# MoonInTheRiver/NeuralSVB

Measured on NVIDIA B200. Metric: audio-seconds/sec generated (HiFi-GAN-NSF generator forward), higher is better.
Workload: dtype 3xbf16 split operands (16-bit mantissa), fp32 accumulate, fp32 storage

## Files before the change

include/svb_vocoder.h:

```cpp
#ifndef SVB_VOCODER_H_
#define SVB_VOCODER_H_

#include <stdint.h>

#ifdef __cplusplus
extern "C" {
#endif

#define SVB_ABI_VERSION 1

typedef enum svb_status {
    SVB_OK = 0,
    SVB_ERR_INVALID = -1,
    SVB_ERR_CUDA = -2,
    SVB_ERR_STATE = -3,
    SVB_ERR_MISSING = -4,
    SVB_ERR_NOMEM = -5
} svb_status;

typedef enum svb_precision {
    SVB_PREC_FP32 = 0,
    SVB_PREC_TF32 = 1,
    SVB_PREC_TF32X3 = 2,
    SVB_PREC_BF16X3 = 3
} svb_precision;

#define SVB_MAX_UPS 8
#define SVB_MAX_RBK 4
#define SVB_MAX_DIL 4

typedef struct svb_gen_config {
    int32_t n_mel;
    int32_t upsample_initial_channel;
    int32_t n_ups;
    int32_t upsample_rates[SVB_MAX_UPS];
    int32_t upsample_kernel_sizes[SVB_MAX_UPS];
    int32_t resblock;
    int32_t n_resblock_kernels;
    int32_t resblock_kernel_sizes[SVB_MAX_RBK];
    int32_t n_dilations;
    int32_t resblock_dilation_sizes[SVB_MAX_RBK][SVB_MAX_DIL];
    int32_t use_pitch_embed;
    int32_t audio_sample_rate;
    int32_t precision;
} svb_gen_config;

typedef struct svb_gen svb_gen_t;

const char *svb_last_error(void);
int svb_abi_version(void);


int svb_gen_create(const svb_gen_config *cfg, int device, svb_gen_t **out);
void svb_gen_destroy(svb_gen_t *g);

int svb_gen_set_weight(svb_gen_t *g, const char *name, const float *data, const int64_t *shape, int32_t ndim);
int svb_fold_weight_norm_host(const float *v_host, const float *g_host, int64_t d0, int64_t inner,
                              float *w_host, int device);
int svb_gen_finalize(svb_gen_t *g);
int svb_gen_set_precision(svb_gen_t *g, int32_t precision);

int svb_gen_forward(svb_gen_t *g, const float *mel_dev, const float *f0_dev, const float *rand_ini_dev,
                    const float *noise_dev, uint64_t seed, int32_t B, int32_t T, float *wav_dev, void *stream);

int svb_gen_spec2wav_host(svb_gen_t *g, const float *mel_host, const float *f0_host, uint64_t seed,
                          int32_t B, int32_t T, float *wav_host, void *stream);

int svb_gen_spec2wav_host_i16(svb_gen_t *g, const float *mel_host, const float *f0_host, uint64_t seed, int32_t B,
                              int32_t T, int32_t norm, int16_t *wav_host, void *stream);
int svb_wav_to_int16(const float *wav_dev, int32_t B, int64_t n, int32_t norm, int16_t *out_dev, void *stream);

int svb_gen_forward_ragged(svb_gen_t *g, const float *mel_dev, const float *f0_dev, const int32_t *lengths_host,
                           const float *rand_ini_dev, const float *noise_dev, uint64_t seed, int32_t B, int32_t T_max,
                           float *wav_dev, void *stream);
int svb_gen_spec2wav_ragged_host(svb_gen_t *g, const float *mel_host, const float *f0_host, const int32_t *lengths_host,
                                 int32_t B, uint64_t seed, float *wav_host, void *stream);
int svb_gen_spec2wav_ragged_host_i16(svb_gen_t *g, const float *mel_host, const float *f0_host, const int32_t *lengths_host,
                                     int32_t B, uint64_t seed, int32_t norm, int16_t *wav_host, void *stream);

int svb_gen_get_tap(svb_gen_t *g, const char *name, float *out_dev, int64_t capacity_floats,
                    int64_t *shape3, void *stream);
int64_t svb_gen_hop(const svb_gen_t *g);
int64_t svb_gen_last_launches(const svb_gen_t *g);
double svb_gen_last_flops(const svb_gen_t *g);
int svb_gen_enable_timing(svb_gen_t *g, int32_t on);
float svb_gen_last_ms(svb_gen_t *g);
int32_t svb_gen_profile_count(svb_gen_t *g);
int svb_gen_profile_get(svb_gen_t *g, int32_t i, char *name, int32_t name_cap, float *ms, double *bytes, double *flops);

int svb_conv_nct_backward(const float *x_dev, const float *w_dev, const float *y_dev, const float *dy_dev, int32_t B,
                          int32_t Cin, int32_t Cout, int32_t Tin, int32_t W, int32_t K, int32_t stride, int32_t dil,
                          int32_t pad, int32_t groups, float out_slope, float *dz_scratch_dev, float *dx_dev,
                          float *dw_dev, float *db_dev, void *stream);
int svb_cond_net_forward(const float *mel_dev, const float *w_dev, const float *bias_dev, int32_t B, int32_t C, int32_t T,
                         int32_t K, int32_t stride, int32_t pad, float *y_dev, void *stream);
int svb_cond_net_backward(const float *mel_dev, const float *dy_dev, int32_t B, int32_t C, int32_t T, int32_t K, int32_t stride,
                          int32_t pad, float *dw_dev, float *db_dev, void *stream);
int svb_avgpool1d_4_2_1_backward(const float *dy_dev, float *dx_dev, int64_t rows, int32_t Tin, void *stream);
int svb_pad_reflect_right_backward(const float *dy_dev, float *dx_dev, int64_t rows, int32_t T, int32_t Tpad, void *stream);
int svb_loss_grad(const float *a_dev, const float *b_dev, int32_t kind, float scale, float *da_dev, int64_t n,
                  int32_t accumulate, void *stream);
int svb_loss_grad_dev(const float *a_dev, const float *b_dev, int32_t kind, float scale, const float *scale_dev,
                      float *da_dev, int64_t n, int32_t accumulate, void *stream);

typedef struct svb_tc_layer svb_tc_layer_t;
int svb_tc_layer_create(int32_t Cin, int32_t Cout, int32_t K, int32_t stride, int32_t pad, int32_t precision, int device,
                        svb_tc_layer_t **out);
int svb_tc_layer_create_grouped(int32_t Cin, int32_t Cout, int32_t K, int32_t stride, int32_t pad, int32_t groups,
                                int32_t precision, int device, svb_tc_layer_t **out);
void svb_tc_layer_destroy(svb_tc_layer_t *layer);
int svb_tc_layer_set_weight_dev(svb_tc_layer_t *layer, const float *w_dev, const float *bias_dev, void *stream);
int64_t svb_tc_layer_out_len(const svb_tc_layer_t *layer, int64_t T);
int svb_tc_layer_forward(svb_tc_layer_t *layer, const float *x_dev, int32_t B, int32_t T, int32_t W, float out_slope,
                         float *y_dev, void *stream);
int svb_tc_layer_backward(svb_tc_layer_t *layer, const float *x_dev, const float *y_dev, const float *dy_dev, int32_t B,
                          int32_t T, int32_t W, float out_slope, float *dx_dev, float *dw_dev, float *db_dev, void *stream);

int svb_gen_set_training(svb_gen_t *g, int32_t on);
int svb_gen_update_weights(svb_gen_t *g);
int svb_gen_set_weight_dev(svb_gen_t *g, const char *name, const float *src_dev, int64_t n, void *stream);
int svb_gen_update_weights_dev(svb_gen_t *g, void *stream);
int svb_fold_weight_norm_dev(const float *v_dev, const float *g_dev, int64_t d0, int64_t inner, float *w_dev, void *stream);
int svb_gen_zero_grad(svb_gen_t *g, void *stream);
int svb_gen_backward(svb_gen_t *g, const float *dwav_dev, void *stream);
int64_t svb_gen_grad_numel(svb_gen_t *g, const char *name);
int svb_gen_get_grad(svb_gen_t *g, const char *name, float *dst_dev, int64_t n, void *stream);
int64_t svb_gen_bwd_launches(const svb_gen_t *g);
int svb_weight_norm_backward(const float *v_dev, const float *g_dev, const float *dw_dev, int64_t rows, int64_t cols,
                             float *dv_dev, float *dg_dev, void *stream);

int svb_conv1d_run(const float *x_nct_dev, const float *w_host, const float *bias_host, const float *res_nct_dev,
                   int32_t B, int32_t Cin, int32_t Cout, int32_t T, int32_t K, int32_t dil,
                   int32_t transposed_stride, float in_slope, float out_scale, int32_t precision, int32_t iters,
                   float *y_nct_dev, float *avg_ms, void *stream);


int svb_conv_nct_forward(const float *x_dev, const float *w_dev, const float *bias_dev, float *y_dev, int32_t B,
                         int32_t Cin, int32_t Cout, int32_t Tin, int32_t W, int32_t K, int32_t stride, int32_t dil,
                         int32_t pad, int32_t groups, float out_slope, void *stream);
int svb_avgpool1d_4_2_1(const float *x_dev, float *y_dev, int64_t rows, int32_t Tin, void *stream);
int svb_pad_reflect_right(const float *x_dev, float *y_dev, int64_t rows, int32_t T, int32_t Tpad, void *stream);
int svb_pair_stats(const float *a_dev, const float *b_dev, int64_t n, int32_t want_log, double *out6_dev, void *stream);
int svb_spectral_sigma_host(const float *w_host, const float *u_host, const float *v_host, int64_t rows, int64_t inner,
                            int device, float *sigma);


typedef enum svb_pad_mode {
    SVB_PAD_CENTER_ZERO = 0,
    SVB_PAD_CENTER_REFLECT = 1,
    SVB_PAD_HALF_REFLECT = 2
} svb_pad_mode;

typedef enum svb_spec_out {
    SVB_OUT_LOG10_MEL = 0,
    SVB_OUT_LN_MEL = 1,
    SVB_OUT_MAG = 2,
    SVB_OUT_MAG_RAW = 3,
    SVB_OUT_MEL_MAG = 4
} svb_spec_out;

typedef struct svb_stft_config {
    int32_t n_fft;
    int32_t hop;
    int32_t win;
    int32_t pad_mode;
    int32_t out_kind;
    int32_t clamp_input;
    int32_t n_mels;
    int32_t frames_major;
    float eps;
} svb_stft_config;

int64_t svb_stft_num_frames(const svb_stft_config *cfg, int64_t n);

int svb_stft_forward(const svb_stft_config *cfg, const float *wav_dev, int32_t B, int64_t n,
                     const float *mel_basis_dev, float *out_dev, void *stream);
int svb_stft_backward(const svb_stft_config *cfg, const float *wav_dev, int32_t B, int64_t n, const float *mel_basis_dev,
                      const float *dout_dev, float *dwav_dev, void *stream);

int svb_denoise(const svb_stft_config *cfg, const float *wav_dev, int32_t B, int64_t n, float v, float *out_dev, void *stream);

int64_t svb_wav2spec_host(const svb_stft_config *cfg, const float *wav_host, int64_t n,
                          const float *mel_basis_host, float *mel_host, float *wav_out_host, int device,
                          void *stream);

int64_t svb_wav2spec_batch_host(const svb_stft_config *cfg, const float *wav_concat_host, const int64_t *lengths,
                                int32_t n_clips, const float *mel_basis_host, float *mel_concat_host, int64_t *frames_out,
                                int device, void *stream);

typedef struct svb_wn svb_wn_t;
int svb_wn_create(int32_t hidden_channels, int32_t kernel_size, int32_t dilation_rate, int32_t n_layers, int32_t gin_channels,
                  int32_t precision, int32_t device, svb_wn_t **out);
void svb_wn_destroy(svb_wn_t *w);
int svb_wn_set_weight(svb_wn_t *w, const char *name, const float *data_host, const int64_t *shape, int32_t ndim);
int svb_wn_finalize(svb_wn_t *w);
int svb_wn_forward(svb_wn_t *w, const float *x_dev, const float *mask_dev, const float *g_dev, int32_t B, int32_t T, float *out_dev,
                   void *stream);
int svb_fvae_decoder_create(int32_t latent_channels, int32_t hidden_channels, int32_t out_channels, int32_t kernel_size, int32_t n_layers,
                            int32_t gin_channels, int32_t stride, int32_t precision, int32_t device, svb_wn_t **out);
int svb_fvae_decoder_forward(svb_wn_t *w, const float *z_dev, const float *mask_dev, const float *g_dev, int32_t B, int32_t T,
                             float *out_dev, void *stream);

int svb_layer_norm_nct(const float *x_dev, const float *gamma_dev, const float *beta_dev, int32_t B, int32_t C, int32_t T, float eps,
                       float *y_dev, void *stream);
int svb_relpos_attention_nct(const float *q_dev, const float *k_dev, const float *v_dev, const float *p_dev, const float *bias_u_dev,
                             const float *bias_v_dev, const float *mask_dev, int32_t B, int32_t C, int32_t T, int32_t n_head,
                             float *out_dev, void *stream);

int64_t svb_tc_schedule_probe(int32_t n_layers, const int32_t *KS, const int32_t *has_res, const int32_t *accumulate, int32_t Cin, int32_t B,
                              int32_t Tq, int32_t MT, int32_t col_blocks, int32_t chain_ordered, int32_t grid, int32_t *items_out,
                              int64_t items_capacity, int32_t *off_out, double *balance_out);
int64_t svb_tc_schedule_probe_ragged(int32_t n_layers, const int32_t *KS, const int32_t *has_res, const int32_t *accumulate,
                                     int32_t Cin, int32_t B, const int32_t *rows_per_clip, int32_t MT, int32_t col_blocks,
                                     int32_t chain_ordered, int32_t grid, int32_t *items_out, int64_t items_capacity,
                                     int32_t *off_out, double *balance_out);

#ifdef __cplusplus
}
#endif
#endif
```

neuralsvb_b200/_native.py:

```python
import ctypes
import os
import shutil
import subprocess
import threading

_HERE = os.path.dirname(os.path.abspath(__file__))
_ROOT = os.path.dirname(_HERE)
CSRC = os.path.join(_HERE, 'csrc')
LIB_PATH = os.path.join(_HERE, 'libsvb_vocoder.so')
HEADER = os.path.join(_ROOT, 'include', 'svb_vocoder.h')
SOURCES = ['wn.cu', 'conformer.cu', 'api.cu', 'conv_ffma.cu', 'conv_tc.cu', 'nsf_source.cu', 'frontend.cu', 'generator.cu', 'layer_api.cu', 'disc_ops.cu',
           'train_ops.cu', 'generator_bwd.cu', 'disc_bwd.cu', 'tc_layer.cu', 'wgrad_tc.cu']
NVCC_FLAGS = ['-gencode', 'arch=compute_100a,code=sm_100a', '-lineinfo', '-O3', '-std=c++17',
              '-Xcompiler', '-fPIC', '-shared']

SVB_MAX_UPS, SVB_MAX_RBK, SVB_MAX_DIL = 8, 4, 4
PREC = {'fp32': 0, 'tf32': 1, 'tf32x3': 2, 'bf16x3': 3}
PAD_CENTER_ZERO, PAD_CENTER_REFLECT, PAD_HALF_REFLECT = 0, 1, 2
OUT_LOG10_MEL, OUT_LN_MEL, OUT_MAG, OUT_MAG_RAW, OUT_MEL_MAG = 0, 1, 2, 3, 4


class GenConfig(ctypes.Structure):
    _fields_ = [
        ('n_mel', ctypes.c_int32),
        ('upsample_initial_channel', ctypes.c_int32),
        ('n_ups', ctypes.c_int32),
        ('upsample_rates', ctypes.c_int32 * SVB_MAX_UPS),
        ('upsample_kernel_sizes', ctypes.c_int32 * SVB_MAX_UPS),
        ('resblock', ctypes.c_int32),
        ('n_resblock_kernels', ctypes.c_int32),
        ('resblock_kernel_sizes', ctypes.c_int32 * SVB_MAX_RBK),
        ('n_dilations', ctypes.c_int32),
        ('resblock_dilation_sizes', (ctypes.c_int32 * SVB_MAX_DIL) * SVB_MAX_RBK),
        ('use_pitch_embed', ctypes.c_int32),
        ('audio_sample_rate', ctypes.c_int32),
        ('precision', ctypes.c_int32),
    ]


class StftConfig(ctypes.Structure):
    _fields_ = [
        ('n_fft', ctypes.c_int32), ('hop', ctypes.c_int32), ('win', ctypes.c_int32),
        ('pad_mode', ctypes.c_int32), ('out_kind', ctypes.c_int32), ('clamp_input', ctypes.c_int32),
        ('n_mels', ctypes.c_int32), ('frames_major', ctypes.c_int32), ('eps', ctypes.c_float),
    ]


def sources():
    return [os.path.join(CSRC, s) for s in SOURCES if os.path.exists(os.path.join(CSRC, s))]


def _stale():
    if not os.path.exists(LIB_PATH):
        return True
    t = os.path.getmtime(LIB_PATH)
    deps = sources() + [HEADER] + [os.path.join(CSRC, f) for f in os.listdir(CSRC) if f.endswith('.cuh')]
    return any(os.path.getmtime(d) > t for d in deps)


def build(force=False, verbose=False):
    if not force and not _stale():
        return LIB_PATH
    nvcc = shutil.which('nvcc') or '/usr/local/cuda/bin/nvcc'
    if not os.path.exists(nvcc):
        raise RuntimeError('nvcc not found: cannot build libsvb_vocoder.so')
    cmd = [nvcc] + NVCC_FLAGS + sources() + ['-o', LIB_PATH + '.tmp']
    if verbose:
        print(' '.join(cmd))
    r = subprocess.run(cmd, capture_output=True, text=True)
    if r.returncode != 0:
        raise RuntimeError('nvcc failed:\n' + r.stdout + r.stderr)
    os.replace(LIB_PATH + '.tmp', LIB_PATH)
    return LIB_PATH


_lib = None
_lock = threading.Lock()

_P = ctypes.c_void_p
_I32, _I64, _U64 = ctypes.c_int32, ctypes.c_int64, ctypes.c_uint64

_PROTOS = {
    'svb_last_error': (ctypes.c_char_p, []),
    'svb_abi_version': (ctypes.c_int, []),
    'svb_gen_create': (ctypes.c_int, [ctypes.POINTER(GenConfig), ctypes.c_int, ctypes.POINTER(_P)]),
    'svb_gen_destroy': (None, [_P]),
    'svb_gen_set_weight': (ctypes.c_int, [_P, ctypes.c_char_p, _P, ctypes.POINTER(_I64), _I32]),
    'svb_fold_weight_norm_host': (ctypes.c_int, [_P, _P, _I64, _I64, _P, ctypes.c_int]),
    'svb_gen_finalize': (ctypes.c_int, [_P]),
    'svb_gen_set_precision': (ctypes.c_int, [_P, _I32]),
    'svb_gen_forward': (ctypes.c_int, [_P, _P, _P, _P, _P, _U64, _I32, _I32, _P, _P]),
    'svb_gen_spec2wav_host': (ctypes.c_int, [_P, _P, _P, _U64, _I32, _I32, _P, _P]),
    'svb_gen_get_tap': (ctypes.c_int, [_P, ctypes.c_char_p, _P, _I64, ctypes.POINTER(_I64), _P]),
    'svb_gen_hop': (_I64, [_P]),
    'svb_gen_last_launches': (_I64, [_P]),
    'svb_gen_last_flops': (ctypes.c_double, [_P]),
    'svb_gen_enable_timing': (ctypes.c_int, [_P, _I32]),
    'svb_gen_last_ms': (ctypes.c_float, [_P]),
    'svb_conv_nct_backward': (ctypes.c_int, [_P, _P, _P, _P, _I32, _I32, _I32, _I32, _I32, _I32, _I32, _I32, _I32, _I32,
                                             ctypes.c_float, _P, _P, _P, _P, _P]),
    'svb_avgpool1d_4_2_1_backward': (ctypes.c_int, [_P, _P, _I64, _I32, _P]),
    'svb_cond_net_forward': (ctypes.c_int, [_P, _P, _P, _I32, _I32, _I32, _I32, _I32, _I32, _P, _P]),
    'svb_cond_net_backward': (ctypes.c_int, [_P, _P, _I32, _I32, _I32, _I32, _I32, _I32, _P, _P, _P]),
    'svb_pad_reflect_right_backward': (ctypes.c_int, [_P, _P, _I64, _I32, _I32, _P]),
    'svb_loss_grad': (ctypes.c_int, [_P, _P, _I32, ctypes.c_float, _P, _I64, _I32, _P]),
    'svb_loss_grad_dev': (ctypes.c_int, [_P, _P, _I32, ctypes.c_float, _P, _P, _I64, _I32, _P]),
    'svb_tc_layer_create': (ctypes.c_int, [_I32, _I32, _I32, _I32, _I32, _I32, ctypes.c_int, ctypes.POINTER(_P)]),
    'svb_tc_layer_create_grouped': (ctypes.c_int, [_I32, _I32, _I32, _I32, _I32, _I32, _I32, ctypes.c_int, ctypes.POINTER(_P)]),
    'svb_tc_layer_destroy': (None, [_P]),
    'svb_tc_layer_set_weight_dev': (ctypes.c_int, [_P, _P, _P, _P]),
    'svb_tc_layer_out_len': (_I64, [_P, _I64]),
    'svb_tc_layer_forward': (ctypes.c_int, [_P, _P, _I32, _I32, _I32, ctypes.c_float, _P, _P]),
    'svb_tc_layer_backward': (ctypes.c_int, [_P, _P, _P, _P, _I32, _I32, _I32, ctypes.c_float, _P, _P, _P, _P]),
    'svb_gen_set_training': (ctypes.c_int, [_P, _I32]),
    'svb_gen_update_weights': (ctypes.c_int, [_P]),
    'svb_gen_zero_grad': (ctypes.c_int, [_P, _P]),
    'svb_gen_set_weight_dev': (ctypes.c_int, [_P, ctypes.c_char_p, _P, _I64, _P]),
    'svb_gen_update_weights_dev': (ctypes.c_int, [_P, _P]),
    'svb_fold_weight_norm_dev': (ctypes.c_int, [_P, _P, _I64, _I64, _P, _P]),
    'svb_gen_backward': (ctypes.c_int, [_P, _P, _P]),
    'svb_gen_grad_numel': (_I64, [_P, ctypes.c_char_p]),
    'svb_gen_get_grad': (ctypes.c_int, [_P, ctypes.c_char_p, _P, _I64, _P]),
    'svb_gen_bwd_launches': (_I64, [_P]),
    'svb_weight_norm_backward': (ctypes.c_int, [_P, _P, _P, _I64, _I64, _P, _P, _P]),
    'svb_gen_profile_count': (_I32, [_P]),
    'svb_gen_profile_get': (ctypes.c_int, [_P, _I32, ctypes.c_char_p, _I32, ctypes.POINTER(ctypes.c_float),
                                            ctypes.POINTER(ctypes.c_double), ctypes.POINTER(ctypes.c_double)]),
    'svb_conv1d_run': (ctypes.c_int, [_P, _P, _P, _P, _I32, _I32, _I32, _I32, _I32, _I32, _I32, ctypes.c_float,
                                      ctypes.c_float, _I32, _I32, _P, ctypes.POINTER(ctypes.c_float), _P]),
    'svb_conv_nct_forward': (ctypes.c_int, [_P, _P, _P, _P, _I32, _I32, _I32, _I32, _I32, _I32, _I32, _I32, _I32, _I32,
                                            ctypes.c_float, _P]),
    'svb_avgpool1d_4_2_1': (ctypes.c_int, [_P, _P, _I64, _I32, _P]),
    'svb_pad_reflect_right': (ctypes.c_int, [_P, _P, _I64, _I32, _I32, _P]),
    'svb_pair_stats': (ctypes.c_int, [_P, _P, _I64, _I32, _P, _P]),
    'svb_spectral_sigma_host': (ctypes.c_int, [_P, _P, _P, _I64, _I64, ctypes.c_int, ctypes.POINTER(ctypes.c_float)]),
    'svb_stft_num_frames': (_I64, [ctypes.POINTER(StftConfig), _I64]),
    'svb_stft_forward': (ctypes.c_int, [ctypes.POINTER(StftConfig), _P, _I32, _I64, _P, _P, _P]),
    'svb_stft_backward': (ctypes.c_int, [ctypes.POINTER(StftConfig), _P, _I32, _I64, _P, _P, _P, _P]),
    'svb_denoise': (ctypes.c_int, [ctypes.POINTER(StftConfig), _P, _I32, _I64, ctypes.c_float, _P, _P]),
    'svb_wav2spec_host': (_I64, [ctypes.POINTER(StftConfig), _P, _I64, _P, _P, _P, ctypes.c_int, _P]),
    'svb_wav2spec_batch_host': (_I64, [ctypes.POINTER(StftConfig), _P, _P, _I32, _P, _P, _P, ctypes.c_int, _P]),
    'svb_gen_spec2wav_host_i16': (ctypes.c_int, [_P, _P, _P, _U64, _I32, _I32, _I32, _P, _P]),
    'svb_wav_to_int16': (ctypes.c_int, [_P, _I32, _I64, _I32, _P, _P]),
    'svb_wn_create': (ctypes.c_int, [_I32, _I32, _I32, _I32, _I32, _I32, _I32, ctypes.POINTER(_P)]),
    'svb_wn_destroy': (None, [_P]),
    'svb_wn_set_weight': (ctypes.c_int, [_P, ctypes.c_char_p, _P, ctypes.POINTER(_I64), _I32]),
    'svb_wn_finalize': (ctypes.c_int, [_P]),
    'svb_wn_forward': (ctypes.c_int, [_P, _P, _P, _P, _I32, _I32, _P, _P]),
    'svb_fvae_decoder_create': (ctypes.c_int, [_I32, _I32, _I32, _I32, _I32, _I32, _I32, _I32, _I32, ctypes.POINTER(_P)]),
    'svb_fvae_decoder_forward': (ctypes.c_int, [_P, _P, _P, _P, _I32, _I32, _P, _P]),
    'svb_tc_schedule_probe': (_I64, [_I32, _P, _P, _P, _I32, _I32, _I32, _I32, _I32, _I32, _I32, _P, _I64, _P, ctypes.POINTER(ctypes.c_double)]),
    'svb_tc_schedule_probe_ragged': (_I64, [_I32, _P, _P, _P, _I32, _I32, _P, _I32, _I32, _I32, _I32, _P, _I64, _P,
                                            ctypes.POINTER(ctypes.c_double)]),
    'svb_gen_forward_ragged': (ctypes.c_int, [_P, _P, _P, _P, _P, _P, _U64, _I32, _I32, _P, _P]),
    'svb_gen_spec2wav_ragged_host': (ctypes.c_int, [_P, _P, _P, _P, _I32, _U64, _P, _P]),
    'svb_gen_spec2wav_ragged_host_i16': (ctypes.c_int, [_P, _P, _P, _P, _I32, _U64, _I32, _P, _P]),
    'svb_layer_norm_nct': (ctypes.c_int, [_P, _P, _P, _I32, _I32, _I32, ctypes.c_float, _P, _P]),
    'svb_relpos_attention_nct': (ctypes.c_int, [_P, _P, _P, _P, _P, _P, _P, _I32, _I32, _I32, _I32, _P, _P]),
}


def declared_symbols():
    import re
    txt = open(HEADER).read()
    txt = re.sub(r'/\*.*?\*/', '', txt, flags=re.S)
    return sorted(set(re.findall(r'\b(svb_[a-z0-9_]+)\s*\(', txt)))


def lib():
    global _lib
    if _lib is not None:
        return _lib
    with _lock:
        if _lib is None:
            if not os.path.exists(LIB_PATH):
                raise RuntimeError(
                    f'{LIB_PATH} is missing: run `python -c "import __graft_entry__ as g; g.build()"` '
                    '(nvcc, sm_100a). neuralsvb_b200 has no CPU or PyTorch fallback.')
            l = ctypes.CDLL(LIB_PATH)
            for name, (res, args) in _PROTOS.items():
                if hasattr(l, name):
                    fn = getattr(l, name)
                    fn.restype, fn.argtypes = res, args
            _lib = l
    return _lib


def check(status, what=''):
    if status is not None and status < 0:
        msg = lib().svb_last_error().decode('utf-8', 'replace')
        raise RuntimeError(f'libsvb_vocoder {what} failed ({status}): {msg}')
    return status


def ptr(t):
    if t is None:
        return None
    assert t.is_contiguous(), 'native calls need contiguous tensors'
    return ctypes.c_void_p(t.data_ptr())


def current_stream_ptr(device=None):
    import torch
    return ctypes.c_void_p(torch.cuda.current_stream(device).cuda_stream)
```

neuralsvb_b200/csrc/conv_tc.cu:

```cuda
#include <algorithm>
#include <cmath>
#include <cstring>
#include <cstdlib>
#include <vector>

#include <cuda_bf16.h>

#include "conv_tc.cuh"
#include "tc_ptx.cuh"

namespace svb {

constexpr int kTcM = 128;
constexpr int kTcCK = 32;
constexpr int kMaxItems = 120;
constexpr int kItemBytes = 2048;


struct TcLayer {
    const float *in;
    const float *res;
    float *out;
    const float *bias;
    const unsigned char *w;
    int KS, dil;
    float out_scale;
    int accumulate;
    int bias_off;
    uint32_t w_res_off;
};

struct TcArgs {
    ConvArgs a;
    TcLayer L[kTcMaxLayers];
    int n_layers;
    const int4 *work;
    const int *work_off;
    int n_tile, n_chunks, MT, nW, nA, tmem_cols;
    int n_sets;
    int col_blocks, groups_per_b, total_groups;
    int w_resident;
    int blk_chunk_step;
    uint32_t w_res_bytes;
    int pdl;
    int collect;
    long long *stats;
    int dbg;
    uint32_t op_bytes;
    uint32_t wtile_bytes;
    uint32_t off_op, off_w, off_stage, off_bias;
};

constexpr int kMaxW = 8;
constexpr int kMaxDevices = 64;
constexpr int kTcThreadsP = 576;
constexpr int kWarpProducer = 16, kWarpMma = 17, kWarpTransform0 = 8;
constexpr int kStageBytes = 8 * 4096;
constexpr int kBiasBytes = 4096;

template <bool ST>
__device__ __forceinline__ void mbar_wait_t(uint64_t *bar, uint32_t parity, long long &acc) {
    if (ST) {
        const long long t = clock64();
        mbar_wait(bar, parity);
        acc += clock64() - t;
    } else {
        mbar_wait(bar, parity);
    }
}
template <bool ST>
__device__ __forceinline__ void mbar_wait_warp(uint64_t *bar, uint32_t parity, long long &acc) {
    mbar_wait_t<ST>(bar, parity, acc);
    __syncwarp();
}
constexpr int kTcStatSlots = 16;

struct TcItem {
    int layer, nblk, mt, b, t0, rows;
};
__device__ __forceinline__ TcItem item_decode(const int4 v) {
    TcItem it;
    it.layer = v.x & 0xff, it.nblk = (v.x >> 8) & 0xffff, it.mt = v.x >> 24, it.b = v.y, it.t0 = v.z, it.rows = v.w;
    return it;
}

template <int MODE, bool ST = false, bool RG = false>
__global__ void __launch_bounds__(kTcThreadsP, 1) conv1d_c4_tc_kernel(const __grid_constant__ TcArgs p) {
    extern __shared__ __align__(1024) unsigned char smem[];
    constexpr bool BF = MODE == SVB_PREC_BF16X3;
    constexpr bool X3 = MODE == SVB_PREC_TF32X3;
    const ConvArgs &a = p.a;
    uint64_t *bars = reinterpret_cast<uint64_t *>(smem);
    uint64_t *raw_full = bars, *a_ready = bars + 4, *a_empty = bars + 8;
    uint64_t *w_full = bars + 12, *w_empty = bars + 12 + kMaxW;
    uint64_t *acc_full = bars + 12 + 2 * kMaxW, *acc_empty = acc_full + 2;
    uint32_t *tmem_ptr = reinterpret_cast<uint32_t *>(acc_empty + 2);
    int *n_items_s = reinterpret_cast<int *>(tmem_ptr + 1);
    TcLayer *Ls = reinterpret_cast<TcLayer *>(smem + 512);
    const int4 *items = reinterpret_cast<const int4 *>(smem + 1024);
    unsigned char *op0 = smem + p.off_op;
    unsigned char *wring = smem + p.off_w;

    const int warp = threadIdx.x >> 5, lane = threadIdx.x & 31;
    const int acc_cols = p.MT * p.n_tile;
    long long st_w0 = 0, st_w1 = 0, st_w2 = 0;
    const long long st_t0 = ST ? clock64() : 0;
    unsigned long long st_g0 = 0;
    if (ST) asm volatile("mov.u64 %0, %%globaltimer;" : "=l"(st_g0));

    if (threadIdx.x == 0) {
        for (int i = 0; i < 4; ++i) mbar_init(raw_full + i, 1), mbar_init(a_ready + i, 8), mbar_init(a_empty + i, 1);
        for (int i = 0; i < 2; ++i) mbar_init(acc_full + i, 1), mbar_init(acc_empty + i, 8);
        for (int i = 0; i < kMaxW; ++i) mbar_init(w_full + i, 1), mbar_init(w_empty + i, 1);
        fence_barrier_init();
    }
    if (warp == kWarpMma) tmem_alloc(tmem_ptr, p.tmem_cols);
    {
        float *sb = reinterpret_cast<float *>(smem + p.off_bias);
        for (int l = 0; l < p.n_layers; ++l)
            for (int i = threadIdx.x; i < a.Cout; i += kTcThreadsP) sb[p.L[l].bias_off + i] = __ldg(p.L[l].bias + i);
        if (threadIdx.x < p.n_layers) Ls[threadIdx.x] = p.L[threadIdx.x];
        int4 *it_w = reinterpret_cast<int4 *>(smem + 1024);
        if (p.work) {
            const int i0 = __ldg(p.work_off + blockIdx.x), n = __ldg(p.work_off + blockIdx.x + 1) - i0;
            for (int i = threadIdx.x; i < n; i += kTcThreadsP) it_w[i] = __ldg(p.work + i0 + i);
            if (threadIdx.x == 0) *n_items_s = n;
        } else if (RG) {
            if (threadIdx.x == 0) {
                int n = 0;
                for (int g = blockIdx.x; g < p.total_groups; g += gridDim.x) {
                    const int tg = g % p.groups_per_b, r = g / p.groups_per_b, b = r % a.B;
                    const int rows = a.rows[b] * a.rows_mul, tiles = (rows + kTcM - 1) / kTcM;
                    if (tg * p.MT >= tiles) continue;
                    it_w[n++] = make_int4(((r / a.B) << 8) | (min(p.MT, tiles - tg * p.MT) << 24), b, tg * (kTcM * p.MT), rows);
                }
                *n_items_s = n;
            }
        } else {
            const int n = ((int)blockIdx.x < p.total_groups) ? (p.total_groups - 1 - (int)blockIdx.x) / (int)gridDim.x + 1 : 0;
            for (int i = threadIdx.x; i < n; i += kTcThreadsP) {
                const int g = blockIdx.x + i * gridDim.x;
                const int tg = g % p.groups_per_b, r = g / p.groups_per_b;
                it_w[i] = make_int4(((r / a.B) << 8) | (p.MT << 24), r % a.B, tg * (kTcM * p.MT), a.Tq);
            }
            if (threadIdx.x == 0) *n_items_s = n;
        }
    }
    tc_fence_before();
    __syncthreads();
    tc_fence_after();
    const uint32_t tmem_base = *tmem_ptr;
    const int n_items = *n_items_s;
    if (p.pdl) {
        asm volatile("griddepcontrol.wait;" ::: "memory");
        asm volatile("griddepcontrol.launch_dependents;" ::: "memory");
    }

    if (warp == kWarpProducer) {
        if (lane == 0) {
            const int gin = c4t_groups(a.Cin);
            const size_t group_stride = (size_t)a.in_Tp * 32;
            int sA = 0, phA = 1, sW = 0, phW = 1;
            if (p.w_resident && n_items > 0) {
                mbar_expect_tx(w_full, p.w_res_bytes);
                for (int l = 0; l < p.n_layers; ++l)
                    bulk_g2s(wring + Ls[l].w_res_off, Ls[l].w, (uint32_t)Ls[l].KS * p.wtile_bytes, w_full);
            }
            for (int n = 0; n < n_items; ++n) {
                const TcItem it = item_decode(items[n]);
                const TcLayer &L = Ls[it.layer];
                const int halo = (L.KS - 1) / 2 * L.dil;
                const uint32_t raw_bytes = (uint32_t)(it.mt * kTcM + 2 * halo) * 128;
                const float *in_c = L.in + (((size_t)it.b * gin + (size_t)it.nblk * p.blk_chunk_step) * a.in_Tp + (kPad + it.t0 - halo)) * 32;
                const unsigned char *w_k = L.w + (size_t)it.nblk * p.n_chunks * L.KS * p.wtile_bytes;
                for (int c = 0; c < p.n_chunks; ++c) {
                    mbar_wait_t<ST>(a_empty + sA, phA, st_w0);
                    mbar_expect_tx(raw_full + sA, raw_bytes);
                    bulk_g2s(op0 + sA * p.op_bytes, in_c, raw_bytes, raw_full + sA);
                    in_c += group_stride;
                    if (++sA == p.nA) sA = 0, phA ^= 1;
                    if (!p.w_resident) {
                        for (int k = 0; k < L.KS; ++k) {
                            mbar_wait_t<ST>(w_empty + sW, phW, st_w1);
                            mbar_expect_tx(w_full + sW, p.wtile_bytes);
                            bulk_g2s(wring + sW * p.wtile_bytes, w_k, p.wtile_bytes, w_full + sW);
                            w_k += p.wtile_bytes;
                            if (++sW == p.nW) sW = 0, phW ^= 1;
                        }
                    }
                }
            }
            if (ST) {
                long long *o = p.stats + (size_t)blockIdx.x * kTcStatSlots;
                o[0] = st_w0, o[1] = st_w1, o[2] = clock64() - st_t0;
            }
        }
    } else if (warp == kWarpMma) {
        const uint32_t elected = elect_one_sync();
        const uint32_t idesc = umma_idesc(BF ? 1 : 2, kTcM, p.n_tile);
        const uint32_t hi_word = desc_hi_sw128(0);
        const uint32_t a_lo_plane = (X3 ? p.op_bytes / 2 : 64u) >> 4;
        const uint32_t b_lo_plane = (X3 ? p.wtile_bytes / 2 : 64u) >> 4;
        const uint32_t op_base = desc_lo(smem_u32(op0)), w_base = desc_lo(smem_u32(wring));
        const uint32_t op_step = p.op_bytes >> 4, wtile_step = p.wtile_bytes >> 4;
        const bool mma_on = ST ? !(p.dbg & 1) : true, hh_only = ST ? (p.dbg & 2) != 0 : false, collect = ST ? p.collect != 0 : true;
        int sA = 0, phA = 0, sW = 0, phW = 0, as = 0, phE = 1;
        if (p.w_resident && n_items > 0) {
            mbar_wait_warp<ST>(w_full, 0, st_w2);
            tc_fence_after();
        }
        const int n_items_u = __reduce_max_sync(0xffffffffu, n_items);
        for (int n = 0; n < n_items_u; ++n) {
            const int ix = __reduce_max_sync(0xffffffffu, items[n].x);
            const int layer = ix & 0xff, mt = ix >> 24;
            const int KS = p.L[layer].KS;
            const uint32_t tap_step = (uint32_t)p.L[layer].dil * (128 >> 4);
            const uint32_t w_res_off = p.L[layer].w_res_off >> 4;
            mbar_wait_warp<ST>(acc_empty + as, phE, st_w0);
            tc_fence_after();
            const uint32_t d_set = tmem_base + (uint32_t)(as * acc_cols);
            uint32_t fresh = 1;
            for (int c = 0; c < p.n_chunks; ++c) {
                mbar_wait_warp<ST>(a_ready + sA, phA, st_w1);
                tc_fence_after();
                uint32_t a_tap = op_base + sA * op_step;
                uint32_t b_tap = w_base + w_res_off;
                for (int k = 0; k < KS; ++k) {
                    if (!p.w_resident) {
                        mbar_wait_warp<ST>(w_full + sW, phW, st_w2);
                        tc_fence_after();
                        b_tap = w_base + sW * wtile_step;
                    }
                    if (mma_on) {
                        uint32_t d = d_set, a_row = a_tap;
#pragma unroll 1
                        for (int m = 0; m < mt; ++m) {
                            const uint32_t acc = fresh ^ 1u;
                            if (BF) {
                                if (hh_only) {
                                    umma<true>(d, a_row, hi_word, b_tap, hi_word, idesc, acc, elected);
                                    umma<true>(d, a_row + 2, hi_word, b_tap + 2, hi_word, idesc, 1u, elected);
                                } else if (collect) {
                                    umma<true>(d, a_row + a_lo_plane, hi_word, b_tap, hi_word, idesc, acc, elected);
                                    umma<true, 1>(d, a_row, hi_word, b_tap + b_lo_plane, hi_word, idesc, 1u, elected);
                                    umma<true, 2>(d, a_row, hi_word, b_tap, hi_word, idesc, 1u, elected);
                                    umma<true>(d, a_row + a_lo_plane + 2, hi_word, b_tap + 2, hi_word, idesc, 1u, elected);
                                    umma<true, 1>(d, a_row + 2, hi_word, b_tap + b_lo_plane + 2, hi_word, idesc, 1u, elected);
                                    umma<true, 2>(d, a_row + 2, hi_word, b_tap + 2, hi_word, idesc, 1u, elected);
                                } else {
                                    umma<true>(d, a_row + a_lo_plane, hi_word, b_tap, hi_word, idesc, acc, elected);
                                    umma<true>(d, a_row, hi_word, b_tap + b_lo_plane, hi_word, idesc, 1u, elected);
                                    umma<true>(d, a_row, hi_word, b_tap, hi_word, idesc, 1u, elected);
                                    umma<true>(d, a_row + a_lo_plane + 2, hi_word, b_tap + 2, hi_word, idesc, 1u, elected);
                                    umma<true>(d, a_row + 2, hi_word, b_tap + b_lo_plane + 2, hi_word, idesc, 1u, elected);
                                    umma<true>(d, a_row + 2, hi_word, b_tap + 2, hi_word, idesc, 1u, elected);
                                }
                            } else {
#pragma unroll
                                for (uint32_t kb = 0; kb < 8; kb += 2) {
                                    const uint32_t acc_k = kb == 0 ? acc : 1u;
                                    if (X3) {
                                        umma<false>(d, a_row + a_lo_plane + kb, hi_word, b_tap + kb, hi_word, idesc, acc_k, elected);
                                        umma<false, 1>(d, a_row + kb, hi_word, b_tap + b_lo_plane + kb, hi_word, idesc, 1u, elected);
                                        umma<false, 2>(d, a_row + kb, hi_word, b_tap + kb, hi_word, idesc, 1u, elected);
                                    } else {
                                        umma<false>(d, a_row + kb, hi_word, b_tap + kb, hi_word, idesc, acc_k, elected);
                                    }
                                }
                            }
                            d += (uint32_t)p.n_tile, a_row += (kTcM * 128) >> 4;
                        }
                    }
                    fresh = 0;
                    a_tap += tap_step, b_tap += wtile_step;
                    if (!p.w_resident) {
                        umma_commit(w_empty + sW, elected);
                        if (++sW == p.nW) sW = 0, phW ^= 1;
                    }
                }
                umma_commit(a_empty + sA, elected);
                if (++sA == p.nA) sA = 0, phA ^= 1;
            }
            umma_commit(acc_full + as, elected);
            if (++as == p.n_sets) as = 0, phE ^= 1;
        }
        if (ST && elected) {
            long long *o = p.stats + (size_t)blockIdx.x * kTcStatSlots;
            o[3] = st_w0, o[4] = st_w1, o[5] = st_w2, o[6] = clock64() - st_t0;
        }
    } else if (warp >= kWarpTransform0) {
        const int tid = threadIdx.x - kWarpTransform0 * 32;
        const int cl = tid & 7;
        const bool odd = cl & 1;
        const float slope = a.in_slope;
        int sA = 0, phA = 0;
        for (int n = 0; n < n_items; ++n) {
            const TcItem it = item_decode(items[n]);
            const int R = it.mt * kTcM + (Ls[it.layer].KS - 1) / 2 * Ls[it.layer].dil * 2;
            for (int c = 0; c < p.n_chunks; ++c) {
                mbar_wait_t<ST>(raw_full + sA, phA, st_w0);
                uint4 *op = reinterpret_cast<uint4 *>(op0 + sA * p.op_bytes);
                for (int r0 = 0; r0 < ((p.dbg & 4) ? 0 : R); r0 += 64) {
                    int rr[2];
                    bool ok[2];
                    float4 v[2];
#pragma unroll
                    for (int u = 0; u < 2; ++u) {
                        rr[u] = r0 + 32 * u + (tid >> 3);
                        ok[u] = rr[u] < R;
                        v[u] = make_float4(0.f, 0.f, 0.f, 0.f);
                        if (ok[u]) v[u] = *reinterpret_cast<const float4 *>(op + (size_t)rr[u] * 8 + cl);
                    }
#pragma unroll
                    for (int u = 0; u < 2; ++u) {
                        float4 &x = v[u];
                        x.x = fmaxf(x.x, x.x * slope), x.y = fmaxf(x.y, x.y * slope);
                        x.z = fmaxf(x.z, x.z * slope), x.w = fmaxf(x.w, x.w * slope);
                    }
                    if (BF) {
                        uint32_t h0[2], h1[2], l0[2], l1[2], g0[2], g1[2];
#pragma unroll
                        for (int u = 0; u < 2; ++u) {
                            const __nv_bfloat162 hA = __floats2bfloat162_rn(v[u].x, v[u].y), hB = __floats2bfloat162_rn(v[u].z, v[u].w);
                            h0[u] = *reinterpret_cast<const uint32_t *>(&hA), h1[u] = *reinterpret_cast<const uint32_t *>(&hB);
                            const __nv_bfloat162 lA = __floats2bfloat162_rn(v[u].x - __uint_as_float(h0[u] << 16),
                                                                           v[u].y - __uint_as_float(h0[u] & 0xffff0000u));
                            const __nv_bfloat162 lB = __floats2bfloat162_rn(v[u].z - __uint_as_float(h1[u] << 16),
                                                                           v[u].w - __uint_as_float(h1[u] & 0xffff0000u));
                            l0[u] = *reinterpret_cast<const uint32_t *>(&lA), l1[u] = *reinterpret_cast<const uint32_t *>(&lB);
                        }
#pragma unroll
                        for (int u = 0; u < 2; ++u) {
                            g0[u] = __shfl_xor_sync(0xffffffffu, odd ? h0[u] : l0[u], 1);
                            g1[u] = __shfl_xor_sync(0xffffffffu, odd ? h1[u] : l1[u], 1);
                        }
#pragma unroll
                        for (int u = 0; u < 2; ++u) {
                            if (!ok[u]) continue;
                            uint4 *row = op + (size_t)rr[u] * 8;
                            const int sw = rr[u] & 7;
                            if (!odd) row[(cl >> 1) ^ sw] = make_uint4(h0[u], h1[u], g0[u], g1[u]);
                            else row[(4 + (cl >> 1)) ^ sw] = make_uint4(g0[u], g1[u], l0[u], l1[u]);
                        }
                    } else {
                        __syncwarp();
#pragma unroll
                        for (int u = 0; u < 2; ++u) {
                            if (!ok[u]) continue;
                            uint4 *row = op + (size_t)rr[u] * 8;
                            const int sw = rr[u] & 7;
                            const float4 h = make_float4(to_tf32(v[u].x), to_tf32(v[u].y), to_tf32(v[u].z), to_tf32(v[u].w));
                            row[cl ^ sw] = make_uint4(__float_as_uint(h.x), __float_as_uint(h.y), __float_as_uint(h.z), __float_as_uint(h.w));
                            if (X3)
                                (row + p.op_bytes / 32)[cl ^ sw] =
                                    make_uint4(__float_as_uint(to_tf32(v[u].x - h.x)), __float_as_uint(to_tf32(v[u].y - h.y)),
                                               __float_as_uint(to_tf32(v[u].z - h.z)), __float_as_uint(to_tf32(v[u].w - h.w)));
                        }
                    }
                }
                fence_proxy_async();
                __syncwarp();
                if (lane == 0) mbar_arrive(a_ready + sA);
                if (++sA == p.nA) sA = 0, phA ^= 1;
            }
        }
        if (ST && tid == 0) {
            long long *o = p.stats + (size_t)blockIdx.x * kTcStatSlots;
            o[7] = st_w0, o[8] = clock64() - st_t0;
        }
    } else {
        const int ew = warp;
        const int lane_base = 32 * (warp & 3);
        const int half = ew >> 2;
        const int gout = c4t_groups(a.Cout);
        float4 *tile = reinterpret_cast<float4 *>(smem + p.off_stage + ew * 4096);
        const int jb = p.n_tile / 32;
        const int wr = lane >> 3, wc = lane & 7;
        const bool no_mem = p.dbg & 8;
        const size_t rstep = (size_t)(a.ups_u > 0 ? a.ups_u : 1) * 8;
        float4 rres[8];
        auto block_base = [&](const TcItem &it, int blk, int &co0, int &q_base) -> size_t {
            const int m = blk / jb, j = blk - m * jb;
            q_base = it.t0 + m * kTcM + lane_base;
            const int cop0 = it.nblk * p.n_tile + j * 32;
            int phi = 0;
            co0 = cop0;
            if (a.ups_u > 0) { phi = cop0 / a.Cout; co0 = cop0 - phi * a.Cout; }
            return (((size_t)it.b * gout + (co0 >> 5)) * a.out_Tp + kPad +
                    (a.ups_u > 0 ? (size_t)q_base * a.ups_u + phi : (size_t)q_base)) * 8;
        };
        auto fetch_res = [&](int n, int blk) {
            if (no_mem || n >= n_items) return;
            const TcItem it = item_decode(items[n]);
            const float4 *res4 = reinterpret_cast<const float4 *>(Ls[it.layer].res);
            if (!res4 || blk >= it.mt * jb) return;
            int co0, q_base;
            const size_t base = block_base(it, blk, co0, q_base);
#pragma unroll
            for (int i = 0; i < 8; ++i) {
                const int rr = 4 * i + wr;
                rres[i] = (q_base + rr < (RG ? it.rows : a.Tq)) ? __ldg(res4 + base + (size_t)rr * rstep + wc) : make_float4(0.f, 0.f, 0.f, 0.f);
            }
        };
        fetch_res(0, half);
        int as = 0, phF = 0;
        for (int n = 0; n < n_items; ++n) {
            const TcItem it = item_decode(items[n]);
            const TcLayer &L = Ls[it.layer];
            const bool has_res = L.res != nullptr;
            float4 *out4 = reinterpret_cast<float4 *>(L.out);
            const float out_scale = L.out_scale;
            const int accumulate = L.accumulate;
            const unsigned char *bias_s = smem + p.off_bias + (size_t)L.bias_off * 4;
            const int nblocks = it.mt * jb;
            mbar_wait_t<ST>(acc_full + as, phF, st_w0);
            tc_fence_after();
            for (int blk = half; blk < nblocks; blk += 2) {
                const int m = blk / jb, j = blk - m * jb;
                int co0, q_base;
                const size_t base = block_base(it, blk, co0, q_base);
                if (has_res) {
#pragma unroll
                    for (int i = 0; i < 8; ++i) tile[(4 * i + wr) * 8 + (wc ^ ((4 * i + wr) & 7))] = rres[i];
                    __syncwarp();
                }
                if (blk + 2 < nblocks) fetch_res(n, blk + 2);
                else fetch_res(n + 1, half);
#pragma unroll
                for (int hq = 0; hq < 2; ++hq) {
                    float v[16];
                    tmem_ld16(tmem_base + ((uint32_t)lane_base << 16) + (uint32_t)(as * acc_cols + m * p.n_tile + j * 32 + hq * 16), v);
#pragma unroll
                    for (int g4 = 0; g4 < 4; ++g4) {
                        const int gq = hq * 4 + g4;
                        const float4 bv = *reinterpret_cast<const float4 *>(bias_s + (size_t)(co0 + 4 * gq) * 4);
                        float4 o = make_float4(v[4 * g4] + bv.x, v[4 * g4 + 1] + bv.y, v[4 * g4 + 2] + bv.z, v[4 * g4 + 3] + bv.w);
                        float4 *slot = tile + lane * 8 + (gq ^ (lane & 7));
                        if (has_res) {
                            const float4 rv = *slot;
                            o.x += rv.x, o.y += rv.y, o.z += rv.z, o.w += rv.w;
                        }
                        o.x *= out_scale, o.y *= out_scale, o.z *= out_scale, o.w *= out_scale;
                        *slot = o;
                    }
                }
                __syncwarp();
                if (!no_mem) {
#pragma unroll
                    for (int i = 0; i < 8; ++i) {
                        const int rr = 4 * i + wr;
                        if (q_base + rr >= (RG ? it.rows : a.Tq)) continue;
                        float4 o = tile[rr * 8 + (wc ^ (rr & 7))];
                        float4 *dst = out4 + base + (size_t)rr * rstep + wc;
                        if (accumulate) {
                            const float4 old = *dst;
                            o.x += old.x, o.y += old.y, o.z += old.z, o.w += old.w;
                        }
                        *dst = o;
                    }
                }
                __syncwarp();
            }
            if (half >= nblocks) fetch_res(n + 1, half);
            tc_fence_before();
            __syncwarp();
            if (lane == 0) mbar_arrive(acc_empty + as);
            if (++as == p.n_sets) as = 0, phF ^= 1;
        }
        if (ST && threadIdx.x == 0) {
            long long *o = p.stats + (size_t)blockIdx.x * kTcStatSlots;
            o[9] = st_w0, o[10] = clock64() - st_t0;
        }
    }
    tc_fence_before();
    __syncthreads();
    if (ST && threadIdx.x == 0) {
        unsigned long long g1;
        asm volatile("mov.u64 %0, %%globaltimer;" : "=l"(g1));
        p.stats[(size_t)blockIdx.x * kTcStatSlots + 11] = clock64() - st_t0;
        p.stats[(size_t)blockIdx.x * kTcStatSlots + 12] = (long long)st_g0;
        p.stats[(size_t)blockIdx.x * kTcStatSlots + 13] = (long long)g1;
    }
    if (warp == kWarpMma) {
        tc_fence_after();
        tmem_dealloc(tmem_base, p.tmem_cols);
    }
}

static float host_tf32(float x) {
    uint32_t u;
    std::memcpy(&u, &x, 4);
    if ((u & 0x7F800000u) == 0x7F800000u) return x;
    u += 0x1000u;
    u &= 0xFFFFE000u;
    float r;
    std::memcpy(&r, &u, 4);
    return r;
}
static uint16_t host_bf16(float x) {
    uint32_t u;
    std::memcpy(&u, &x, 4);
    if ((u & 0x7F800000u) == 0x7F800000u) return (uint16_t)(u >> 16);
    u += 0x7FFFu + ((u >> 16) & 1u);
    return (uint16_t)(u >> 16);
}
static float bf16_to_float(uint16_t h) {
    const uint32_t u = (uint32_t)h << 16;
    float r;
    std::memcpy(&r, &u, 4);
    return r;
}

static int pick_n_tile(int CoutP) {
    if (CoutP % 32 != 0) return 0;
    if (CoutP <= 128) return CoutP;
    for (int n = 128; n >= 32; n -= 32)
        if (CoutP % n == 0) return n;
    return 0;
}

int tc_pack_weights(const float *packed, int KS, int Cin, int CoutP, TcWeights *out, std::vector<void *> *allocs, int force_n_tile) {
    out->KS = KS, out->Cin = Cin, out->CoutP = CoutP, out->ok = false;
    const int n_tile = force_n_tile > 0 ? force_n_tile : pick_n_tile(CoutP);
    if (force_n_tile > 0 && (CoutP % force_n_tile != 0 || force_n_tile % 32 != 0 || force_n_tile > 128)) return SVB_OK;
    if (n_tile == 0 || n_tile % 8 != 0 || Cin % 4 != 0) return SVB_OK;
    out->n_tile = n_tile;
    const int n_chunks = (Cin + kTcCK - 1) / kTcCK, n_blk = CoutP / n_tile;
    const size_t tile_b = (size_t)n_tile * 128;
    const size_t n_tiles = (size_t)n_blk * n_chunks * KS;
    std::vector<unsigned char> tf(n_tiles * tile_b), tf3(n_tiles * tile_b * 2), bf(n_tiles * tile_b);
    for (int nb = 0; nb < n_blk; ++nb)
        for (int c = 0; c < n_chunks; ++c)
            for (int k = 0; k < KS; ++k) {
                const size_t t = ((size_t)nb * n_chunks + c) * KS + k;
                float *t1 = reinterpret_cast<float *>(tf.data() + t * tile_b);
                float *t3h = reinterpret_cast<float *>(tf3.data() + t * tile_b * 2);
                float *t3l = reinterpret_cast<float *>(tf3.data() + t * tile_b * 2 + tile_b);
                uint16_t *tb = reinterpret_cast<uint16_t *>(bf.data() + t * tile_b);
                for (int n = 0; n < n_tile; ++n)
                    for (int ci = 0; ci < kTcCK; ++ci) {
                        const int cin_i = c * kTcCK + ci;
                        const float w = cin_i < Cin ? packed[((size_t)k * Cin + cin_i) * CoutP + nb * n_tile + n] : 0.f;
                        const float h = host_tf32(w);
                        const int c16 = ci >> 2;
                        const size_t i4 = (size_t)n * 32 + ((c16 ^ (n & 7)) << 2) + (ci & 3);
                        t1[i4] = h, t3h[i4] = h, t3l[i4] = host_tf32(w - h);
                        const uint16_t bh = host_bf16(w), bl = host_bf16(w - bf16_to_float(bh));
                        const int ch = ci >> 3, cl = 4 + (ci >> 3);
                        tb[(size_t)n * 64 + ((ch ^ (n & 7)) << 3) + (ci & 7)] = bh;
                        tb[(size_t)n * 64 + ((cl ^ (n & 7)) << 3) + (ci & 7)] = bl;
                    }
            }
    auto up = [&](const void *src, size_t bytes, void **dst) -> int {
        SVB_CUDA(cudaMalloc(dst, bytes));
        allocs->push_back(*dst);
        SVB_CUDA(cudaMemcpy(*dst, src, bytes, cudaMemcpyHostToDevice));
        return SVB_OK;
    };
    SVB_TRY(up(tf.data(), tf.size(), &out->blob[SVB_PREC_TF32]));
    SVB_TRY(up(tf3.data(), tf3.size(), &out->blob[SVB_PREC_TF32X3]));
    SVB_TRY(up(bf.data(), bf.size(), &out->blob[SVB_PREC_BF16X3]));
    out->ok = true;
    return SVB_OK;
}

__global__ void tc_repack_kernel(const float *__restrict__ packed, int KS, int Cin, int CoutP, int n_tile, int n_chunks,
                                 long long total, unsigned char *__restrict__ tf, unsigned char *__restrict__ tf3,
                                 unsigned char *__restrict__ bf) {
    const long long i = (long long)blockIdx.x * blockDim.x + threadIdx.x;
    if (i >= total) return;
    const int ci = (int)(i % kTcCK);
    const int n = (int)((i / kTcCK) % n_tile);
    const long long t = i / ((long long)kTcCK * n_tile);
    const int k = (int)(t % KS);
    const int c = (int)((t / KS) % n_chunks);
    const int nb = (int)(t / ((long long)KS * n_chunks));
    const int cin_i = c * kTcCK + ci;
    const float w = cin_i < Cin ? packed[((size_t)k * Cin + cin_i) * CoutP + nb * n_tile + n] : 0.f;
    auto tf32 = [](float x) {
        uint32_t u = __float_as_uint(x);
        if ((u & 0x7F800000u) == 0x7F800000u) return x;
        u += 0x1000u;
        u &= 0xFFFFE000u;
        return __uint_as_float(u);
    };
    const size_t tile_b = (size_t)n_tile * 128;
    const float h = tf32(w);
    const size_t i4 = (size_t)n * 32 + (((ci >> 2) ^ (n & 7)) << 2) + (ci & 3);
    reinterpret_cast<float *>(tf + t * tile_b)[i4] = h;
    reinterpret_cast<float *>(tf3 + t * tile_b * 2)[i4] = h;
    reinterpret_cast<float *>(tf3 + t * tile_b * 2 + tile_b)[i4] = tf32(w - h);
    const __nv_bfloat16 bh = __float2bfloat16_rn(w);
    const __nv_bfloat16 bl = __float2bfloat16_rn(w - __bfloat162float(bh));
    uint16_t *tb = reinterpret_cast<uint16_t *>(bf + t * tile_b);
    const int ch = ci >> 3, cl = 4 + (ci >> 3);
    tb[(size_t)n * 64 + ((ch ^ (n & 7)) << 3) + (ci & 7)] = __bfloat16_as_ushort(bh);
    tb[(size_t)n * 64 + ((cl ^ (n & 7)) << 3) + (ci & 7)] = __bfloat16_as_ushort(bl);
}

int tc_repack_weights_dev(const float *packed_dev, const TcWeights &w, cudaStream_t st) {
    if (!w.ok) return SVB_OK;
    const int n_chunks = (w.Cin + kTcCK - 1) / kTcCK, n_blk = w.CoutP / w.n_tile;
    const long long total = (long long)n_blk * n_chunks * w.KS * w.n_tile * kTcCK;
    tc_repack_kernel<<<(unsigned)((total + 255) / 256), 256, 0, st>>>(
        packed_dev, w.KS, w.Cin, w.CoutP, w.n_tile, n_chunks, total, reinterpret_cast<unsigned char *>(w.blob[SVB_PREC_TF32]),
        reinterpret_cast<unsigned char *>(w.blob[SVB_PREC_TF32X3]), reinterpret_cast<unsigned char *>(w.blob[SVB_PREC_BF16X3]));
    SVB_CUDA(cudaGetLastError());
    return SVB_OK;
}

bool tc_supported(const TcWeights &w, const ConvArgs &a) {
    if (a.cin_blk > 0 && (a.cin_blk % 32 != 0 || a.ups_u != 0 || (a.CoutP / w.n_tile) * a.cin_blk != a.Cin || w.Cin != a.cin_blk)) return false;
    return w.ok && a.Cin % 4 == 0 && a.bias != nullptr && (a.KS - 1) / 2 * a.dil <= kPad &&
           (a.ups_u == 0 || a.Cout % 32 == 0) && a.Cout <= 3072;
}

template <int MODE, bool ST, bool RG = false>
static int launch_mode(const TcArgs &p, int grid, size_t smem, cudaStream_t st) {
    auto kern = conv1d_c4_tc_kernel<MODE, ST, RG>;
    static size_t configured[kMaxDevices] = {};
    static bool carve[kMaxDevices] = {};
    int dev = 0;
    SVB_CUDA(cudaGetDevice(&dev));
    dev = dev < kMaxDevices ? dev : kMaxDevices - 1;
    if (smem > configured[dev] || dev == kMaxDevices - 1) {
        SVB_CUDA(cudaFuncSetAttribute(kern, cudaFuncAttributeMaxDynamicSharedMemorySize, (int)smem));
        configured[dev] = smem;
    }
    if (!carve[dev]) {
        SVB_CUDA(cudaFuncSetAttribute(kern, cudaFuncAttributePreferredSharedMemoryCarveout, cudaSharedmemCarveoutMaxShared));
        carve[dev] = true;
    }
    cudaLaunchConfig_t cfg = {};
    cfg.gridDim = dim3(grid), cfg.blockDim = dim3(kTcThreadsP), cfg.dynamicSmemBytes = smem, cfg.stream = st;
    cudaLaunchAttribute attr[1];
    attr[0].id = cudaLaunchAttributeProgrammaticStreamSerialization;
    attr[0].val.programmaticStreamSerializationAllowed = p.pdl ? 1 : 0;
    cfg.attrs = attr, cfg.numAttrs = 1;
    SVB_CUDA(cudaLaunchKernelEx(&cfg, kern, p));
    return SVB_OK;
}

static int sm_count() {
    static int n[kMaxDevices] = {};
    int dev = 0;
    cudaGetDevice(&dev);
    const int slot = dev < kMaxDevices ? dev : kMaxDevices - 1;
    if (n[slot] == 0 || slot == kMaxDevices - 1) {
        cudaDeviceGetAttribute(&n[slot], cudaDevAttrMultiProcessorCount, dev);
        if (n[slot] <= 0) n[slot] = 148;
    }
    return n[slot];
}

static int tc_plan(int n, const TcWeights *const *w, const ConvArgs *a, int precision, TcArgs &p, size_t &smem) {
    SVB_CHECK(n >= 1 && n <= kTcMaxLayers, SVB_ERR_INVALID, "tc conv: %d layers in one launch", n);
    const ConvArgs &a0 = a[0];
    for (int l = 1; l < n; ++l)
        SVB_CHECK(a[l].B == a0.B && a[l].Cin == a0.Cin && a[l].Cout == a0.Cout && a[l].CoutP == a0.CoutP && a[l].Tq == a0.Tq &&
                      a[l].in_Tp == a0.in_Tp && a[l].out_Tp == a0.out_Tp && a[l].ups_u == a0.ups_u && a[l].in_slope == a0.in_slope &&
                      a[l].cin_blk == a0.cin_blk && w[l]->n_tile == w[0]->n_tile,
                  SVB_ERR_INVALID, "tc conv: layers of one launch must share the shape class");
    p.a = a0, p.n_layers = n;
    p.work = nullptr, p.work_off = nullptr;
    const int cin_eff = a0.cin_blk > 0 ? a0.cin_blk : a0.Cin;
    p.n_tile = w[0]->n_tile, p.n_chunks = (cin_eff + kTcCK - 1) / kTcCK;
    p.blk_chunk_step = a0.cin_blk > 0 ? p.n_chunks : 0;
    int halo = 0, ks_sum = 0;
    for (int l = 0; l < n; ++l) halo = std::max(halo, (a[l].KS - 1) / 2 * a[l].dil), ks_sum += a[l].KS;
    const int tiles = (a0.Tq + kTcM - 1) / kTcM;
    p.col_blocks = a0.CoutP / p.n_tile;
    const int planes = precision == SVB_PREC_TF32X3 ? 2 : 1;
    p.wtile_bytes = (uint32_t)p.n_tile * 128 * planes;
    p.dbg = 0;
    if (const char *e = getenv("SVB_TC_DBG")) p.dbg = atoi(e);
    p.collect = 1;
    if (const char *e = getenv("SVB_TC_COLLECT")) p.collect = atoi(e) != 0;
    p.pdl = 1;
    if (const char *e = getenv("SVB_TC_PDL")) p.pdl = atoi(e) != 0;
    int force_mt = 0;
    if (const char *e = getenv("SVB_TC_MT")) force_mt = atoi(e);
    smem = 0;
    const size_t bias_bytes = (size_t)n * a0.Cout <= 1024 ? kBiasBytes : 3 * kBiasBytes;
    SVB_CHECK((size_t)n * a0.Cout * 4 <= bias_bytes, SVB_ERR_INVALID, "tc conv: %d layers x %d biases exceed the shared-memory bias area", n, a0.Cout);
    const size_t budget = 226 * 1024 - kStageBytes - bias_bytes;
    int force_sets = 0;
    if (const char *e = getenv("SVB_TC_SETS")) force_sets = atoi(e);
    bool planned = false;
    for (int MT : {4, 2, 1}) {
        if (force_mt && MT != force_mt && MT != 1) continue;
        int sets = 2 * MT * p.n_tile <= 512 ? 2 : 1;
        if (force_sets) sets = force_sets;
        if (sets * MT * p.n_tile > 512) continue;
        if (!force_mt) {
            if (MT == 4) continue;
            if (MT == 2 && tiles < 2) continue;
        }
        p.n_sets = sets;
        if ((tiles + MT - 1) / MT * MT * kTcM > round_up(a0.Tq, kTileT) && MT != 1) continue;
        p.MT = MT;
        const int R = MT * kTcM + 2 * halo;
        p.op_bytes = (uint32_t)round_up(R, 8) * 128 * planes;
        p.nA = 3;
        if (const char *e = getenv("SVB_TC_NA")) p.nA = std::max(2, std::min(4, atoi(e)));
        p.off_op = 1024 + kItemBytes;
        const size_t res_bytes = (size_t)ks_sum * p.wtile_bytes;
        const bool can_res = p.n_chunks == 1 && p.col_blocks == 1;
        p.w_resident = 0;
        for (int nA : {p.nA, 2}) {
            if (can_res && p.off_op + (size_t)nA * p.op_bytes + res_bytes <= budget) {
                p.nA = nA, p.w_resident = 1;
                break;
            }
        }
        p.off_w = p.off_op + (uint32_t)p.nA * p.op_bytes;
        if (!p.w_resident && p.off_w + 2 * (size_t)p.wtile_bytes > budget) {
            p.nA = 2;
            p.off_w = p.off_op + (uint32_t)p.nA * p.op_bytes;
        }
        if (!p.w_resident && p.off_w + 2 * (size_t)p.wtile_bytes > budget && MT != 1) continue;
        SVB_CHECK(p.w_resident || p.off_w + (size_t)p.wtile_bytes <= budget, SVB_ERR_INVALID,
                  "tc conv: tile does not fit shared memory (N %d)", p.n_tile);
        const size_t avail = budget - p.off_w;
        size_t w_area;
        if (p.w_resident) {
            p.nW = 1, p.w_res_bytes = (uint32_t)res_bytes, w_area = res_bytes;
        } else {
            p.nW = std::max(1, std::min((int)(avail / p.wtile_bytes), kMaxW));
            p.w_res_bytes = 0, w_area = (size_t)p.nW * p.wtile_bytes;
        }
        p.off_stage = p.off_w + (uint32_t)round_up((int)w_area, 1024);
        p.off_bias = p.off_stage + kStageBytes;
        smem = (size_t)p.off_bias + bias_bytes;
        planned = true;
        break;
    }
    SVB_CHECK(planned && smem <= 227 * 1024, SVB_ERR_INVALID, "tc conv: no tiling fits (N %d, %d layers)", p.n_tile, n);
    uint32_t res_off = 0;
    for (int l = 0; l < n; ++l) {
        TcLayer &L = p.L[l];
        L.in = a[l].in, L.res = a[l].res, L.out = a[l].out, L.bias = a[l].bias;
        L.w = reinterpret_cast<const unsigned char *>(w[l]->blob[precision]);
        L.KS = a[l].KS, L.dil = a[l].dil, L.out_scale = a[l].out_scale, L.accumulate = a[l].accumulate;
        L.bias_off = l * a0.Cout, L.w_res_off = res_off;
        res_off += (uint32_t)a[l].KS * p.wtile_bytes;
    }
    for (int l = n; l < kTcMaxLayers; ++l) p.L[l] = p.L[0];
    if (getenv("SVB_TC_VERBOSE"))
        fprintf(stderr, "[tc] %d layer(s) Cin %d CoutP %d KS %d.. halo %d Tq %d | n_tile %d MT %d sets %d nA %d nW %d resident %d smem %zu\n", n,
                a0.Cin, a0.CoutP, a0.KS, halo, a0.Tq, p.n_tile, p.MT, p.n_sets, p.nA, p.nW, p.w_resident, smem);
    int cols = 32;
    while (cols < p.n_sets * p.MT * p.n_tile) cols <<= 1;
    p.tmem_cols = cols;
    p.groups_per_b = (tiles + p.MT - 1) / p.MT;
    p.total_groups = p.groups_per_b * a0.B * p.col_blocks;
    p.stats = nullptr;
    return SVB_OK;
}

static int tc_dispatch(TcArgs &p, int precision, int grid, size_t smem, cudaStream_t st) {
    const ConvArgs &a = p.a;
    const bool want_stats = getenv("SVB_TC_STATS") != nullptr;
    if (a.rows) {
        switch (precision) {
            case SVB_PREC_TF32: return launch_mode<SVB_PREC_TF32, false, true>(p, grid, smem, st);
            case SVB_PREC_TF32X3: return launch_mode<SVB_PREC_TF32X3, false, true>(p, grid, smem, st);
            default: return launch_mode<SVB_PREC_BF16X3, false, true>(p, grid, smem, st);
        }
    }
    if ((want_stats || p.dbg != 0 || !p.collect) && precision == SVB_PREC_BF16X3) {
        const size_t n = (size_t)grid * kTcStatSlots;
        SVB_CUDA(cudaMalloc((void **)&p.stats, n * sizeof(long long)));
        SVB_CUDA(cudaMemsetAsync(p.stats, 0, n * sizeof(long long), st));
        SVB_TRY((launch_mode<SVB_PREC_BF16X3, true>(p, grid, smem, st)));
        SVB_CUDA(cudaStreamSynchronize(st));
        std::vector<long long> h(n);
        SVB_CUDA(cudaMemcpy(h.data(), p.stats, n * sizeof(long long), cudaMemcpyDeviceToHost));
        SVB_CUDA(cudaFree(p.stats));
        double mean[kTcStatSlots] = {};
        long long mx[kTcStatSlots] = {};
        for (int c = 0; c < grid; ++c)
            for (int i = 0; i < kTcStatSlots; ++i) mean[i] += (double)h[(size_t)c * kTcStatSlots + i] / grid, mx[i] = std::max(mx[i], h[(size_t)c * kTcStatSlots + i]);
        long long g_first = h[12], g_last = h[13];
        for (int c = 0; c < grid; ++c) g_first = std::min(g_first, h[(size_t)c * kTcStatSlots + 12]), g_last = std::max(g_last, h[(size_t)c * kTcStatSlots + 13]);
        if (want_stats) fprintf(stderr, "[tc-stats] grid span %.1f us (globaltimer, first CTA start -> last CTA end) = %.2f GHz over the mean CTA\n",
                                (g_last - g_first) / 1e3, mean[11] / std::max(1.0, (double)(g_last - g_first)));
        if (want_stats) fprintf(stderr,
                "[tc-stats] %dx C%d>%d k%d d%d Tq %d grid %d groups %d MT %d | kcycles mean (max): total %.0f (%.0f) | producer: a_empty %.0f w_empty %.0f of %.0f | "
                "mma: acc_empty %.0f a_ready %.0f w_full %.0f of %.0f | transform: raw_full %.0f of %.0f | epilogue: acc_full %.0f of %.0f\n",
                p.n_layers, a.Cin, a.CoutP, a.KS, a.dil, a.Tq, grid, p.total_groups, p.MT, mean[11] / 1e3, mx[11] / 1e3, mean[0] / 1e3, mean[1] / 1e3, mean[2] / 1e3,
                mean[3] / 1e3, mean[4] / 1e3, mean[5] / 1e3, mean[6] / 1e3, mean[7] / 1e3, mean[8] / 1e3, mean[9] / 1e3, mean[10] / 1e3);
        return SVB_OK;
    }
    switch (precision) {
        case SVB_PREC_TF32: return launch_mode<SVB_PREC_TF32, false>(p, grid, smem, st);
        case SVB_PREC_TF32X3: return launch_mode<SVB_PREC_TF32X3, false>(p, grid, smem, st);
        default: return launch_mode<SVB_PREC_BF16X3, false>(p, grid, smem, st);
    }
}

int launch_conv_tc(const TcWeights &w, const ConvArgs &a, int precision, cudaStream_t st, int max_ctas) {
    SVB_CHECK(precision >= SVB_PREC_TF32 && precision <= SVB_PREC_BF16X3, SVB_ERR_INVALID, "tc conv: bad precision %d",
              precision);
    TcArgs p;
    size_t smem = 0;
    const TcWeights *wp = &w;
    SVB_TRY(tc_plan(1, &wp, &a, precision, p, smem));
    const int grid = std::min(p.total_groups, max_ctas > 0 ? std::min(max_ctas, sm_count()) : sm_count());
    if ((p.total_groups + grid - 1) / grid > kMaxItems) {
        const int per_b = p.groups_per_b * p.col_blocks;
        const int nb = std::max(1, kMaxItems * grid / per_b);
        SVB_CHECK(per_b <= kMaxItems * grid, SVB_ERR_INVALID, "tc conv: one clip alone has %d work items", per_b);
        for (int b0 = 0; b0 < a.B; b0 += nb) {
            ConvArgs s = a;
            s.B = std::min(nb, a.B - b0);
            s.in = a.in + (size_t)b0 * c4t_groups(a.Cin) * a.in_Tp * 32;
            s.out = a.out + (size_t)b0 * c4t_groups(a.Cout) * a.out_Tp * 32;
            if (a.res) s.res = a.res + (size_t)b0 * c4t_groups(a.Cout) * a.out_Tp * 32;
            if (a.rows) s.rows = a.rows + b0;
            SVB_TRY(launch_conv_tc(w, s, precision, st, max_ctas));
        }
        return SVB_OK;
    }
    return tc_dispatch(p, precision, grid, smem, st);
}

bool tc_merge_fits(int n, int B, int Tq, int Cout, int n_tile, const int *rows) {
    long long groups = 0;
    for (int b = 0; b < B; ++b) {
        const int tiles = ((rows ? rows[b] : Tq) + kTcM - 1) / kTcM;
        groups += (tiles + 1) / 2;
    }
    groups *= std::max(1, Cout / std::max(1, n_tile));
    return groups * n <= (long long)(kMaxItems * 8 / 10) * sm_count();
}

void tc_worklist_free(TcWorkList *wl) {
    if (wl->items) cudaFree(wl->items);
    if (wl->off) cudaFree(wl->off);
    *wl = TcWorkList();
}

int tc_schedule(int n, const int *KS, const int *has_res, const int *accum, int Cin, int B, int Tq, int MT, int col_blocks, bool chain_ordered,
                int grid, std::vector<int4> *items_out, std::vector<int> *off_out, double *balance_out, const int *rows) {
    const double beta = 160.0 / std::max(32, Cin);
    struct Unit {
        double cost;
        int nblk, b, t0, mt, layer;
    };
    auto unit_cost = [&](int layer, int mt) {
        if (layer >= 0) return mt * (KS[layer] + beta + (has_res[layer] ? 1.0 : 0.0));
        double c = 0;
        for (int l = 0; l < n; ++l) c += mt * (KS[l] + beta + (has_res[l] ? 1.0 : 0.0) + (accum[l] ? 1.0 : 0.0));
        return c;
    };
    std::vector<Unit> units;
    for (int nblk = 0; nblk < col_blocks; ++nblk)
        for (int b = 0; b < B; ++b) {
            const int tiles = ((rows ? rows[b] : Tq) + kTcM - 1) / kTcM;
            for (int t = 0; t < tiles; t += MT) {
                const int mt = std::min(MT, tiles - t);
                if (chain_ordered) {
                    units.push_back({unit_cost(-1, mt), nblk, b, t * kTcM, mt, -1});
                } else {
                    for (int l = 0; l < n; ++l) units.push_back({unit_cost(l, mt), nblk, b, t * kTcM, mt, l});
                }
            }
        }
    std::vector<double> load;
    std::vector<std::vector<int>> mine;
    double balance = 0;
    for (int round = 0; round < 4; ++round) {
        std::stable_sort(units.begin(), units.end(), [](const Unit &x, const Unit &y) { return x.cost > y.cost; });
        load.assign(grid, 0.0);
        mine.assign(grid, std::vector<int>());
        for (size_t u = 0; u < units.size(); ++u) {
            int best = 0;
            for (int c = 1; c < grid; ++c)
                if (load[c] < load[best]) best = c;
            load[best] += units[u].cost;
            mine[best].push_back((int)u);
        }
        double mx = 0, sum = 0;
        for (double v : load) mx = std::max(mx, v), sum += v;
        balance = sum / grid / mx;
        if (balance >= 0.95 || !getenv("SVB_TC_SPLIT")) break;
        int split = 0;
        for (size_t u = units.size(); u-- > 0 && split < grid;) {
            if (units[u].mt != 2) continue;
            Unit h0 = units[u], h1 = units[u];
            h0.mt = h1.mt = 1, h1.t0 += kTcM;
            h0.cost = h1.cost = unit_cost(h0.layer, 1);
            units[u] = h0;
            units.push_back(h1);
            ++split;
        }
        if (!split) break;
    }
    std::vector<int4> &items = *items_out;
    std::vector<int> &off = *off_out;
    items.clear();
    off.assign(grid + 1, 0);
    for (int c = 0; c < grid; ++c) {
        std::sort(mine[c].begin(), mine[c].end(), [&](int x, int y) {
            const Unit &X = units[x], &Y = units[y];
            if (X.layer != Y.layer) return X.layer < Y.layer;
            if (X.nblk != Y.nblk) return X.nblk < Y.nblk;
            if (X.b != Y.b) return X.b < Y.b;
            return X.t0 < Y.t0;
        });
        const char *il = getenv("SVB_TC_INTERLEAVE");
        if (!chain_ordered && n > 1 && !(il && atoi(il) == 0)) {
            std::vector<std::vector<int>> by(n);
            for (int u : mine[c]) by[units[u].layer].push_back(u);
            std::vector<int> order;
            std::vector<size_t> pos(n, 0);
            const size_t total = mine[c].size();
            while (order.size() < total) {
                int best = -1;
                double lag = -1e30;
                for (int l = 0; l < n; ++l) {
                    if (pos[l] >= by[l].size()) continue;
                    const double want = (double)(order.size() + 1) * by[l].size() / total - (double)pos[l];
                    if (want > lag) lag = want, best = l;
                }
                order.push_back(by[best][pos[best]++]);
            }
            mine[c] = order;
        }
        for (int u : mine[c]) {
            const Unit &U = units[u];
            for (int l = (U.layer < 0 ? 0 : U.layer); l < (U.layer < 0 ? n : U.layer + 1); ++l)
                items.push_back(make_int4(l | (U.nblk << 8) | (U.mt << 24), U.b, U.t0, rows ? rows[U.b] : Tq));
        }
        off[c + 1] = (int)items.size();
        SVB_CHECK(off[c + 1] - off[c] <= kMaxItems, SVB_ERR_INVALID, "tc conv: %d work items on one CTA (limit %d)", off[c + 1] - off[c], kMaxItems);
    }
    *balance_out = balance;
    return SVB_OK;
}

int tc_worklist_build(int n, const TcWeights *const *w, const ConvArgs *a, int precision, bool chain_ordered, TcWorkList *out,
                      const int *rows, cudaStream_t st) {
    TcArgs p;
    size_t smem = 0;
    SVB_TRY(tc_plan(n, w, a, precision, p, smem));
    const int grid = sm_count();
    int KS[kTcMaxLayers], has_res[kTcMaxLayers], accum[kTcMaxLayers];
    for (int l = 0; l < n; ++l) KS[l] = a[l].KS, has_res[l] = a[l].res != nullptr, accum[l] = a[l].accumulate;
    std::vector<int4> items;
    std::vector<int> off;
    double balance = 0;
    SVB_TRY(tc_schedule(n, KS, has_res, accum, a[0].Cin, a[0].B, a[0].Tq, p.MT, p.col_blocks, chain_ordered, grid, &items, &off, &balance,
                        rows));
    if (items.size() > out->cap_items || off.size() > out->cap_off) {
        if (out->items) SVB_CUDA(cudaFree(out->items));
        if (out->off) SVB_CUDA(cudaFree(out->off));
        out->items = nullptr, out->off = nullptr;
        out->cap_items = std::max<size_t>(items.size(), 1) * 5 / 4, out->cap_off = off.size();
        SVB_CUDA(cudaMalloc((void **)&out->items, out->cap_items * sizeof(int4)));
        SVB_CUDA(cudaMalloc((void **)&out->off, out->cap_off * sizeof(int)));
    }
    SVB_CUDA(cudaMemcpyAsync(out->items, items.data(), items.size() * sizeof(int4), cudaMemcpyHostToDevice, st));
    SVB_CUDA(cudaMemcpyAsync(out->off, off.data(), off.size() * sizeof(int), cudaMemcpyHostToDevice, st));
    out->grid = grid, out->n_items = (int)items.size(), out->MT = p.MT, out->n_layers = n, out->chain_ordered = chain_ordered;
    out->valid = true;
    if (getenv("SVB_TC_VERBOSE"))
        fprintf(stderr, "[tc] work list: %d layers, %zu items over %d CTAs, balance %.3f (mean / max load)\n", n, items.size(), grid, balance);
    return SVB_OK;
}

int launch_conv_tc_multi(int n, const TcWeights *const *w, const ConvArgs *a, int precision, cudaStream_t st, const TcWorkList &wl) {
    SVB_CHECK(precision >= SVB_PREC_TF32 && precision <= SVB_PREC_BF16X3, SVB_ERR_INVALID, "tc conv: bad precision %d", precision);
    TcArgs p;
    size_t smem = 0;
    SVB_TRY(tc_plan(n, w, a, precision, p, smem));
    SVB_CHECK(wl.valid && wl.n_layers == n && wl.MT == p.MT && wl.grid == sm_count(), SVB_ERR_STATE,
              "tc conv: work list was built for another plan (layers %d / %d, MT %d / %d)", wl.n_layers, n, wl.MT, p.MT);
    p.work = wl.items, p.work_off = wl.off;
    return tc_dispatch(p, precision, wl.grid, smem, st);
}

}

extern "C" int64_t svb_tc_schedule_probe(int32_t n_layers, const int32_t *KS, const int32_t *has_res, const int32_t *accumulate, int32_t Cin,
                                         int32_t B, int32_t Tq, int32_t MT, int32_t col_blocks, int32_t chain_ordered, int32_t grid,
                                         int32_t *items_out, int64_t items_capacity, int32_t *off_out, double *balance_out) {
    SVB_CHECK(n_layers >= 1 && n_layers <= svb::kTcMaxLayers && KS && has_res && accumulate && B > 0 && Tq > 0 && (MT == 1 || MT == 2) &&
                  col_blocks >= 1 && grid >= 1 && items_out && off_out && balance_out,
              SVB_ERR_INVALID, "tc_schedule_probe: bad argument");
    std::vector<int4> items;
    std::vector<int> off;
    int ks[svb::kTcMaxLayers], hr[svb::kTcMaxLayers], ac[svb::kTcMaxLayers];
    for (int l = 0; l < n_layers; ++l) ks[l] = KS[l], hr[l] = has_res[l], ac[l] = accumulate[l];
    SVB_TRY(svb::tc_schedule(n_layers, ks, hr, ac, Cin, B, Tq, MT, col_blocks, chain_ordered != 0, grid, &items, &off, balance_out, nullptr));
    SVB_CHECK((int64_t)items.size() <= items_capacity, SVB_ERR_INVALID, "tc_schedule_probe: %zu items, capacity %lld", items.size(),
              (long long)items_capacity);
    for (size_t i = 0; i < items.size(); ++i) {
        int32_t *o = items_out + 5 * i;
        o[0] = items[i].x & 0xff, o[1] = (items[i].x >> 8) & 0xffff, o[2] = items[i].y, o[3] = items[i].z, o[4] = items[i].x >> 24;
    }
    for (int c = 0; c <= grid; ++c) off_out[c] = off[c];
    return (int64_t)items.size();
}

extern "C" int64_t svb_tc_schedule_probe_ragged(int32_t n_layers, const int32_t *KS, const int32_t *has_res, const int32_t *accumulate,
                                                int32_t Cin, int32_t B, const int32_t *rows_per_clip, int32_t MT, int32_t col_blocks,
                                                int32_t chain_ordered, int32_t grid, int32_t *items_out, int64_t items_capacity,
                                                int32_t *off_out, double *balance_out) {
    SVB_CHECK(n_layers >= 1 && n_layers <= svb::kTcMaxLayers && KS && has_res && accumulate && B > 0 && rows_per_clip && (MT == 1 || MT == 2) &&
                  col_blocks >= 1 && grid >= 1 && items_out && off_out && balance_out,
              SVB_ERR_INVALID, "tc_schedule_probe_ragged: bad argument");
    int Tq = 0;
    for (int b = 0; b < B; ++b) {
        SVB_CHECK(rows_per_clip[b] >= 1, SVB_ERR_INVALID, "tc_schedule_probe_ragged: clip %d has %d rows", b, rows_per_clip[b]);
        Tq = std::max(Tq, (int)rows_per_clip[b]);
    }
    std::vector<int4> items;
    std::vector<int> off;
    int ks[svb::kTcMaxLayers], hr[svb::kTcMaxLayers], ac[svb::kTcMaxLayers];
    for (int l = 0; l < n_layers; ++l) ks[l] = KS[l], hr[l] = has_res[l], ac[l] = accumulate[l];
    const std::vector<int> rows(rows_per_clip, rows_per_clip + B);
    SVB_TRY(svb::tc_schedule(n_layers, ks, hr, ac, Cin, B, Tq, MT, col_blocks, chain_ordered != 0, grid, &items, &off, balance_out, rows.data()));
    SVB_CHECK((int64_t)items.size() <= items_capacity, SVB_ERR_INVALID, "tc_schedule_probe_ragged: %zu items, capacity %lld", items.size(),
              (long long)items_capacity);
    for (size_t i = 0; i < items.size(); ++i) {
        int32_t *o = items_out + 5 * i;
        o[0] = items[i].x & 0xff, o[1] = (items[i].x >> 8) & 0xffff, o[2] = items[i].y, o[3] = items[i].z, o[4] = items[i].x >> 24;
    }
    for (int c = 0; c <= grid; ++c) off_out[c] = off[c];
    return (int64_t)items.size();
}
```

neuralsvb_b200/csrc/conv_tc.cuh:

```cuda
#pragma once
#include <vector>

#include "conv_ffma.cuh"

namespace svb {

struct TcWeights {
    void *blob[4] = {nullptr, nullptr, nullptr, nullptr};
    int KS = 0, Cin = 0, CoutP = 0;
    int n_tile = 0;
    bool ok = false;
};

int tc_pack_weights(const float *packed_ffma, int KS, int Cin, int CoutP, TcWeights *out, std::vector<void *> *allocs,
                    int force_n_tile = 0);
int tc_repack_weights_dev(const float *packed_ffma_dev, const TcWeights &w, cudaStream_t st);
bool tc_supported(const TcWeights &w, const ConvArgs &a);

constexpr int kTcMaxLayers = 3;
struct TcWorkList {
    int4 *items = nullptr;
    int *off = nullptr;
    int grid = 0, n_items = 0, MT = 0, n_layers = 0;
    bool chain_ordered = false;
    bool valid = false;
    size_t cap_items = 0, cap_off = 0;
};
int tc_worklist_build(int n, const TcWeights *const *w, const ConvArgs *a, int precision, bool chain_ordered, TcWorkList *out,
                      const int *rows = nullptr, cudaStream_t st = 0);
void tc_worklist_free(TcWorkList *wl);
bool tc_merge_fits(int n, int B, int Tq, int Cout, int n_tile, const int *rows = nullptr);
int launch_conv_tc_multi(int n, const TcWeights *const *w, const ConvArgs *a, int precision, cudaStream_t st, const TcWorkList &wl);
int launch_conv_tc(const TcWeights &w, const ConvArgs &a, int precision, cudaStream_t st, int max_ctas = 0);

}
```

neuralsvb_b200/csrc/generator.cu:

```cuda
#include <algorithm>
#include <cstring>
#include <map>
#include <string>
#include <vector>

#include "generator.cuh"

using namespace svb;

int svb::gen_upload(svb_gen *g, const std::vector<float> &h, float **out) {
    float *d = nullptr;
    SVB_CUDA(cudaMalloc((void **)&d, std::max<size_t>(h.size(), 4) * sizeof(float)));
    SVB_CUDA(cudaMemcpy(d, h.data(), h.size() * sizeof(float), cudaMemcpyHostToDevice));
    g->dev_allocs.push_back(d);
    *out = d;
    return SVB_OK;
}

int svb::gen_get_w(svb_gen *g, const std::string &name, std::vector<int64_t> want, const HostTensor **out) {
    auto it = g->host_w.find(name);
    SVB_CHECK(it != g->host_w.end(), SVB_ERR_MISSING, "weight '%s' was never set", name.c_str());
    if (!want.empty()) {
        bool ok = it->second.shape.size() == want.size();
        for (size_t i = 0; ok && i < want.size(); ++i) ok = it->second.shape[i] == want[i];
        if (!ok) {
            std::string s;
            for (auto v : it->second.shape) s += std::to_string(v) + ",";
            std::string w;
            for (auto v : want) w += std::to_string(v) + ",";
            set_error("weight '%s' has shape [%s] but the config needs [%s]", name.c_str(), s.c_str(), w.c_str());
            return SVB_ERR_INVALID;
        }
    }
    *out = &it->second;
    return SVB_OK;
}

namespace {

int pack_conv(svb_gen *g, const std::string &prefix, int Cin, int Cout, int K, int dil, ConvLayer *L) {
    const HostTensor *w, *b;
    SVB_TRY(gen_get_w(g, prefix + ".weight", {Cout, Cin, K}, &w));
    SVB_TRY(gen_get_w(g, prefix + ".bias", {Cout}, &b));
    const std::vector<float> p = pack_conv_weights(w->data.data(), Cout, Cin, K);
    L->Cin = Cin, L->Cout = Cout, L->CoutP = Cout, L->KS = K, L->dil = dil, L->ups_u = 0;
    L->macs_per_row = (double)Cin * Cout * K;
    SVB_TRY(gen_upload(g, p, &L->w));
    SVB_TRY(gen_upload(g, b->data, &L->b));
    SVB_TRY(tc_pack_weights(p.data(), K, Cin, Cout, &L->tc, &g->dev_allocs));
    return SVB_OK;
}

int pack_convT(svb_gen *g, const std::string &prefix, int Cin, int Cout, int K, int u, int pad, ConvLayer *L) {
    const HostTensor *w, *b;
    SVB_TRY(gen_get_w(g, prefix + ".weight", {Cin, Cout, K}, &w));
    SVB_TRY(gen_get_w(g, prefix + ".bias", {Cout}, &b));
    int KS = 0;
    const std::vector<float> p = pack_convT_weights(w->data.data(), Cin, Cout, K, u, pad, &KS);
    SVB_CHECK(KS <= 11, SVB_ERR_INVALID, "upsampler %s: kernel %d / stride %d needs %d taps", prefix.c_str(), K, u, KS);
    L->Cin = Cin, L->Cout = Cout, L->CoutP = u * Cout, L->KS = KS, L->dil = 1, L->ups_u = u;
    L->macs_per_row = (double)Cin * Cout * K;
    SVB_TRY(gen_upload(g, p, &L->w));
    SVB_TRY(gen_upload(g, b->data, &L->b));
    SVB_TRY(tc_pack_weights(p.data(), KS, Cin, u * Cout, &L->tc, &g->dev_allocs));
    return SVB_OK;
}

struct Plan {
    size_t total = 0;
    size_t take(size_t bytes) {
        const size_t off = total;
        total += (bytes + 255) / 256 * 256;
        return off;
    }
};

Buffers plan_workspace(const svb_gen *g, int B, int T, size_t *total) {
    Plan p;
    Buffers b;
    b.mel = p.take(c4t_floats(B, g->cfg.n_mel, T) * 4);
    b.pre = p.take(c4t_floats(B, g->cfg.upsample_initial_channel, T) * 4);
    b.har = p.take((size_t)B * T * g->hop * 4);
    b.nsf = p.take(nsf_workspace_bytes(B, T, g->hop));
    int Ti = T;
    for (auto &s : g->stages) {
        Ti *= s.u;
        const size_t n = c4t_floats(B, s.C, Ti) * 4;
        b.X.push_back(p.take(n)), b.S.push_back(p.take(n));
        b.A.emplace_back(), b.R.emplace_back();
        for (int j = 0; j < g->cfg.n_resblock_kernels; ++j) {
            std::vector<size_t> a(g->cfg.n_dilations), r(g->cfg.n_dilations);
            for (int m = 0; m < g->cfg.n_dilations; ++m) {
                a[m] = (m == 0 || g->training) ? p.take(n) : a[0];
                r[m] = (m == 0 || g->training) ? p.take(n) : r[0];
            }
            b.A.back().push_back(a), b.R.back().push_back(r);
        }
    }
    if (g->training) {
        b.sines = p.take((size_t)B * T * g->hop * 9 * 4);
        b.wav = p.take((size_t)B * T * g->hop * 4);
    }
    *total = p.total;
    return b;
}

cudaEvent_t prof_event(svb_gen *g) {
    if (g->ev_used == g->ev_pool.size()) {
        cudaEvent_t e;
        cudaEventCreate(&e);
        g->ev_pool.push_back(e);
    }
    return g->ev_pool[g->ev_used++];
}
struct ProfScope {
    svb_gen *g;
    cudaStream_t st;
    cudaEvent_t e1 = nullptr;
    ProfScope(svb_gen *g_, cudaStream_t st_, const char *name, double bytes, double flops) : g(g_), st(st_) {
        if (!g->profile) return;
        cudaEvent_t e0 = prof_event(g);
        e1 = prof_event(g);
        cudaEventRecord(e0, st);
        g->recs.push_back({name, e0, e1, bytes, flops});
    }
    ~ProfScope() {
        if (e1) cudaEventRecord(e1, st);
    }
};

double valid_rows_total(const svb_gen *g, int Tq) { return g->cur_frames * (double)(Tq / g->cur_T); }
std::vector<int> clip_rows(const svb_gen *g, int Tq) {
    std::vector<int> r(g->cur_len);
    for (int &v : r) v *= Tq / g->cur_T;
    return r;
}

int run_conv(svb_gen *g, const ConvLayer &L, const float *in, int in_Tp, float *out, int out_Tp, const float *res,
             int B, int Tq, float in_slope, float scale, int accumulate, cudaStream_t st, int max_ctas = 0) {
    const double rows = valid_rows_total(g, Tq);
    g->last_launches += 1;
    g->last_flops += 2.0 * L.macs_per_row * rows;
    const bool tc = g->cfg.precision != SVB_PREC_FP32 && L.tc.ok;
    const double rows_out = rows * (L.ups_u > 0 ? L.ups_u : 1);
    const double bytes = 4.0 * (rows * L.Cin + rows_out * L.Cout * (1 + (res ? 1 : 0) + (accumulate ? 1 : 0)));
    ProfScope ps(g, st, tc ? (L.ups_u ? "conv1d_c4_tc (upsampler)" : "conv1d_c4_tc (resblock)") : "conv1d_c4_ffma", bytes,
                 2.0 * L.macs_per_row * rows);
    ConvArgs a;
    a.in = in, a.w = L.w, a.bias = L.b, a.res = res, a.out = out;
    a.B = B, a.Cin = L.Cin, a.in_Tp = in_Tp, a.Cout = L.Cout, a.out_Tp = out_Tp, a.CoutP = L.CoutP, a.Tq = Tq;
    a.KS = L.KS, a.dil = L.dil, a.ups_u = L.ups_u, a.in_slope = in_slope, a.out_scale = scale, a.accumulate = accumulate;
    a.rows = g->cur_len_dev, a.rows_mul = Tq / g->cur_T;
    if (g->cfg.precision != SVB_PREC_FP32 && tc_supported(L.tc, a)) return launch_conv_tc(L.tc, a, g->cfg.precision, st, max_ctas);
    return launch_conv_ffma(a, st);
}

int run_conv_multi(svb_gen *g, int stage, int nk, const ConvLayer *const *Ls, const float *const *in, float *const *out,
                   const float *const *res, const float *scale, const int *accumulate, bool chain_ordered, int B, int Tq, int Tp,
                   float in_slope, cudaStream_t st) {
    ConvArgs a[kTcMaxLayers];
    const TcWeights *w[kTcMaxLayers];
    double bytes = 0, flops = 0;
    const double rows = valid_rows_total(g, Tq);
    for (int j = 0; j < nk; ++j) {
        const ConvLayer &L = *Ls[j];
        a[j].in = in[j], a[j].w = L.w, a[j].bias = L.b, a[j].res = res[j], a[j].out = out[j];
        a[j].B = B, a[j].Cin = L.Cin, a[j].in_Tp = Tp, a[j].Cout = L.Cout, a[j].out_Tp = Tp, a[j].CoutP = L.CoutP, a[j].Tq = Tq;
        a[j].KS = L.KS, a[j].dil = L.dil, a[j].ups_u = 0, a[j].in_slope = in_slope, a[j].out_scale = scale[j], a[j].accumulate = accumulate[j];
        a[j].rows = g->cur_len_dev, a[j].rows_mul = Tq / g->cur_T;
        w[j] = &L.tc;
        bytes += 4.0 * (rows * L.Cin + rows * L.Cout * (1 + (res[j] ? 1 : 0) + (accumulate[j] ? 1 : 0)));
        flops += 2.0 * L.macs_per_row * rows;
    }
    g->last_launches += 1;
    g->last_flops += flops;
    ProfScope ps(g, st, "conv1d_c4_tc (resblock)", bytes, flops);
    for (int attempt = 0; attempt < 2; ++attempt) {
        const int key = stage * 4 + (chain_ordered ? 2 : 0) + attempt;
        TcWorkList &wl = g->worklists[key];
        if (!wl.valid) {
            const std::vector<int> rh = clip_rows(g, Tq);
            SVB_TRY(tc_worklist_build(nk, w, a, g->cfg.precision, chain_ordered, &wl, rh.empty() ? nullptr : rh.data(), st));
        }
        const int rc = launch_conv_tc_multi(nk, w, a, g->cfg.precision, st, wl);
        if (rc != SVB_ERR_STATE) return rc;
    }
    set_error("merged launch: no cached work list matches the plan of stage %d", stage);
    return SVB_ERR_STATE;
}

int forward_impl(svb_gen *g, const float *mel, bool mel_frame_major, const float *f0, const float *rand_ini,
                 const float *noise, uint64_t seed, int B, int T, float *wav, cudaStream_t st, const int32_t *lens = nullptr,
                 bool packed = false) {
    SVB_CHECK(g && g->finalized, SVB_ERR_STATE, "generator: forward before finalize");
    SVB_CHECK(!g->dirty, SVB_ERR_STATE, "generator: weights were set after finalize; call svb_gen_update_weights first");
    SVB_CHECK(mel && wav && B > 0 && T > 0, SVB_ERR_INVALID, "generator: null buffer or empty batch (B %d T %d)", B, T);
    SVB_CHECK(!f0 || g->cfg.use_pitch_embed, SVB_ERR_INVALID, "generator: f0 given but use_pitch_embed is off");
    SVB_CHECK((rand_ini == nullptr) == (noise == nullptr), SVB_ERR_INVALID,
              "generator: rand_ini and noise must be given together");
    SVB_CHECK(!lens || !g->training, SVB_ERR_INVALID,
              "generator: a ragged batch is inference only (training takes clips of equal length)");
    SVB_CHECK(!packed || (lens && mel_frame_major && !noise), SVB_ERR_INVALID, "generator: bad packed-layout call");
    SVB_CUDA(cudaSetDevice(g->device));
    size_t need = 0;
    Buffers bf = plan_workspace(g, B, T, &need);
    if (need > g->ws_cap) {
        if (g->ws) SVB_CUDA(cudaFree(g->ws));
        g->ws = nullptr, g->ws_cap = 0;
        SVB_CUDA(cudaMalloc((void **)&g->ws, need));
        g->ws_cap = need, g->ws_B = 0;
    }
    std::vector<int> len;
    if (lens) len.assign(lens, lens + B);
    if (g->ws_B != B || g->ws_T != T || len != g->wl_len) {
        for (auto &kv : g->worklists) kv.second.valid = false;
        g->wl_len = len;
    }
    if (g->ws_B != B || g->ws_T != T || g->ws_training != g->training) {
        SVB_CUDA(cudaMemsetAsync(g->ws, 0, need, st));
        g->ws_B = B, g->ws_T = T, g->ws_training = g->training;
        g->hw.assign(B, 0);
    }
    g->cur_len = len, g->cur_len_dev = nullptr, g->cur_T = T, g->cur_frames = (double)B * T;
    Ragged rg;
    int stale_rows = 0;
    if (lens) {
        std::vector<int> tab(3 * (size_t)B + 1);
        double frames = 0;
        for (int b = 0; b < B; ++b) {
            tab[b] = len[b], tab[B + b] = g->hw[b], tab[2 * B + b] = (int)frames;
            stale_rows = std::max(stale_rows, g->hw[b] - len[b]);
            frames += len[b];
        }
        tab[3 * B] = (int)frames;
        if (tab.size() > g->rg_cap) {
            if (g->rg_dev) SVB_CUDA(cudaFree(g->rg_dev));
            g->rg_dev = nullptr, g->rg_cap = 0;
            SVB_CUDA(cudaMalloc((void **)&g->rg_dev, tab.size() * sizeof(int)));
            g->rg_cap = tab.size();
        }
        SVB_CUDA(cudaMemcpyAsync(g->rg_dev, tab.data(), tab.size() * sizeof(int), cudaMemcpyHostToDevice, st));
        g->cur_len_dev = g->rg_dev, g->cur_frames = frames;
        rg.len = g->rg_dev, rg.off = packed ? g->rg_dev + 2 * B : nullptr;
    }
    for (int b = 0; b < B; ++b) g->hw[b] = lens ? len[b] : T;
    g->bf = bf, g->last_T = T, g->last_nsf = f0 != nullptr;
    g->last_launches = 0, g->last_flops = 0, g->last_B = B;
    g->taps.clear();
    g->recs.clear(), g->ev_used = 0;
    if (g->timing) SVB_CUDA(cudaEventRecord(g->ev0, st));

    auto F = [&](size_t off) { return reinterpret_cast<float *>(g->ws + off); };
    const int n_mel = g->cfg.n_mel, C0 = g->cfg.upsample_initial_channel;
    const int Tp0 = c4t_rows(T);
    const double frames = g->cur_frames;
    if (stale_rows > 0) {
        std::vector<ZeroSeg> segs;
        segs.push_back({F(bf.pre), c4t_groups(C0), Tp0, 1});
        int mul = 1, max_rows = stale_rows;
        for (size_t i = 0; i < g->stages.size(); ++i) {
            const Stage &s = g->stages[i];
            mul *= s.u;
            const int Tip = c4t_rows(T * mul), gr = c4t_groups(s.C);
            std::vector<size_t> offs = {bf.X[i], bf.S[i]};
            for (auto &v : bf.A[i]) offs.insert(offs.end(), v.begin(), v.end());
            for (auto &v : bf.R[i]) offs.insert(offs.end(), v.begin(), v.end());
            std::sort(offs.begin(), offs.end());
            offs.erase(std::unique(offs.begin(), offs.end()), offs.end());
            for (size_t o : offs) segs.push_back({F(o), gr, Tip, mul});
            max_rows = std::max(max_rows, stale_rows * mul);
        }
        ProfScope ps(g, st, "zero stale rows", 0, 0);
        for (size_t i0 = 0; i0 < segs.size(); i0 += kMaxZeroSegs)
            SVB_TRY(launch_zero_tails(segs.data() + i0, (int)std::min<size_t>(kMaxZeroSegs, segs.size() - i0), B, g->rg_dev,
                                      g->rg_dev + B, max_rows, st));
        g->last_launches += (int64_t)((segs.size() + kMaxZeroSegs - 1) / kMaxZeroSegs);
    }
    {
        ProfScope ps(g, st, "mel layout", 8.0 * n_mel * frames, 0);
        if (mel_frame_major) SVB_TRY(launch_btc_to_c4t(mel, F(bf.mel), B, n_mel, T, Tp0, st, rg));
        else SVB_TRY(launch_nct_to_c4t(mel, F(bf.mel), B, n_mel, T, Tp0, st, rg));
    }
    g->last_launches += 1;

    const int Tw = T * g->hop;
    float *har = nullptr;
    bool har_on_side = false;
    if (f0) {
        har = F(bf.har);
        har_on_side = !g->profile;
        cudaStream_t ns = har_on_side ? g->side[0] : st;
        if (har_on_side) {
            SVB_CUDA(cudaEventRecord(g->ev_fork, st));
            SVB_CUDA(cudaStreamWaitEvent(ns, g->ev_fork, 0));
        }
        int l = 0;
        {
            const double samples = frames * g->hop;
            ProfScope ps(g, ns, "nsf source (4 kernels)", 4.0 * (frames + samples * (noise ? 10 : 1)), 60.0 * samples * 9);
            SVB_TRY(launch_nsf_source(f0, rand_ini, noise, seed, B, T, g->hop, (float)g->cfg.audio_sample_rate, g->lin_w,
                                      g->lin_b_dev, g->ws + bf.nsf, har, g->training ? F(bf.sines) : nullptr, ns, &l, rg.len, rg.off));
        }
        if (har_on_side) SVB_CUDA(cudaEventRecord(g->ev_chain[0], ns));
        g->last_launches += l;
        g->taps["har_source"] = Tap{har, 1, Tw, 0, true};
    }

    SVB_TRY(run_conv(g, g->conv_pre, F(bf.mel), Tp0, F(bf.pre), Tp0, nullptr, B, T, 1.f, 1.f, 0, st));
    g->taps["conv_pre"] = Tap{F(bf.pre), C0, T, Tp0, false};

    const float *x_in = F(bf.pre);
    int Tin = T, Tin_p = Tp0;
    const int nk = g->cfg.n_resblock_kernels, nd = g->cfg.n_dilations;
    for (size_t i = 0; i < g->stages.size(); ++i) {
        Stage &s = g->stages[i];
        const int Ti = Tin * s.u, Tip = c4t_rows(Ti);
        float *X = F(bf.X[i]), *S = F(bf.S[i]);
        SVB_TRY(run_conv(g, s.up, x_in, Tin_p, X, Tip, nullptr, B, Tin, 0.1f, 1.f, 0, st));
        if (f0) {
            if (har_on_side && i == 0) SVB_CUDA(cudaStreamWaitEvent(st, g->ev_chain[0], 0));
            const double rows = valid_rows_total(g, Ti);
            ProfScope ps(g, st, "noise_conv_add", 4.0 * (2.0 * rows * s.C + frames * g->hop), 2.0 * rows * s.C * s.noise.K);
            SVB_TRY(launch_noise_conv_add(X, B, s.C, Ti, Tip, har, Tw, s.noise.w, s.noise.b, s.noise.K, s.noise.stride,
                                          s.noise.pad, st, rg, Ti / T, g->hop));
            g->last_launches += 1;
            g->last_flops += 2.0 * rows * s.C * s.noise.K;
        }
        g->taps["ups" + std::to_string(i)] = Tap{X, s.C, Ti, Tip, false};
        const bool par = g->chains > 1 && nk > 1 && nk <= 3 && g->cfg.precision != SVB_PREC_FP32 && !g->profile;
        const int sms = 148;
        bool merged = g->merge && !par && nk > 1 && nk <= kTcMaxLayers && g->cfg.precision != SVB_PREC_FP32 &&
                      s.c1[0][0].tc.ok;
        if (merged) {
            const std::vector<int> rh = clip_rows(g, Ti);
            merged = tc_merge_fits(nk, B, Ti, s.C, s.c1[0][0].tc.n_tile, rh.empty() ? nullptr : rh.data());
        }
        for (int j = 0; merged && j < nk; ++j)
            for (int m = 0; m < nd; ++m) {
                ConvArgs probe;
                probe.Cin = s.C, probe.Cout = s.C, probe.CoutP = s.C, probe.KS = s.c1[j][m].KS, probe.dil = s.c1[j][m].dil, probe.ups_u = 0;
                probe.bias = s.c1[j][m].b, probe.cin_blk = 0;
                merged = merged && tc_supported(s.c1[j][m].tc, probe) && s.c1[j][m].tc.n_tile == s.c1[0][0].tc.n_tile;
                if (g->cfg.resblock == 1) merged = merged && s.c2[j][m].tc.ok && s.c2[j][m].tc.n_tile == s.c1[0][0].tc.n_tile;
            }
        if (merged) {
            for (int m = 0; m < nd; ++m) {
                const bool last = m == nd - 1;
                const ConvLayer *L1[kTcMaxLayers], *L2[kTcMaxLayers];
                const float *xin[kTcMaxLayers], *ain[kTcMaxLayers], *none[kTcMaxLayers];
                float *aout[kTcMaxLayers], *dst[kTcMaxLayers];
                float one[kTcMaxLayers], scl[kTcMaxLayers];
                int zero[kTcMaxLayers], acc[kTcMaxLayers];
                for (int j = 0; j < nk; ++j) {
                    L1[j] = &s.c1[j][m], none[j] = nullptr, one[j] = 1.f, zero[j] = 0;
                    scl[j] = last ? 1.f / nk : 1.f, acc[j] = (last && j > 0) ? 1 : 0;
                    if (g->cfg.resblock == 1) {
                        L2[j] = &s.c2[j][m];
                        xin[j] = m == 0 ? X : F(bf.R[i][j][m - 1]);
                        aout[j] = F(bf.A[i][j][m]), ain[j] = aout[j];
                        dst[j] = last ? S : F(bf.R[i][j][m]);
                    } else {
                        xin[j] = m == 0 ? X : (m % 2 ? F(bf.R[i][j][m - 1]) : F(bf.A[i][j][m - 1]));
                        dst[j] = last ? S : (m % 2 ? F(bf.A[i][j][m]) : F(bf.R[i][j][m]));
                    }
                }
                if (g->cfg.resblock == 1) {
                    SVB_TRY(run_conv_multi(g, (int)i, nk, L1, xin, aout, none, one, zero, false, B, Ti, Tip, 0.1f, st));
                    SVB_TRY(run_conv_multi(g, (int)i, nk, L2, ain, dst, xin, scl, acc, last, B, Ti, Tip, 0.1f, st));
                } else {
                    SVB_TRY(run_conv_multi(g, (int)i, nk, L1, xin, dst, xin, scl, acc, last, B, Ti, Tip, 0.1f, st));
                }
            }
        }
        if (par) SVB_CUDA(cudaEventRecord(g->ev_fork, st));
        for (int j = 0; j < nk && !merged; ++j) {
            cudaStream_t cs = par ? g->side[j] : st;
            int cap = 0;
            if (par) {
                double wsum = 0, wj = 0;
                for (int jj = 0; jj < nk; ++jj) {
                    const double wv = g->cfg.resblock_kernel_sizes[jj] + g->chain_bias;
                    wsum += wv;
                    if (jj == j) wj = wv;
                }
                cap = std::max(8, (int)(sms * wj / wsum + 0.5));
                if (g->chains == 2) cap = 0;
            }
            if (par) SVB_CUDA(cudaStreamWaitEvent(cs, g->ev_fork, 0));
            for (int m = 0; m < nd; ++m) {
                float *A = F(bf.A[i][j][m]);
                const float *xin = m == 0 ? X : F(bf.R[i][j][m - 1]);
                const bool last = m == nd - 1;
                float *dst = last ? S : F(bf.R[i][j][m]);
                const float scale = last ? 1.f / nk : 1.f;
                const int accum = (last && j > 0) ? 1 : 0;
                if (g->cfg.resblock == 1) {
                    SVB_TRY(run_conv(g, s.c1[j][m], xin, Tip, A, Tip, nullptr, B, Ti, 0.1f, 1.f, 0, cs, cap));
                    if (par && last && j > 0) SVB_CUDA(cudaStreamWaitEvent(cs, g->ev_chain[j - 1], 0));
                    SVB_TRY(run_conv(g, s.c2[j][m], A, Tip, dst, Tip, xin, B, Ti, 0.1f, scale, accum, cs, cap));
                } else {
                    const float *xin2 = m == 0 ? X : (m % 2 ? F(bf.R[i][j][m - 1]) : F(bf.A[i][j][m - 1]));
                    float *dst2 = last ? S : (m % 2 ? F(bf.A[i][j][m]) : F(bf.R[i][j][m]));
                    if (par && last && j > 0) SVB_CUDA(cudaStreamWaitEvent(cs, g->ev_chain[j - 1], 0));
                    SVB_TRY(run_conv(g, s.c1[j][m], xin2, Tip, dst2, Tip, xin2, B, Ti, 0.1f, scale, accum, cs, cap));
                }
            }
            if (par) SVB_CUDA(cudaEventRecord(g->ev_chain[j], cs));
        }
        if (par) SVB_CUDA(cudaStreamWaitEvent(st, g->ev_chain[nk - 1], 0));
        g->taps["stage" + std::to_string(i)] = Tap{S, s.C, Ti, Tip, false};
        x_in = S, Tin = Ti, Tin_p = Tip;
    }
    {
        const double rows = valid_rows_total(g, Tin);
        ProfScope ps(g, st, "conv_post_tanh", 4.0 * rows * (g->post_C + 1.0), 2.0 * rows * g->post_C * g->post_K);
        SVB_TRY(launch_conv_post_tanh(x_in, B, g->post_C, Tin, Tin_p, g->post_wq, g->post_b_dev, g->post_K, 0.01f, wav, st, rg,
                                      Tin / T));
    }
    g->last_launches += 1;
    g->last_flops += 2.0 * valid_rows_total(g, Tin) * g->post_C * g->post_K;
    if (g->training) SVB_CUDA(cudaMemcpyAsync(F(bf.wav), wav, (size_t)B * Tw * 4, cudaMemcpyDeviceToDevice, st));
    if (g->timing) SVB_CUDA(cudaEventRecord(g->ev1, st));
    return SVB_OK;
}

}

extern "C" int svb_gen_create(const svb_gen_config *cfg, int device, svb_gen_t **out) {
    SVB_CHECK(cfg && out, SVB_ERR_INVALID, "gen_create: null argument");
    SVB_CHECK(cfg->n_ups >= 1 && cfg->n_ups <= SVB_MAX_UPS, SVB_ERR_INVALID, "gen_create: n_ups %d out of range", cfg->n_ups);
    SVB_CHECK(cfg->n_resblock_kernels >= 1 && cfg->n_resblock_kernels <= SVB_MAX_RBK, SVB_ERR_INVALID,
              "gen_create: n_resblock_kernels %d out of range", cfg->n_resblock_kernels);
    SVB_CHECK(cfg->n_dilations >= 1 && cfg->n_dilations <= SVB_MAX_DIL, SVB_ERR_INVALID, "gen_create: n_dilations %d",
              cfg->n_dilations);
    SVB_CHECK(cfg->resblock == 1 || cfg->resblock == 2, SVB_ERR_INVALID, "gen_create: resblock must be 1 or 2");
    SVB_CHECK(cfg->n_mel > 0 && cfg->n_mel % 4 == 0, SVB_ERR_INVALID, "gen_create: n_mel %d must be a multiple of 4",
              cfg->n_mel);
    SVB_CHECK(cfg->precision >= 0 && cfg->precision <= 3, SVB_ERR_INVALID, "gen_create: bad precision %d", cfg->precision);
    const int cfin = cfg->upsample_initial_channel >> cfg->n_ups;
    SVB_CHECK(cfin >= 4 && (cfin << cfg->n_ups) == cfg->upsample_initial_channel && cfin % 4 == 0, SVB_ERR_INVALID,
              "gen_create: upsample_initial_channel %d must stay a multiple of 4 after %d halvings",
              cfg->upsample_initial_channel, cfg->n_ups);
    for (int j = 0; j < cfg->n_resblock_kernels; ++j) {
        const int k = cfg->resblock_kernel_sizes[j];
        SVB_CHECK(k % 2 == 1 && k >= 1 && k <= 11, SVB_ERR_INVALID, "gen_create: resblock kernel %d unsupported", k);
        for (int m = 0; m < cfg->n_dilations; ++m)
            SVB_CHECK((k - 1) / 2 * cfg->resblock_dilation_sizes[j][m] <= kPad && cfg->resblock_dilation_sizes[j][m] >= 1,
                      SVB_ERR_INVALID, "gen_create: kernel %d dilation %d exceeds the %d-row halo", k,
                      cfg->resblock_dilation_sizes[j][m], kPad);
    }
    int count = 0;
    SVB_CUDA(cudaGetDeviceCount(&count));
    SVB_CHECK(device >= 0 && device < count, SVB_ERR_INVALID, "gen_create: device %d of %d", device, count);
    SVB_CUDA(cudaSetDevice(device));
    svb_gen *g = new (std::nothrow) svb_gen();
    SVB_CHECK(g, SVB_ERR_NOMEM, "gen_create: out of host memory");
    g->cfg = *cfg, g->device = device;
    g->hop = 1;
    for (int i = 0; i < cfg->n_ups; ++i) g->hop *= cfg->upsample_rates[i];
    SVB_CUDA(cudaEventCreate(&g->ev0));
    SVB_CUDA(cudaEventCreate(&g->ev1));
    SVB_CUDA(cudaEventCreateWithFlags(&g->ev_fork, cudaEventDisableTiming));
    for (int i = 0; i < 3; ++i) {
        SVB_CUDA(cudaStreamCreateWithFlags(&g->side[i], cudaStreamNonBlocking));
        SVB_CUDA(cudaEventCreateWithFlags(&g->ev_chain[i], cudaEventDisableTiming));
    }
    if (const char *e = getenv("SVB_CHAINS")) g->chains = atoi(e);
    if (const char *e = getenv("SVB_MERGE")) g->merge = atoi(e) != 0;
    if (const char *e = getenv("SVB_CHAIN_BIAS")) g->chain_bias = atof(e);
    *out = g;
    return SVB_OK;
}

extern "C" void svb_gen_destroy(svb_gen_t *g) {
    if (!g) return;
    cudaSetDevice(g->device);
    for (void *p : g->dev_allocs) cudaFree(p);
    for (auto &kv : g->worklists) tc_worklist_free(&kv.second);
    if (g->ws) cudaFree(g->ws);
    if (g->rg_dev) cudaFree(g->rg_dev);
    if (g->bws) cudaFree(g->bws);
    for (void *p : g->job_allocs) cudaFree(p);
    for (auto &kv : g->nat_dev) cudaFree(kv.second.p);
    if (g->grad_flat) cudaFree(g->grad_flat);
    if (g->pin_in) cudaFreeHost(g->pin_in);
    if (g->pin_out) cudaFreeHost(g->pin_out);
    if (g->dev_in) cudaFree(g->dev_in);
    if (g->dev_out) cudaFree(g->dev_out);
    if (g->dev_i16) cudaFree(g->dev_i16);
    for (cudaEvent_t e : g->ev_pool) cudaEventDestroy(e);
    for (int i = 0; i < 3; ++i) {
        if (g->side[i]) cudaStreamDestroy(g->side[i]);
        if (g->ev_chain[i]) cudaEventDestroy(g->ev_chain[i]);
    }
    if (g->ev_fork) cudaEventDestroy(g->ev_fork);
    if (g->ev0) cudaEventDestroy(g->ev0);
    if (g->ev1) cudaEventDestroy(g->ev1);
    delete g;
}

extern "C" int svb_gen_set_weight(svb_gen_t *g, const char *name, const float *data, const int64_t *shape, int32_t ndim) {
    SVB_CHECK(g && name && data && shape && ndim >= 1 && ndim <= 4, SVB_ERR_INVALID, "set_weight: bad argument");
    SVB_CHECK(!g->finalized || g->training, SVB_ERR_STATE, "set_weight('%s') after finalize (only a training handle takes new weights)", name);
    if (g->finalized) g->dirty = true;
    HostTensor t;
    size_t n = 1;
    for (int i = 0; i < ndim; ++i) {
        SVB_CHECK(shape[i] > 0, SVB_ERR_INVALID, "set_weight('%s'): non-positive dim", name);
        t.shape.push_back(shape[i]);
        n *= (size_t)shape[i];
    }
    t.data.assign(data, data + n);
    g->host_w[name] = std::move(t);
    return SVB_OK;
}

int svb::gen_build_layers(svb_gen *g) {
    SVB_CUDA(cudaSetDevice(g->device));
    for (void *p : g->dev_allocs) cudaFree(p);
    g->dev_allocs.clear();
    g->stages.clear();
    g->conv_pre = ConvLayer();
    const svb_gen_config &c = g->cfg;
    const int C0 = c.upsample_initial_channel;
    SVB_TRY(pack_conv(g, "conv_pre", c.n_mel, C0, 7, 1, &g->conv_pre));
    int cin = C0;
    g->stages.resize(c.n_ups);
    for (int i = 0; i < c.n_ups; ++i) {
        Stage &s = g->stages[i];
        const int u = c.upsample_rates[i], k = c.upsample_kernel_sizes[i];
        s.C = cin / 2, s.u = u;
        SVB_CHECK(k >= u && (k - u) % 2 == 0, SVB_ERR_INVALID, "upsampler %d: kernel %d / rate %d unsupported", i, k, u);
        SVB_TRY(pack_convT(g, "ups." + std::to_string(i), cin, s.C, k, u, (k - u) / 2, &s.up));
        if (c.use_pitch_embed) {
            int stride = 1;
            for (int r = i + 1; r < c.n_ups; ++r) stride *= c.upsample_rates[r];
            const bool last = i + 1 == c.n_ups;
            s.noise.C = s.C, s.noise.K = last ? 1 : 2 * stride, s.noise.stride = last ? 1 : stride;
            s.noise.pad = last ? 0 : stride / 2;
            const HostTensor *w, *b;
            SVB_TRY(gen_get_w(g, "noise_convs." + std::to_string(i) + ".weight", {s.C, 1, s.noise.K}, &w));
            SVB_TRY(gen_get_w(g, "noise_convs." + std::to_string(i) + ".bias", {s.C}, &b));
            std::vector<float> wt((size_t)s.noise.K * s.C);
            for (int ch = 0; ch < s.C; ++ch)
                for (int j = 0; j < s.noise.K; ++j) wt[(size_t)j * s.C + ch] = w->data[(size_t)ch * s.noise.K + j];
            SVB_TRY(gen_upload(g, wt, &s.noise.w));
            SVB_TRY(gen_upload(g, b->data, &s.noise.b));
        }
        s.c1.resize(c.n_resblock_kernels), s.c2.resize(c.n_resblock_kernels);
        for (int j = 0; j < c.n_resblock_kernels; ++j) {
            const int n = i * c.n_resblock_kernels + j, rk = c.resblock_kernel_sizes[j];
            s.c1[j].resize(c.n_dilations), s.c2[j].resize(c.n_dilations);
            for (int m = 0; m < c.n_dilations; ++m) {
                const int d = c.resblock_dilation_sizes[j][m];
                const std::string base = "resblocks." + std::to_string(n);
                if (c.resblock == 1) {
                    SVB_TRY(pack_conv(g, base + ".convs1." + std::to_string(m), s.C, s.C, rk, d, &s.c1[j][m]));
                    SVB_TRY(pack_conv(g, base + ".convs2." + std::to_string(m), s.C, s.C, rk, 1, &s.c2[j][m]));
                } else {
                    SVB_TRY(pack_conv(g, base + ".convs." + std::to_string(m), s.C, s.C, rk, d, &s.c1[j][m]));
                }
            }
        }
        cin = s.C;
    }
    {
        const HostTensor *w, *b;
        SVB_TRY(gen_get_w(g, "conv_post.weight", {1, cin, 7}, &w));
        SVB_TRY(gen_get_w(g, "conv_post.bias", {1}, &b));
        std::vector<float> p((size_t)cin * 7);
        for (int cq = 0; cq < cin / 4; ++cq)
            for (int k = 0; k < 7; ++k)
                for (int e = 0; e < 4; ++e) p[((size_t)cq * 7 + k) * 4 + e] = w->data[(size_t)(cq * 4 + e) * 7 + k];
        SVB_TRY(gen_upload(g, p, &g->post_wq));
        SVB_TRY(gen_upload(g, b->data, &g->post_b_dev));
        g->post_K = 7, g->post_C = cin;
    }
    if (c.use_pitch_embed) {
        const HostTensor *w, *b;
        SVB_TRY(gen_get_w(g, "m_source.l_linear.weight", {1, 9}, &w));
        SVB_TRY(gen_get_w(g, "m_source.l_linear.bias", {1}, &b));
        SVB_TRY(gen_upload(g, w->data, &g->lin_w));
        SVB_TRY(gen_upload(g, b->data, &g->lin_b_dev));
    }
    return SVB_OK;
}

extern "C" int svb_gen_finalize(svb_gen_t *g) {
    SVB_CHECK(g, SVB_ERR_INVALID, "finalize: null handle");
    SVB_CHECK(!g->finalized, SVB_ERR_STATE, "finalize called twice");
    SVB_TRY(gen_build_layers(g));
    g->finalized = true;
    return SVB_OK;
}

extern "C" int svb_gen_set_precision(svb_gen_t *g, int32_t precision) {
    SVB_CHECK(g && precision >= 0 && precision <= 3, SVB_ERR_INVALID, "set_precision: bad argument");
    g->cfg.precision = precision;
    return SVB_OK;
}

extern "C" int svb_gen_forward(svb_gen_t *g, const float *mel_dev, const float *f0_dev, const float *rand_ini_dev,
                               const float *noise_dev, uint64_t seed, int32_t B, int32_t T, float *wav_dev, void *stream) {
    return forward_impl(g, mel_dev, false, f0_dev, rand_ini_dev, noise_dev, seed, B, T, wav_dev, as_stream(stream));
}

namespace {
int check_lengths(const char *what, const int32_t *lens, int B, int T_max) {
    SVB_CHECK(lens, SVB_ERR_INVALID, "%s: lengths is NULL", what);
    SVB_CHECK(B > 0, SVB_ERR_INVALID, "%s: empty batch (B %d)", what, B);
    long long frames = 0;
    for (int b = 0; b < B; ++b) {
        SVB_CHECK(lens[b] >= 1 && (T_max <= 0 || lens[b] <= T_max), SVB_ERR_INVALID,
                  "%s: length %d of clip %d is outside [1, T_max %d]", what, lens[b], b, T_max);
        frames += lens[b];
    }
    SVB_CHECK(frames < (1ll << 31) / 4096, SVB_ERR_INVALID, "%s: %lld frames in one batch", what, frames);
    return SVB_OK;
}
}

extern "C" int svb_gen_forward_ragged(svb_gen_t *g, const float *mel_dev, const float *f0_dev, const int32_t *lengths_host,
                                      const float *rand_ini_dev, const float *noise_dev, uint64_t seed, int32_t B, int32_t T_max,
                                      float *wav_dev, void *stream) {
    SVB_CHECK(T_max > 0, SVB_ERR_INVALID, "gen_forward_ragged: T_max %d", T_max);
    SVB_TRY(check_lengths("gen_forward_ragged", lengths_host, B, T_max));
    SVB_CHECK(g, SVB_ERR_INVALID, "gen_forward_ragged: null handle");
    return forward_impl(g, mel_dev, false, f0_dev, rand_ini_dev, noise_dev, seed, B, T_max, wav_dev, as_stream(stream), lengths_host);
}

extern "C" int svb_gen_spec2wav_host(svb_gen_t *g, const float *mel_host, const float *f0_host, uint64_t seed, int32_t B,
                                     int32_t T, float *wav_host, void *stream) {
    SVB_CHECK(g && g->finalized, SVB_ERR_STATE, "spec2wav: generator not finalized");
    SVB_CHECK(mel_host && wav_host && B > 0 && T > 0, SVB_ERR_INVALID, "spec2wav: null buffer or empty input");
    SVB_CUDA(cudaSetDevice(g->device));
    cudaStream_t st = as_stream(stream);
    const size_t n_mel = (size_t)B * T * g->cfg.n_mel, n_f0 = f0_host ? (size_t)B * T : 0;
    const size_t n_in = n_mel + n_f0, n_out = (size_t)B * T * g->hop;
    if (n_in > g->pin_in_cap) {
        if (g->pin_in) cudaFreeHost(g->pin_in);
        if (g->dev_in) cudaFree(g->dev_in);
        g->pin_in = nullptr, g->dev_in = nullptr, g->pin_in_cap = 0;
        SVB_CUDA(cudaMallocHost((void **)&g->pin_in, n_in * 4));
        SVB_CUDA(cudaMalloc((void **)&g->dev_in, n_in * 4));
        g->pin_in_cap = n_in;
    }
    if (n_out > g->pin_out_cap) {
        if (g->pin_out) cudaFreeHost(g->pin_out);
        if (g->dev_out) cudaFree(g->dev_out);
        g->pin_out = nullptr, g->dev_out = nullptr, g->pin_out_cap = 0;
        SVB_CUDA(cudaMallocHost((void **)&g->pin_out, n_out * 4));
        SVB_CUDA(cudaMalloc((void **)&g->dev_out, n_out * 4));
        g->pin_out_cap = n_out;
    }
    memcpy(g->pin_in, mel_host, n_mel * 4);
    if (f0_host) memcpy(g->pin_in + n_mel, f0_host, n_f0 * 4);
    SVB_CUDA(cudaMemcpyAsync(g->dev_in, g->pin_in, n_in * 4, cudaMemcpyHostToDevice, st));
    SVB_TRY(forward_impl(g, g->dev_in, true, f0_host ? g->dev_in + n_mel : nullptr, nullptr, nullptr, seed, B, T,
                         g->dev_out, st));
    SVB_CUDA(cudaMemcpyAsync(g->pin_out, g->dev_out, n_out * 4, cudaMemcpyDeviceToHost, st));
    SVB_CUDA(cudaStreamSynchronize(st));
    memcpy(wav_host, g->pin_out, n_out * 4);
    return SVB_OK;
}

namespace {
__global__ void clip_absmax_kernel(const float *__restrict__ x, long long n, unsigned *__restrict__ mx, const int *__restrict__ off, int hop) {
    const int b = blockIdx.y;
    const size_t base = off ? (size_t)off[b] * hop : (size_t)b * n;
    if (off) n = (long long)(off[b + 1] - off[b]) * hop;
    float m = 0.f;
    for (long long i = (long long)blockIdx.x * blockDim.x + threadIdx.x; i < n; i += (long long)gridDim.x * blockDim.x)
        m = fmaxf(m, fabsf(x[base + i]));
#pragma unroll
    for (int o = 16; o > 0; o >>= 1) m = fmaxf(m, __shfl_xor_sync(0xffffffffu, m, o));
    if ((threadIdx.x & 31) == 0) atomicMax(mx + b, __float_as_uint(m));
}
__global__ void to_int16_kernel(const float *__restrict__ x, long long n, const unsigned *__restrict__ mx, int16_t *__restrict__ y,
                                const int *__restrict__ off, int hop) {
    const int b = blockIdx.y;
    const size_t base = off ? (size_t)off[b] * hop : (size_t)b * n;
    if (off) n = (long long)(off[b + 1] - off[b]) * hop;
    for (long long i = (long long)blockIdx.x * blockDim.x + threadIdx.x; i < n; i += (long long)gridDim.x * blockDim.x) {
        float v = x[base + i];
        if (mx) v = __fdiv_rn(v, __uint_as_float(mx[b]));
        v = __fmul_rn(v, 32767.f);
        y[base + i] = (int16_t)__float2int_rz(v);
    }
}
int wav_to_int16(const float *wav_dev, int B, long long n, int norm, int16_t *out_dev, unsigned *mx_dev, cudaStream_t st,
                 const int *off = nullptr, int hop = 1) {
    const dim3 grid((unsigned)std::min<long long>((n + 255) / 256, 148 * 4), (unsigned)B);
    if (norm) {
        SVB_CUDA(cudaMemsetAsync(mx_dev, 0, (size_t)B * sizeof(unsigned), st));
        clip_absmax_kernel<<<grid, 256, 0, st>>>(wav_dev, n, mx_dev, off, hop);
    }
    to_int16_kernel<<<grid, 256, 0, st>>>(wav_dev, n, norm ? mx_dev : nullptr, out_dev, off, hop);
    SVB_CUDA(cudaGetLastError());
    return SVB_OK;
}
}

extern "C" int svb_wav_to_int16(const float *wav_dev, int32_t B, int64_t n, int32_t norm, int16_t *out_dev, void *stream) {
    SVB_CHECK(wav_dev && out_dev && B > 0 && n > 0, SVB_ERR_INVALID, "wav_to_int16: bad argument");
    cudaStream_t st = as_stream(stream);
    unsigned *mx = nullptr;
    if (norm) SVB_CUDA(cudaMallocAsync((void **)&mx, (size_t)B * sizeof(unsigned), st));
    const int rc = wav_to_int16(wav_dev, B, n, norm, out_dev, mx, st);
    if (mx) cudaFreeAsync(mx, st);
    return rc;
}

extern "C" int svb_gen_spec2wav_host_i16(svb_gen_t *g, const float *mel_host, const float *f0_host, uint64_t seed, int32_t B,
                                         int32_t T, int32_t norm, int16_t *wav_host, void *stream) {
    SVB_CHECK(g && g->finalized, SVB_ERR_STATE, "spec2wav_i16: generator not finalized");
    SVB_CHECK(mel_host && wav_host && B > 0 && T > 0, SVB_ERR_INVALID, "spec2wav_i16: null buffer or empty input");
    SVB_CUDA(cudaSetDevice(g->device));
    cudaStream_t st = as_stream(stream);
    const size_t n_mel = (size_t)B * T * g->cfg.n_mel, n_f0 = f0_host ? (size_t)B * T : 0;
    const size_t n_in = n_mel + n_f0, n_out = (size_t)B * T * g->hop;
    if (n_in > g->pin_in_cap) {
        if (g->pin_in) cudaFreeHost(g->pin_in);
        if (g->dev_in) cudaFree(g->dev_in);
        g->pin_in = nullptr, g->dev_in = nullptr, g->pin_in_cap = 0;
        SVB_CUDA(cudaMallocHost((void **)&g->pin_in, n_in * 4));
        SVB_CUDA(cudaMalloc((void **)&g->dev_in, n_in * 4));
        g->pin_in_cap = n_in;
    }
    if (n_out > g->pin_out_cap) {
        if (g->pin_out) cudaFreeHost(g->pin_out);
        if (g->dev_out) cudaFree(g->dev_out);
        g->pin_out = nullptr, g->dev_out = nullptr, g->pin_out_cap = 0;
        SVB_CUDA(cudaMallocHost((void **)&g->pin_out, n_out * 4));
        SVB_CUDA(cudaMalloc((void **)&g->dev_out, n_out * 4));
        g->pin_out_cap = n_out;
    }
    if (n_out > g->i16_cap) {
        if (g->dev_i16) cudaFree(g->dev_i16);
        g->dev_i16 = nullptr, g->i16_cap = 0;
        SVB_CUDA(cudaMalloc((void **)&g->dev_i16, n_out * 2 + (size_t)4096 * sizeof(unsigned)));
        g->i16_cap = n_out;
    }
    SVB_CHECK(B <= 4096, SVB_ERR_INVALID, "spec2wav_i16: batch %d > 4096", B);
    memcpy(g->pin_in, mel_host, n_mel * 4);
    if (f0_host) memcpy(g->pin_in + n_mel, f0_host, n_f0 * 4);
    SVB_CUDA(cudaMemcpyAsync(g->dev_in, g->pin_in, n_in * 4, cudaMemcpyHostToDevice, st));
    SVB_TRY(forward_impl(g, g->dev_in, true, f0_host ? g->dev_in + n_mel : nullptr, nullptr, nullptr, seed, B, T, g->dev_out, st));
    unsigned *mx;
    mx = reinterpret_cast<unsigned *>(reinterpret_cast<char *>(g->dev_i16) + (g->i16_cap * 2 + 3) / 4 * 4);
    SVB_TRY(wav_to_int16(g->dev_out, B, (long long)T * g->hop, norm, g->dev_i16, mx, st));
    SVB_CUDA(cudaMemcpyAsync(g->pin_out, g->dev_i16, n_out * 2, cudaMemcpyDeviceToHost, st));
    SVB_CUDA(cudaStreamSynchronize(st));
    memcpy(wav_host, g->pin_out, n_out * 2);
    return SVB_OK;
}

namespace {
int spec2wav_ragged(svb_gen_t *g, const char *what, const float *mel_host, const float *f0_host, const int32_t *lens, int B,
                    uint64_t seed, bool i16, int norm, void *wav_host, void *stream) {
    SVB_CHECK(mel_host && wav_host, SVB_ERR_INVALID, "%s: null buffer", what);
    SVB_TRY(check_lengths(what, lens, B, 0));
    SVB_CHECK(g && g->finalized, SVB_ERR_STATE, "%s: generator not finalized", what);
    SVB_CHECK(!i16 || B <= 4096, SVB_ERR_INVALID, "%s: batch %d > 4096", what, B);
    int T_max = 0;
    size_t frames = 0;
    for (int b = 0; b < B; ++b) T_max = std::max(T_max, (int)lens[b]), frames += lens[b];
    SVB_CUDA(cudaSetDevice(g->device));
    cudaStream_t st = as_stream(stream);
    const size_t n_mel = frames * g->cfg.n_mel, n_f0 = f0_host ? frames : 0;
    const size_t n_in = n_mel + n_f0, n_out = frames * g->hop;
    if (n_in > g->pin_in_cap) {
        if (g->pin_in) cudaFreeHost(g->pin_in);
        if (g->dev_in) cudaFree(g->dev_in);
        g->pin_in = nullptr, g->dev_in = nullptr, g->pin_in_cap = 0;
        SVB_CUDA(cudaMallocHost((void **)&g->pin_in, n_in * 4));
        SVB_CUDA(cudaMalloc((void **)&g->dev_in, n_in * 4));
        g->pin_in_cap = n_in;
    }
    if (n_out > g->pin_out_cap) {
        if (g->pin_out) cudaFreeHost(g->pin_out);
        if (g->dev_out) cudaFree(g->dev_out);
        g->pin_out = nullptr, g->dev_out = nullptr, g->pin_out_cap = 0;
        SVB_CUDA(cudaMallocHost((void **)&g->pin_out, n_out * 4));
        SVB_CUDA(cudaMalloc((void **)&g->dev_out, n_out * 4));
        g->pin_out_cap = n_out;
    }
    if (i16 && n_out > g->i16_cap) {
        if (g->dev_i16) cudaFree(g->dev_i16);
        g->dev_i16 = nullptr, g->i16_cap = 0;
        SVB_CUDA(cudaMalloc((void **)&g->dev_i16, n_out * 2 + (size_t)4096 * sizeof(unsigned)));
        g->i16_cap = n_out;
    }
    memcpy(g->pin_in, mel_host, n_mel * 4);
    if (f0_host) memcpy(g->pin_in + n_mel, f0_host, n_f0 * 4);
    SVB_CUDA(cudaMemcpyAsync(g->dev_in, g->pin_in, n_in * 4, cudaMemcpyHostToDevice, st));
    SVB_TRY(forward_impl(g, g->dev_in, true, f0_host ? g->dev_in + n_mel : nullptr, nullptr, nullptr, seed, B, T_max, g->dev_out, st,
                         lens, true));
    if (i16) {
        unsigned *mx = reinterpret_cast<unsigned *>(reinterpret_cast<char *>(g->dev_i16) + (g->i16_cap * 2 + 3) / 4 * 4);
        SVB_TRY(wav_to_int16(g->dev_out, B, (long long)T_max * g->hop, norm, g->dev_i16, mx, st, g->rg_dev + 2 * B, g->hop));
        SVB_CUDA(cudaMemcpyAsync(g->pin_out, g->dev_i16, n_out * 2, cudaMemcpyDeviceToHost, st));
    } else {
        SVB_CUDA(cudaMemcpyAsync(g->pin_out, g->dev_out, n_out * 4, cudaMemcpyDeviceToHost, st));
    }
    SVB_CUDA(cudaStreamSynchronize(st));
    memcpy(wav_host, g->pin_out, n_out * (i16 ? 2 : 4));
    return SVB_OK;
}
}

extern "C" int svb_gen_spec2wav_ragged_host(svb_gen_t *g, const float *mel_host, const float *f0_host, const int32_t *lengths_host,
                                            int32_t B, uint64_t seed, float *wav_host, void *stream) {
    return spec2wav_ragged(g, "spec2wav_ragged", mel_host, f0_host, lengths_host, B, seed, false, 0, wav_host, stream);
}

extern "C" int svb_gen_spec2wav_ragged_host_i16(svb_gen_t *g, const float *mel_host, const float *f0_host, const int32_t *lengths_host,
                                                int32_t B, uint64_t seed, int32_t norm, int16_t *wav_host, void *stream) {
    return spec2wav_ragged(g, "spec2wav_ragged_i16", mel_host, f0_host, lengths_host, B, seed, true, norm, wav_host, stream);
}

extern "C" int svb_gen_get_tap(svb_gen_t *g, const char *name, float *out_dev, int64_t capacity_floats, int64_t *shape3,
                               void *stream) {
    SVB_CHECK(g && name && out_dev && shape3, SVB_ERR_INVALID, "get_tap: null argument");
    auto it = g->taps.find(name);
    SVB_CHECK(it != g->taps.end(), SVB_ERR_INVALID, "get_tap: no activation named '%s' in the last forward", name);
    const Tap &t = it->second;
    const int B = g->last_B;
    shape3[0] = B, shape3[1] = t.C, shape3[2] = t.T;
    SVB_CHECK((int64_t)B * t.C * t.T <= capacity_floats, SVB_ERR_INVALID, "get_tap: buffer too small");
    cudaStream_t st = as_stream(stream);
    if (t.plain) SVB_CUDA(cudaMemcpyAsync(out_dev, t.p, (size_t)B * t.T * 4, cudaMemcpyDeviceToDevice, st));
    else SVB_TRY(launch_c4t_to_nct(t.p, out_dev, B, t.C, t.T, t.Tp, st));
    return SVB_OK;
}

extern "C" int64_t svb_gen_hop(const svb_gen_t *g) { return g ? g->hop : 0; }
extern "C" int64_t svb_gen_last_launches(const svb_gen_t *g) { return g ? g->last_launches : 0; }
extern "C" double svb_gen_last_flops(const svb_gen_t *g) { return g ? g->last_flops : 0.0; }
extern "C" int svb_gen_enable_timing(svb_gen_t *g, int32_t on) {
    SVB_CHECK(g, SVB_ERR_INVALID, "enable_timing: null handle");
    g->timing = on != 0;
    g->profile = on == 2;
    return SVB_OK;
}
extern "C" int32_t svb_gen_profile_count(svb_gen_t *g) { return g ? (int32_t)g->recs.size() : 0; }
extern "C" int svb_gen_profile_get(svb_gen_t *g, int32_t i, char *name, int32_t name_cap, float *ms, double *bytes,
                                   double *flops) {
    SVB_CHECK(g && i >= 0 && i < (int32_t)g->recs.size() && name && ms && bytes && flops && name_cap > 0, SVB_ERR_INVALID,
              "profile_get: bad argument");
    const auto &r = g->recs[i];
    SVB_CUDA(cudaEventSynchronize(r.e1));
    SVB_CUDA(cudaEventElapsedTime(ms, r.e0, r.e1));
    snprintf(name, name_cap, "%s", r.name);
    *bytes = r.bytes, *flops = r.flops;
    return SVB_OK;
}
extern "C" float svb_gen_last_ms(svb_gen_t *g) {
    if (!g || !g->timing) return -1.f;
    float ms = -1.f;
    if (cudaEventSynchronize(g->ev1) != cudaSuccess) return -1.f;
    if (cudaEventElapsedTime(&ms, g->ev0, g->ev1) != cudaSuccess) return -1.f;
    return ms;
}
```

neuralsvb_b200/csrc/generator.cuh:

```cuda
#pragma once
#include <map>
#include <string>
#include <vector>

#include "conv_ffma.cuh"
#include "conv_tc.cuh"
#include "nsf_source.cuh"

namespace svb {

struct HostTensor {
    std::vector<int64_t> shape;
    std::vector<float> data;
};

struct ConvLayer {
    float *w = nullptr;
    float *b = nullptr;
    TcWeights tc;
    int Cin = 0, Cout = 0, CoutP = 0, KS = 1, dil = 1, ups_u = 0;
    double macs_per_row = 0;
};

struct NoiseConv {
    float *w = nullptr, *b = nullptr;
    int C = 0, K = 1, stride = 1, pad = 0;
};

struct Stage {
    int C = 0;
    int u = 1;
    ConvLayer up;
    NoiseConv noise;
    std::vector<std::vector<ConvLayer>> c1, c2;
};

struct Tap {
    const float *p = nullptr;
    int C = 0, T = 0, Tp = 0;
    bool plain = false;
};

struct Buffers {
    size_t mel = 0, pre = 0, har = 0, nsf = 0, sines = 0, wav = 0;
    std::vector<size_t> X, S;
    std::vector<std::vector<std::vector<size_t>>> A, R;
};

struct BwdStage {
    std::vector<std::vector<ConvLayer>> d1, d2;
    float *up_wt = nullptr;
};

struct PackJob {
    std::string src;
    float *dst = nullptr;
    int *idx = nullptr;
    size_t n = 0;
    const TcWeights *tc = nullptr;
};

struct GradBuf {
    float *p = nullptr;
    size_t n = 0;
};
}

struct svb_gen {
    svb_gen_config cfg{};
    int device = 0;
    bool finalized = false;
    std::map<std::string, svb::HostTensor> host_w;
    std::vector<void *> dev_allocs;

    svb::ConvLayer conv_pre;
    std::vector<svb::Stage> stages;
    float *post_wq = nullptr;
    int post_K = 7, post_C = 0;
    float *lin_w = nullptr;
    float *lin_b_dev = nullptr;
    int hop = 1;

    char *ws = nullptr;
    size_t ws_cap = 0;
    int ws_B = 0, ws_T = 0;
    std::map<std::string, svb::Tap> taps;
    int last_B = 0, last_T = 0;
    bool last_nsf = false;
    svb::Buffers bf;

    bool training = false, ws_training = false, dirty = false;
    bool bwd_built = false;
    std::vector<svb::BwdStage> bwd;
    float *zero_bias = nullptr;
    float *post_w_nat = nullptr;
    float *post_b_dev = nullptr;
    float *grad_flat = nullptr;
    size_t grad_floats = 0;
    std::map<std::string, svb::GradBuf> grads;
    char *bws = nullptr;
    size_t bws_cap = 0;
    int bws_B = 0, bws_T = 0;
    int64_t bwd_launches = 0;
    std::map<std::string, svb::GradBuf> nat_dev;
    std::vector<svb::PackJob> jobs;
    std::vector<void *> job_allocs;
    bool dev_dirty = false;

    float *pin_in = nullptr, *pin_out = nullptr, *dev_in = nullptr, *dev_out = nullptr;
    size_t pin_in_cap = 0, pin_out_cap = 0;
    int16_t *dev_i16 = nullptr;
    size_t i16_cap = 0;

    int64_t last_launches = 0;
    double last_flops = 0;
    bool timing = false;
    cudaEvent_t ev0 = nullptr, ev1 = nullptr;

    struct LaunchRec {
        const char *name;
        cudaEvent_t e0, e1;
        double bytes, flops;
    };
    cudaStream_t side[3] = {nullptr, nullptr, nullptr};
    cudaEvent_t ev_fork = nullptr, ev_chain[3] = {nullptr, nullptr, nullptr};
    int chains = 1;
    double chain_bias = 4.0;

    bool merge = true;
    std::map<int, svb::TcWorkList> worklists;
    std::vector<int> wl_len;

    std::vector<int> hw;
    int *rg_dev = nullptr;
    size_t rg_cap = 0;
    std::vector<int> cur_len;
    const int *cur_len_dev = nullptr;
    double cur_frames = 0;
    int cur_T = 1;

    bool profile = false;
    std::vector<LaunchRec> recs;
    std::vector<cudaEvent_t> ev_pool;
    size_t ev_used = 0;
};


namespace svb {
int gen_upload(svb_gen *g, const std::vector<float> &h, float **out);
int gen_get_w(svb_gen *g, const std::string &name, std::vector<int64_t> want, const HostTensor **out);
int gen_build_layers(svb_gen *g);
int gen_build_bwd_layers(svb_gen *g);
}
```

Measured before the change: 5219.

## Fuse resblock conv1/conv2 pairs into a single tcgen05 kernel keeping intermediates in smem

Adds a pair kernel that computes each resblock's dilated conv1 and following conv2 back to back inside one CTA. The conv1 output is staged in shared memory as bf16x3 split operands for conv2, with halo rows recomputed, so the intermediate activation never round-trips through global memory. It comes with its own work-item scheduler, weight residency and a probe API. It is enabled by default for C=32 stages in inference, which are the late high-rate stages. The cost is more kernel complexity and redundant halo compute per tile.

```diff
diff --git a/include/svb_vocoder.h b/include/svb_vocoder.h
--- a/include/svb_vocoder.h
+++ b/include/svb_vocoder.h
@@ -214,6 +214,9 @@
                                      int32_t Cin, int32_t B, const int32_t *rows_per_clip, int32_t MT, int32_t col_blocks,
                                      int32_t chain_ordered, int32_t grid, int32_t *items_out, int64_t items_capacity,
                                      int32_t *off_out, double *balance_out);
+int64_t svb_tc_pair_schedule_probe(int32_t n_chains, const int32_t *KS1, const int32_t *KS2, int32_t C, int32_t B, int32_t Tq,
+                                   const int32_t *rows_per_clip, int32_t chain_ordered, int32_t grid, int32_t *items_out,
+                                   int64_t items_capacity, int32_t *off_out, double *balance_out);
 
 #ifdef __cplusplus
 }
diff --git a/neuralsvb_b200/_native.py b/neuralsvb_b200/_native.py
--- a/neuralsvb_b200/_native.py
+++ b/neuralsvb_b200/_native.py
@@ -152,6 +152,7 @@
     'svb_tc_schedule_probe': (_I64, [_I32, _P, _P, _P, _I32, _I32, _I32, _I32, _I32, _I32, _I32, _P, _I64, _P, ctypes.POINTER(ctypes.c_double)]),
     'svb_tc_schedule_probe_ragged': (_I64, [_I32, _P, _P, _P, _I32, _I32, _P, _I32, _I32, _I32, _I32, _P, _I64, _P,
                                             ctypes.POINTER(ctypes.c_double)]),
+    'svb_tc_pair_schedule_probe': (_I64, [_I32, _P, _P, _I32, _I32, _I32, _P, _I32, _I32, _P, _I64, _P, ctypes.POINTER(ctypes.c_double)]),
     'svb_gen_forward_ragged': (ctypes.c_int, [_P, _P, _P, _P, _P, _P, _U64, _I32, _I32, _P, _P]),
     'svb_gen_spec2wav_ragged_host': (ctypes.c_int, [_P, _P, _P, _P, _I32, _U64, _P, _P]),
     'svb_gen_spec2wav_ragged_host_i16': (ctypes.c_int, [_P, _P, _P, _P, _I32, _U64, _I32, _P, _P]),
diff --git a/neuralsvb_b200/csrc/conv_tc.cu b/neuralsvb_b200/csrc/conv_tc.cu
--- a/neuralsvb_b200/csrc/conv_tc.cu
+++ b/neuralsvb_b200/csrc/conv_tc.cu
@@ -82,6 +82,68 @@
     TcItem it;
     it.layer = v.x & 0xff, it.nblk = (v.x >> 8) & 0xffff, it.mt = v.x >> 24, it.b = v.y, it.t0 = v.z, it.rows = v.w;
     return it;
+}
+
+template <bool BF, bool X3>
+__device__ __forceinline__ void transform_slab(uint4 *op, int R, float slope, int tid, int cl, bool odd, uint32_t op_bytes) {
+    for (int r0 = 0; r0 < R; r0 += 64) {
+        int rr[2];
+        bool ok[2];
+        float4 v[2];
+#pragma unroll
+        for (int u = 0; u < 2; ++u) {
+            rr[u] = r0 + 32 * u + (tid >> 3);
+            ok[u] = rr[u] < R;
+            v[u] = make_float4(0.f, 0.f, 0.f, 0.f);
+            if (ok[u]) v[u] = *reinterpret_cast<const float4 *>(op + (size_t)rr[u] * 8 + cl);
+        }
+#pragma unroll
+        for (int u = 0; u < 2; ++u) {
+            float4 &x = v[u];
+            x.x = fmaxf(x.x, x.x * slope), x.y = fmaxf(x.y, x.y * slope);
+            x.z = fmaxf(x.z, x.z * slope), x.w = fmaxf(x.w, x.w * slope);
+        }
+        if (BF) {
+            uint32_t h0[2], h1[2], l0[2], l1[2], g0[2], g1[2];
+#pragma unroll
+            for (int u = 0; u < 2; ++u) {
+                const __nv_bfloat162 hA = __floats2bfloat162_rn(v[u].x, v[u].y), hB = __floats2bfloat162_rn(v[u].z, v[u].w);
+                h0[u] = *reinterpret_cast<const uint32_t *>(&hA), h1[u] = *reinterpret_cast<const uint32_t *>(&hB);
+                const __nv_bfloat162 lA = __floats2bfloat162_rn(v[u].x - __uint_as_float(h0[u] << 16),
+                                                               v[u].y - __uint_as_float(h0[u] & 0xffff0000u));
+                const __nv_bfloat162 lB = __floats2bfloat162_rn(v[u].z - __uint_as_float(h1[u] << 16),
+                                                               v[u].w - __uint_as_float(h1[u] & 0xffff0000u));
+                l0[u] = *reinterpret_cast<const uint32_t *>(&lA), l1[u] = *reinterpret_cast<const uint32_t *>(&lB);
+            }
+#pragma unroll
+            for (int u = 0; u < 2; ++u) {
+                g0[u] = __shfl_xor_sync(0xffffffffu, odd ? h0[u] : l0[u], 1);
+                g1[u] = __shfl_xor_sync(0xffffffffu, odd ? h1[u] : l1[u], 1);
+            }
+#pragma unroll
+            for (int u = 0; u < 2; ++u) {
+                if (!ok[u]) continue;
+                uint4 *row = op + (size_t)rr[u] * 8;
+                const int sw = rr[u] & 7;
+                if (!odd) row[(cl >> 1) ^ sw] = make_uint4(h0[u], h1[u], g0[u], g1[u]);
+                else row[(4 + (cl >> 1)) ^ sw] = make_uint4(g0[u], g1[u], l0[u], l1[u]);
+            }
+        } else {
+            __syncwarp();
+#pragma unroll
+            for (int u = 0; u < 2; ++u) {
+                if (!ok[u]) continue;
+                uint4 *row = op + (size_t)rr[u] * 8;
+                const int sw = rr[u] & 7;
+                const float4 h = make_float4(to_tf32(v[u].x), to_tf32(v[u].y), to_tf32(v[u].z), to_tf32(v[u].w));
+                row[cl ^ sw] = make_uint4(__float_as_uint(h.x), __float_as_uint(h.y), __float_as_uint(h.z), __float_as_uint(h.w));
+                if (X3)
+                    (row + op_bytes / 32)[cl ^ sw] =
+                        make_uint4(__float_as_uint(to_tf32(v[u].x - h.x)), __float_as_uint(to_tf32(v[u].y - h.y)),
+                                   __float_as_uint(to_tf32(v[u].z - h.z)), __float_as_uint(to_tf32(v[u].w - h.w)));
+            }
+        }
+    }
 }
 
 template <int MODE, bool ST = false, bool RG = false>
@@ -981,6 +1043,610 @@
     return tc_dispatch(p, precision, wl.grid, smem, st);
 }
 
+
+constexpr int kPairSets = 4;
+constexpr int kPairMaxB = 3;
+
+struct PairChain {
+    const float *x;
+    float *out;
+    const float *b1, *b2;
+    const unsigned char *w1, *w2;
+    int KS1, dil1, KS2;
+    float out_scale;
+    int accumulate;
+    int bias1_off, bias2_off;
+};
+
+struct PairArgs {
+    ConvArgs a;
+    PairChain L[kTcMaxLayers];
+    int n_chains;
+    const int4 *work;
+    const int *work_off;
+    int n_tile, n_chunks, nA, nB, nW, tmem_cols;
+    int w_resident;
+    int pdl;
+    long long *stats;
+    uint32_t op_bytes, c2_plane, wtile_bytes;
+    uint32_t off_op, off_c2, off_w, off_stage, off_bias;
+};
+
+__device__ __forceinline__ void pair_step(int s, int L, bool &c2, int &i) {
+    if (s < 2) c2 = false, i = s;
+    else if (s == 2 * L) c2 = true, i = L - 1;
+    else if (s & 1) c2 = true, i = (s - 3) >> 1;
+    else c2 = false, i = (s >> 1) + 1;
+}
+__device__ __forceinline__ int pair_c1_rows(int i, int L, int h1, int h2) { return i < L ? kTcM + 2 * h1 : 2 * h2 + 2 * h1; }
+
+template <bool ST>
+__global__ void __launch_bounds__(kTcThreadsP, 1) conv1d_pair_tc_kernel(const __grid_constant__ PairArgs p) {
+    extern __shared__ __align__(1024) unsigned char smem[];
+    const ConvArgs &a = p.a;
+    uint64_t *bars = reinterpret_cast<uint64_t *>(smem);
+    uint64_t *raw_full = bars, *a_ready = bars + 4, *a_empty = bars + 8;
+    uint64_t *w_full = bars + 12, *w_empty = bars + 12 + kMaxW;
+    uint64_t *acc_full = bars + 12 + 2 * kMaxW, *acc_empty = acc_full + kPairSets;
+    uint64_t *c2_full = acc_empty + kPairSets, *c2_empty = c2_full + kPairMaxB;
+    uint32_t *tmem_ptr = reinterpret_cast<uint32_t *>(c2_empty + kPairMaxB);
+    int *n_items_s = reinterpret_cast<int *>(tmem_ptr + 1);
+    PairChain *Ls = reinterpret_cast<PairChain *>(smem + 512);
+    const int4 *items = reinterpret_cast<const int4 *>(smem + 1024);
+    unsigned char *op0 = smem + p.off_op;
+    unsigned char *c2b = smem + p.off_c2;
+    unsigned char *wring = smem + p.off_w;
+
+    const int warp = threadIdx.x >> 5, lane = threadIdx.x & 31;
+    long long st_w0 = 0, st_w1 = 0, st_w2 = 0, st_w3 = 0;
+    const long long st_t0 = ST ? clock64() : 0;
+    unsigned long long st_g0 = 0;
+    if (ST) asm volatile("mov.u64 %0, %%globaltimer;" : "=l"(st_g0));
+
+    if (threadIdx.x == 0) {
+        for (int i = 0; i < 4; ++i) mbar_init(raw_full + i, 1), mbar_init(a_ready + i, 8), mbar_init(a_empty + i, 1);
+        for (int i = 0; i < kPairSets; ++i) mbar_init(acc_full + i, 1), mbar_init(acc_empty + i, 8);
+        for (int i = 0; i < kMaxW; ++i) mbar_init(w_full + i, 1), mbar_init(w_empty + i, 1);
+        for (int i = 0; i < kPairMaxB; ++i) mbar_init(c2_full + i, 16), mbar_init(c2_empty + i, 1);
+        fence_barrier_init();
+    }
+    if (warp == kWarpMma) tmem_alloc(tmem_ptr, p.tmem_cols);
+    {
+        float *sb = reinterpret_cast<float *>(smem + p.off_bias);
+        for (int l = 0; l < p.n_chains; ++l)
+            for (int i = threadIdx.x; i < a.Cout; i += kTcThreadsP)
+                sb[p.L[l].bias1_off + i] = __ldg(p.L[l].b1 + i), sb[p.L[l].bias2_off + i] = __ldg(p.L[l].b2 + i);
+        if (threadIdx.x < p.n_chains) Ls[threadIdx.x] = p.L[threadIdx.x];
+        int4 *it_w = reinterpret_cast<int4 *>(smem + 1024);
+        const int i0 = __ldg(p.work_off + blockIdx.x), n = __ldg(p.work_off + blockIdx.x + 1) - i0;
+        for (int i = threadIdx.x; i < n; i += kTcThreadsP) it_w[i] = __ldg(p.work + i0 + i);
+        if (threadIdx.x == 0) *n_items_s = n;
+    }
+    tc_fence_before();
+    __syncthreads();
+    tc_fence_after();
+    const uint32_t tmem_base = *tmem_ptr;
+    const int n_items = *n_items_s;
+    if (p.pdl) {
+        asm volatile("griddepcontrol.wait;" ::: "memory");
+        asm volatile("griddepcontrol.launch_dependents;" ::: "memory");
+    }
+
+    if (warp == kWarpProducer) {
+        if (lane == 0) {
+            const int gin = c4t_groups(a.Cin);
+            const size_t group_stride = (size_t)a.in_Tp * 32;
+            int sA = 0, phA = 1, sW = 0, phW = 1, loaded = -1, reloads = 0;
+            for (int n = 0; n < n_items; ++n) {
+                const int4 v = items[n];
+                const int j = v.x & 0xff, L = v.x >> 8;
+                const PairChain &C = Ls[j];
+                const int h1 = (C.KS1 - 1) / 2 * C.dil1, h2 = (C.KS2 - 1) / 2;
+                if (p.w_resident && j != loaded) {
+                    if (reloads > 0) mbar_wait_t<ST>(w_empty, (reloads - 1) & 1, st_w1);
+                    mbar_expect_tx(w_full, (uint32_t)(C.KS1 + C.KS2) * p.wtile_bytes);
+                    bulk_g2s(wring, C.w1, (uint32_t)C.KS1 * p.wtile_bytes, w_full);
+                    bulk_g2s(wring + (size_t)C.KS1 * p.wtile_bytes, C.w2, (uint32_t)C.KS2 * p.wtile_bytes, w_full);
+                    loaded = j, ++reloads;
+                }
+                const float *x_b = C.x + ((size_t)v.y * gin * a.in_Tp + kPad) * 32;
+                for (int s = 0; s <= 2 * L; ++s) {
+                    bool c2;
+                    int i;
+                    pair_step(s, L, c2, i);
+                    const unsigned char *w_k = c2 ? C.w2 : C.w1;
+                    const int KS = c2 ? C.KS2 : C.KS1;
+                    const float *in_c = x_b + (ptrdiff_t)(v.z - h2 + kTcM * i - h1) * 32;
+                    const uint32_t raw_bytes = (uint32_t)pair_c1_rows(i, L, h1, h2) * 128;
+                    for (int c = 0; c < p.n_chunks; ++c) {
+                        if (!c2) {
+                            mbar_wait_t<ST>(a_empty + sA, phA, st_w0);
+                            mbar_expect_tx(raw_full + sA, raw_bytes);
+                            bulk_g2s(op0 + sA * p.op_bytes, in_c, raw_bytes, raw_full + sA);
+                            in_c += group_stride;
+                            if (++sA == p.nA) sA = 0, phA ^= 1;
+                        }
+                        if (!p.w_resident) {
+                            for (int k = 0; k < KS; ++k) {
+                                mbar_wait_t<ST>(w_empty + sW, phW, st_w1);
+                                mbar_expect_tx(w_full + sW, p.wtile_bytes);
+                                bulk_g2s(wring + sW * p.wtile_bytes, w_k, p.wtile_bytes, w_full + sW);
+                                w_k += p.wtile_bytes;
+                                if (++sW == p.nW) sW = 0, phW ^= 1;
+                            }
+                        }
+                    }
+                }
+            }
+            if (ST) {
+                long long *o = p.stats + (size_t)blockIdx.x * kTcStatSlots;
+                o[0] = st_w0, o[1] = st_w1, o[2] = clock64() - st_t0;
+            }
+        }
+    } else if (warp == kWarpMma) {
+        const uint32_t elected = elect_one_sync();
+        const uint32_t idesc = umma_idesc(1, kTcM, p.n_tile);
+        const uint32_t hi_word = desc_hi_sw128(0);
+        const uint32_t lo_plane = 64u >> 4;
+        const uint32_t op_base = desc_lo(smem_u32(op0)), c2_base = desc_lo(smem_u32(c2b)), w_base = desc_lo(smem_u32(wring));
+        const uint32_t op_step = p.op_bytes >> 4, plane_step = p.c2_plane >> 4, wtile_step = p.wtile_bytes >> 4;
+        int sA = 0, phA = 0, sW = 0, phW = 0, as = 0, phE = 1, sB = 0, phB = 0, loaded = -1, reloads = 0;
+        const int n_items_u = __reduce_max_sync(0xffffffffu, n_items);
+        for (int n = 0; n < n_items_u; ++n) {
+            const int ix = __reduce_max_sync(0xffffffffu, items[n].x);
+            const int j = ix & 0xff, L = ix >> 8;
+            const int KS1 = p.L[j].KS1, KS2 = p.L[j].KS2;
+            const uint32_t tap1 = (uint32_t)p.L[j].dil1 * (128 >> 4);
+            if (p.w_resident && j != loaded) {
+                if (reloads > 0) umma_commit(w_empty, elected);
+                mbar_wait_warp<ST>(w_full, reloads & 1, st_w2);
+                tc_fence_after();
+                loaded = j, ++reloads;
+            }
+            for (int s = 0; s <= 2 * L; ++s) {
+                bool c2;
+                int i;
+                pair_step(s, L, c2, i);
+                mbar_wait_warp<ST>(acc_empty + as, phE, st_w0);
+                tc_fence_after();
+                if (c2) {
+                    mbar_wait_warp<ST>(c2_full + sB, phB, st_w3);
+                    tc_fence_after();
+                }
+                const uint32_t d = tmem_base + (uint32_t)(as * p.n_tile);
+                const int KS = c2 ? KS2 : KS1;
+                const uint32_t tap_step = c2 ? (128u >> 4) : tap1;
+                uint32_t fresh = 1;
+                for (int c = 0; c < p.n_chunks; ++c) {
+                    uint32_t a_tap;
+                    if (!c2) {
+                        mbar_wait_warp<ST>(a_ready + sA, phA, st_w1);
+                        tc_fence_after();
+                        a_tap = op_base + sA * op_step;
+                    } else {
+                        a_tap = c2_base + (uint32_t)(sB * p.n_chunks + c) * plane_step;
+                    }
+                    uint32_t b_tap = w_base + (c2 ? (uint32_t)KS1 * wtile_step : 0u);
+                    for (int k = 0; k < KS; ++k) {
+                        if (!p.w_resident) {
+                            mbar_wait_warp<ST>(w_full + sW, phW, st_w2);
+                            tc_fence_after();
+                            b_tap = w_base + sW * wtile_step;
+                        }
+                        const uint32_t acc = fresh ^ 1u;
+                        umma<true>(d, a_tap + lo_plane, hi_word, b_tap, hi_word, idesc, acc, elected);
+                        umma<true, 1>(d, a_tap, hi_word, b_tap + lo_plane, hi_word, idesc, 1u, elected);
+                        umma<true, 2>(d, a_tap, hi_word, b_tap, hi_word, idesc, 1u, elected);
+                        umma<true>(d, a_tap + lo_plane + 2, hi_word, b_tap + 2, hi_word, idesc, 1u, elected);
+                        umma<true, 1>(d, a_tap + 2, hi_word, b_tap + lo_plane + 2, hi_word, idesc, 1u, elected);
+                        umma<true, 2>(d, a_tap + 2, hi_word, b_tap + 2, hi_word, idesc, 1u, elected);
+                        fresh = 0;
+                        a_tap += tap_step, b_tap += wtile_step;
+                        if (!p.w_resident) {
+                            umma_commit(w_empty + sW, elected);
+                            if (++sW == p.nW) sW = 0, phW ^= 1;
+                        }
+                    }
+                    if (!c2) {
+                        umma_commit(a_empty + sA, elected);
+                        if (++sA == p.nA) sA = 0, phA ^= 1;
+                    }
+                }
+                if (c2) {
+                    umma_commit(c2_empty + sB, elected);
+                    if (++sB == p.nB) sB = 0, phB ^= 1;
+                }
+                umma_commit(acc_full + as, elected);
+                if (++as == kPairSets) as = 0, phE ^= 1;
+            }
+        }
+        if (ST && elected) {
+            long long *o = p.stats + (size_t)blockIdx.x * kTcStatSlots;
+            o[3] = st_w0, o[4] = st_w1, o[5] = st_w2, o[6] = clock64() - st_t0, o[14] = st_w3;
+        }
+    } else if (warp >= kWarpTransform0) {
+        const int tid = threadIdx.x - kWarpTransform0 * 32;
+        const int cl = tid & 7;
+        const bool odd = cl & 1;
+        int sA = 0, phA = 0;
+        for (int n = 0; n < n_items; ++n) {
+            const int4 v = items[n];
+            const int L = v.x >> 8;
+            const PairChain &C = Ls[v.x & 0xff];
+            const int h1 = (C.KS1 - 1) / 2 * C.dil1, h2 = (C.KS2 - 1) / 2;
+            for (int i = 0; i <= L; ++i) {
+                const int R = pair_c1_rows(i, L, h1, h2);
+                for (int c = 0; c < p.n_chunks; ++c) {
+                    mbar_wait_t<ST>(raw_full + sA, phA, st_w0);
+                    transform_slab<true, false>(reinterpret_cast<uint4 *>(op0 + sA * p.op_bytes), R, a.in_slope, tid, cl, odd, p.op_bytes);
+                    fence_proxy_async();
+                    __syncwarp();
+                    if (lane == 0) mbar_arrive(a_ready + sA);
+                    if (++sA == p.nA) sA = 0, phA ^= 1;
+                }
+            }
+        }
+        if (ST && tid == 0) {
+            long long *o = p.stats + (size_t)blockIdx.x * kTcStatSlots;
+            o[7] = st_w0, o[8] = clock64() - st_t0;
+        }
+    } else {
+        const int lane_base = 32 * (warp & 3), half = warp >> 2;
+        const int gout = c4t_groups(a.Cout);
+        float4 *tile = reinterpret_cast<float4 *>(smem + p.off_stage + warp * 4096);
+        const float *sbias = reinterpret_cast<const float *>(smem + p.off_bias);
+        const int jb = p.n_tile / 32;
+        const int wr = lane >> 3, wc = lane & 7;
+        const int row = lane_base + lane;
+        const float slope = a.in_slope;
+        int as = 0, phF = 0, hs = -1, phH = 1;
+        for (int n = 0; n < n_items; ++n) {
+            const int4 v = items[n];
+            const int L = v.x >> 8, b = v.y, t0 = v.z, rows = v.w;
+            const PairChain &C = Ls[v.x & 0xff];
+            const int h2 = (C.KS2 - 1) / 2;
+            for (int s = 0; s <= 2 * L; ++s) {
+                bool c2;
+                int i;
+                pair_step(s, L, c2, i);
+                if (!c2) {
+                    const int ts = hs;
+                    if (i < L) {
+                        if (++hs == p.nB) hs = 0, phH ^= 1;
+                        mbar_wait_t<ST>(c2_empty + hs, phH, st_w1);
+                    }
+                    mbar_wait_t<ST>(acc_full + as, phF, st_w0);
+                    tc_fence_after();
+                    const int t = t0 - h2 + kTcM * i + row;
+                    const bool valid = t >= 0 && t < rows;
+                    const bool head = i < L, tail = i > 0 && row < 2 * h2;
+#pragma unroll 1
+                    for (int q = 0; q < jb; ++q) {
+                        const int col = half * (p.n_tile / 2) + 16 * q;
+                        float vv[16];
+                        tmem_ld16(tmem_base + ((uint32_t)lane_base << 16) + (uint32_t)(as * p.n_tile + col), vv);
+                        const float *bs = sbias + C.bias1_off + col;
+                        uint32_t hi[8], lo[8];
+#pragma unroll
+                        for (int u = 0; u < 8; ++u) {
+                            float x0 = vv[2 * u] + bs[2 * u], x1 = vv[2 * u + 1] + bs[2 * u + 1];
+                            x0 = fmaxf(x0, x0 * slope), x1 = fmaxf(x1, x1 * slope);
+                            bf16_split2(x0, x1, hi[u], lo[u]);
+                            if (!valid) hi[u] = 0u, lo[u] = 0u;
+                        }
+                        const int pl = col >> 5, c8 = (col & 31) >> 3;
+                        auto put = [&](int slot, int r) {
+                            uint4 *rw = reinterpret_cast<uint4 *>(c2b + (size_t)(slot * p.n_chunks + pl) * p.c2_plane + (size_t)r * 128);
+                            const int sw = r & 7;
+                            rw[c8 ^ sw] = make_uint4(hi[0], hi[1], hi[2], hi[3]);
+                            rw[(c8 + 1) ^ sw] = make_uint4(hi[4], hi[5], hi[6], hi[7]);
+                            rw[(4 + c8) ^ sw] = make_uint4(lo[0], lo[1], lo[2], lo[3]);
+                            rw[(5 + c8) ^ sw] = make_uint4(lo[4], lo[5], lo[6], lo[7]);
+                        };
+                        if (head) put(hs, row);
+                        if (tail) put(ts, kTcM + row);
+                    }
+                    fence_proxy_async();
+                    tc_fence_before();
+                    __syncwarp();
+                    if (lane == 0) {
+                        mbar_arrive(acc_empty + as);
+                        if (head) mbar_arrive(c2_full + hs);
+                        if (i > 0) mbar_arrive(c2_full + ts);
+                    }
+                } else {
+                    const int blk = jb == 1 ? (half == (i & 1) ? 0 : -1) : half;
+                    const int q_base = t0 + kTcM * i + lane_base;
+                    const size_t base = (((size_t)b * gout + (blk < 0 ? 0 : blk)) * a.out_Tp + kPad + q_base) * 8;
+                    if (blk >= 0) {
+                        const float4 *res4 = reinterpret_cast<const float4 *>(C.x);
+#pragma unroll
+                        for (int i8 = 0; i8 < 8; ++i8) {
+                            const int rr = 4 * i8 + wr;
+                            tile[rr * 8 + (wc ^ (rr & 7))] =
+                                q_base + rr < rows ? __ldg(res4 + base + (size_t)rr * 8 + wc) : make_float4(0.f, 0.f, 0.f, 0.f);
+                        }
+                        __syncwarp();
+                    }
+                    mbar_wait_t<ST>(acc_full + as, phF, st_w0);
+                    tc_fence_after();
+                    if (blk >= 0) {
+                        const float out_scale = C.out_scale;
+                        const float *bs = sbias + C.bias2_off + blk * 32;
+#pragma unroll
+                        for (int hq = 0; hq < 2; ++hq) {
+                            float vv[16];
+                            tmem_ld16(tmem_base + ((uint32_t)lane_base << 16) + (uint32_t)(as * p.n_tile + blk * 32 + hq * 16), vv);
+#pragma unroll
+                            for (int g4 = 0; g4 < 4; ++g4) {
+                                const int gq = hq * 4 + g4;
+                                const float4 bv = *reinterpret_cast<const float4 *>(bs + 4 * gq);
+                                float4 o = make_float4(vv[4 * g4] + bv.x, vv[4 * g4 + 1] + bv.y, vv[4 * g4 + 2] + bv.z, vv[4 * g4 + 3] + bv.w);
+                                float4 *slot = tile + lane * 8 + (gq ^ (lane & 7));
+                                const float4 rv = *slot;
+                                o.x += rv.x, o.y += rv.y, o.z += rv.z, o.w += rv.w;
+                                o.x *= out_scale, o.y *= out_scale, o.z *= out_scale, o.w *= out_scale;
+                                *slot = o;
+                            }
+                        }
+                        __syncwarp();
+                        float4 *out4 = reinterpret_cast<float4 *>(C.out);
+#pragma unroll
+                        for (int i8 = 0; i8 < 8; ++i8) {
+                            const int rr = 4 * i8 + wr;
+                            if (q_base + rr >= rows) continue;
+                            float4 o = tile[rr * 8 + (wc ^ (rr & 7))];
+                            float4 *dst = out4 + base + (size_t)rr * 8 + wc;
+                            if (C.accumulate) {
+                                const float4 old = *dst;
+                                o.x += old.x, o.y += old.y, o.z += old.z, o.w += old.w;
+                            }
+                            *dst = o;
+                        }
+                        __syncwarp();
+                    }
+                    tc_fence_before();
+                    __syncwarp();
+                    if (lane == 0) mbar_arrive(acc_empty + as);
+                }
+                if (++as == kPairSets) as = 0, phF ^= 1;
+            }
+        }
+        if (ST && threadIdx.x == 0) {
+            long long *o = p.stats + (size_t)blockIdx.x * kTcStatSlots;
+            o[9] = st_w0, o[10] = clock64() - st_t0, o[15] = st_w1;
+        }
+    }
+    tc_fence_before();
+    __syncthreads();
+    if (ST && threadIdx.x == 0) {
+        unsigned long long g1;
+        asm volatile("mov.u64 %0, %%globaltimer;" : "=l"(g1));
+        p.stats[(size_t)blockIdx.x * kTcStatSlots + 11] = clock64() - st_t0;
+        p.stats[(size_t)blockIdx.x * kTcStatSlots + 12] = (long long)st_g0;
+        p.stats[(size_t)blockIdx.x * kTcStatSlots + 13] = (long long)g1;
+    }
+    if (warp == kWarpMma) {
+        tc_fence_after();
+        tmem_dealloc(tmem_base, p.tmem_cols);
+    }
+}
+
+bool tc_pair_supported(int C, int precision, const TcWeights &w1, const TcWeights &w2, int KS1, int dil1, int KS2, int dil2) {
+    return precision == SVB_PREC_BF16X3 && (C == 32 || C == 64) && w1.ok && w2.ok && w1.n_tile == C && w2.n_tile == C &&
+           w1.Cin == C && w2.Cin == C && w1.CoutP == C && w2.CoutP == C && w1.KS == KS1 && w2.KS == KS2 && dil2 == 1 && KS2 >= 3 &&
+           (KS1 - 1) / 2 * dil1 + (KS2 - 1) / 2 <= kPad;
+}
+
+static int tc_pair_plan(int n, const TcPairChain *ch, const ConvArgs &a, int precision, PairArgs &p, size_t &smem) {
+    SVB_CHECK(n >= 1 && n <= kTcMaxLayers, SVB_ERR_INVALID, "tc pair: %d chains in one launch", n);
+    SVB_CHECK(a.Cin == a.Cout && a.CoutP == a.Cout && a.in_Tp == a.out_Tp && a.ups_u == 0, SVB_ERR_INVALID, "tc pair: bad shape class");
+    for (int l = 0; l < n; ++l)
+        SVB_CHECK(tc_pair_supported(a.Cout, precision, *ch[l].w1, *ch[l].w2, ch[l].KS1, ch[l].dil1, ch[l].KS2, 1), SVB_ERR_INVALID,
+                  "tc pair: chain %d (C %d, k %d, d %d, precision %d) has no pair kernel", l, a.Cout, ch[l].KS1, ch[l].dil1, precision);
+    p.a = a, p.n_chains = n, p.work = nullptr, p.work_off = nullptr, p.stats = nullptr;
+    p.n_tile = a.Cout, p.n_chunks = a.Cout / kTcCK;
+    p.wtile_bytes = (uint32_t)p.n_tile * 128;
+    p.pdl = 1;
+    if (const char *e = getenv("SVB_TC_PDL")) p.pdl = atoi(e) != 0;
+    int h1 = 0, h2 = 0, ks_pair = 0;
+    for (int l = 0; l < n; ++l)
+        h1 = std::max(h1, (ch[l].KS1 - 1) / 2 * ch[l].dil1), h2 = std::max(h2, (ch[l].KS2 - 1) / 2), ks_pair = std::max(ks_pair, ch[l].KS1 + ch[l].KS2);
+    p.op_bytes = (uint32_t)round_up(kTcM + 2 * h1, 8) * 128;
+    p.c2_plane = (uint32_t)round_up(kTcM + 2 * h2, 8) * 128;
+    const size_t bias_bytes = (size_t)round_up(2 * n * a.Cout * 4, 1024);
+    const size_t limit = 227 * 1024, fixed = 1024 + kItemBytes, tail = kStageBytes + bias_bytes;
+    p.w_resident = p.n_chunks == 1;
+    const size_t res_bytes = (size_t)ks_pair * p.wtile_bytes;
+    bool planned = false;
+    for (int min_w : {4, 2}) {
+        for (int nB : {3, 2}) {
+            for (int nA : {3, 2}) {
+                const size_t used = fixed + (size_t)nA * p.op_bytes + (size_t)nB * p.n_chunks * p.c2_plane + tail;
+                if (used > limit) continue;
+                if (p.w_resident) {
+                    if (used + round_up((int)res_bytes, 1024) > limit) continue;
+                    p.nW = 1;
+                } else {
+                    p.nW = (int)std::min<size_t>(kMaxW, (limit - used) / p.wtile_bytes);
+                    if (p.nW < min_w) continue;
+                }
+                p.nA = nA, p.nB = nB, planned = true;
+                break;
+            }
+            if (planned) break;
+        }
+        if (planned) break;
+    }
+    SVB_CHECK(planned, SVB_ERR_INVALID, "tc pair: no shared-memory plan fits (C %d, halo %d / %d)", a.Cout, h1, h2);
+    p.off_op = 1024 + kItemBytes;
+    p.off_c2 = p.off_op + (uint32_t)p.nA * p.op_bytes;
+    p.off_w = p.off_c2 + (uint32_t)(p.nB * p.n_chunks) * p.c2_plane;
+    const size_t w_area = p.w_resident ? res_bytes : (size_t)p.nW * p.wtile_bytes;
+    p.off_stage = p.off_w + (uint32_t)round_up((int)w_area, 1024);
+    p.off_bias = p.off_stage + kStageBytes;
+    smem = (size_t)p.off_bias + bias_bytes;
+    SVB_CHECK(smem <= limit, SVB_ERR_INVALID, "tc pair: %zu bytes of shared memory", smem);
+    for (int l = 0; l < n; ++l) {
+        PairChain &L = p.L[l];
+        L.x = ch[l].x, L.out = ch[l].out, L.b1 = ch[l].b1, L.b2 = ch[l].b2;
+        L.w1 = reinterpret_cast<const unsigned char *>(ch[l].w1->blob[precision]);
+        L.w2 = reinterpret_cast<const unsigned char *>(ch[l].w2->blob[precision]);
+        L.KS1 = ch[l].KS1, L.dil1 = ch[l].dil1, L.KS2 = ch[l].KS2, L.out_scale = ch[l].out_scale, L.accumulate = ch[l].accumulate;
+        L.bias1_off = 2 * l * a.Cout, L.bias2_off = (2 * l + 1) * a.Cout;
+    }
+    for (int l = n; l < kTcMaxLayers; ++l) p.L[l] = p.L[0];
+    int cols = 32;
+    while (cols < kPairSets * p.n_tile) cols <<= 1;
+    p.tmem_cols = cols;
+    if (getenv("SVB_TC_VERBOSE"))
+        fprintf(stderr, "[tc] pair: %d chain(s) C %d halo %d + %d Tq %d | nA %d nB %d nW %d resident %d smem %zu\n", n, a.Cout, h1, h2, a.Tq, p.nA,
+                p.nB, p.nW, p.w_resident, smem);
+    return SVB_OK;
+}
+
+int tc_pair_schedule(int n, const int *KS1, const int *KS2, int C, int B, int Tq, bool chain_ordered, int grid, std::vector<int4> *items_out,
+                     std::vector<int> *off_out, double *balance_out, const int *rows) {
+    const double beta = 160.0 / std::max(32, C);
+    double wj[kTcMaxLayers], w_all = 0;
+    for (int j = 0; j < n; ++j) wj[j] = KS1[j] + KS2[j] + 2 * beta + 1.0, w_all += wj[j];
+    struct Seg {
+        int j, b, tiles;
+        double w;
+    };
+    std::vector<Seg> segs;
+    for (int j = 0; j < (chain_ordered ? 1 : n); ++j)
+        for (int b = 0; b < B; ++b) {
+            const int tiles = ((rows ? rows[b] : Tq) + kTcM - 1) / kTcM;
+            if (tiles > 0) segs.push_back({chain_ordered ? -1 : j, b, tiles, chain_ordered ? w_all : wj[j]});
+        }
+    double total = 0;
+    for (const Seg &g : segs) total += g.tiles * g.w;
+    const double target = total / grid;
+    std::vector<int4> &items = *items_out;
+    std::vector<int> &off = *off_out;
+    items.clear();
+    off.assign(grid + 1, 0);
+    std::vector<double> load(grid, 0.0);
+    int c = 0;
+    double cum = 0;
+    for (const Seg &g : segs) {
+        int t = 0;
+        while (t < g.tiles) {
+            int take = g.tiles - t;
+            if (c < grid - 1) take = std::min(take, (int)std::lround(((c + 1) * target - cum) / g.w));
+            if (take <= 0) {
+                ++c;
+                continue;
+            }
+            const int r = rows ? rows[g.b] : Tq;
+            for (int j = (g.j < 0 ? 0 : g.j); j < (g.j < 0 ? n : g.j + 1); ++j) {
+                SVB_CHECK(take < (1 << 23), SVB_ERR_INVALID, "tc pair: %d tiles in one item", take);
+                items.push_back(make_int4(j | (take << 8), g.b, t * kTcM, r));
+            }
+            load[c] += take * g.w;
+            cum += take * g.w, t += take;
+            off[c + 1] = (int)items.size();
+            if (c < grid - 1 && cum >= (c + 1) * target - 0.5 * g.w) ++c;
+        }
+    }
+    for (int k = 1; k <= grid; ++k) off[k] = std::max(off[k], off[k - 1]);
+    for (int k = 0; k < grid; ++k)
+        SVB_CHECK(off[k + 1] - off[k] <= kMaxItems, SVB_ERR_INVALID, "tc pair: %d work items on one CTA (limit %d)", off[k + 1] - off[k], kMaxItems);
+    double mx = 0;
+    for (double v : load) mx = std::max(mx, v);
+    *balance_out = mx > 0 ? total / grid / mx : 1.0;
+    return SVB_OK;
+}
+
+int tc_pair_worklist_build(int n, const TcPairChain *ch, const ConvArgs &a, int precision, bool chain_ordered, TcWorkList *out,
+                           const int *rows, cudaStream_t st) {
+    PairArgs p;
+    size_t smem = 0;
+    SVB_TRY(tc_pair_plan(n, ch, a, precision, p, smem));
+    const int grid = sm_count();
+    int ks1[kTcMaxLayers], ks2[kTcMaxLayers];
+    for (int l = 0; l < n; ++l) ks1[l] = ch[l].KS1, ks2[l] = ch[l].KS2;
+    std::vector<int4> items;
+    std::vector<int> off;
+    double balance = 0;
+    SVB_TRY(tc_pair_schedule(n, ks1, ks2, a.Cout, a.B, a.Tq, chain_ordered, grid, &items, &off, &balance, rows));
+    if (items.size() > out->cap_items || off.size() > out->cap_off) {
+        if (out->items) SVB_CUDA(cudaFree(out->items));
+        if (out->off) SVB_CUDA(cudaFree(out->off));
+        out->items = nullptr, out->off = nullptr;
+        out->cap_items = std::max<size_t>(items.size(), 1) * 5 / 4, out->cap_off = off.size();
+        SVB_CUDA(cudaMalloc((void **)&out->items, out->cap_items * sizeof(int4)));
+        SVB_CUDA(cudaMalloc((void **)&out->off, out->cap_off * sizeof(int)));
+    }
+    SVB_CUDA(cudaMemcpyAsync(out->items, items.data(), items.size() * sizeof(int4), cudaMemcpyHostToDevice, st));
+    SVB_CUDA(cudaMemcpyAsync(out->off, off.data(), off.size() * sizeof(int), cudaMemcpyHostToDevice, st));
+    out->grid = grid, out->n_items = (int)items.size(), out->MT = 1, out->n_layers = n, out->chain_ordered = chain_ordered;
+    out->valid = true;
+    if (getenv("SVB_TC_VERBOSE"))
+        fprintf(stderr, "[tc] pair work list: %d chains, %zu items over %d CTAs, balance %.3f (mean / max load)\n", n, items.size(), grid, balance);
+    return SVB_OK;
+}
+
+template <bool ST>
+static int launch_pair(const PairArgs &p, int grid, size_t smem, cudaStream_t st) {
+    auto kern = conv1d_pair_tc_kernel<ST>;
+    static size_t configured[kMaxDevices] = {};
+    static bool carve[kMaxDevices] = {};
+    int dev = 0;
+    SVB_CUDA(cudaGetDevice(&dev));
+    dev = dev < kMaxDevices ? dev : kMaxDevices - 1;
+    if (smem > configured[dev] || dev == kMaxDevices - 1) {
+        SVB_CUDA(cudaFuncSetAttribute(kern, cudaFuncAttributeMaxDynamicSharedMemorySize, (int)smem));
+        configured[dev] = smem;
+    }
+    if (!carve[dev]) {
+        SVB_CUDA(cudaFuncSetAttribute(kern, cudaFuncAttributePreferredSharedMemoryCarveout, cudaSharedmemCarveoutMaxShared));
+        carve[dev] = true;
+    }
+    cudaLaunchConfig_t cfg = {};
+    cfg.gridDim = dim3(grid), cfg.blockDim = dim3(kTcThreadsP), cfg.dynamicSmemBytes = smem, cfg.stream = st;
+    cudaLaunchAttribute attr[1];
+    attr[0].id = cudaLaunchAttributeProgrammaticStreamSerialization;
+    attr[0].val.programmaticStreamSerializationAllowed = p.pdl ? 1 : 0;
+    cfg.attrs = attr, cfg.numAttrs = 1;
+    SVB_CUDA(cudaLaunchKernelEx(&cfg, kern, p));
+    return SVB_OK;
+}
+
+int launch_conv_pair_tc(int n, const TcPairChain *ch, const ConvArgs &a, int precision, cudaStream_t st, const TcWorkList &wl) {
+    PairArgs p;
+    size_t smem = 0;
+    SVB_TRY(tc_pair_plan(n, ch, a, precision, p, smem));
+    SVB_CHECK(wl.valid && wl.n_layers == n && wl.MT == 1 && wl.grid == sm_count(), SVB_ERR_STATE, "tc pair: work list was built for another plan");
+    p.work = wl.items, p.work_off = wl.off;
+    if (!getenv("SVB_TC_STATS")) return launch_pair<false>(p, wl.grid, smem, st);
+    const int grid = wl.grid;
+    const size_t ns = (size_t)grid * kTcStatSlots;
+    SVB_CUDA(cudaMalloc((void **)&p.stats, ns * sizeof(long long)));
+    SVB_CUDA(cudaMemsetAsync(p.stats, 0, ns * sizeof(long long), st));
+    SVB_TRY(launch_pair<true>(p, grid, smem, st));
+    SVB_CUDA(cudaStreamSynchronize(st));
+    std::vector<long long> h(ns);
+    SVB_CUDA(cudaMemcpy(h.data(), p.stats, ns * sizeof(long long), cudaMemcpyDeviceToHost));
+    SVB_CUDA(cudaFree(p.stats));
+    double mean[kTcStatSlots] = {};
+    long long mx[kTcStatSlots] = {};
+    for (int c = 0; c < grid; ++c)
+        for (int i = 0; i < kTcStatSlots; ++i) mean[i] += (double)h[(size_t)c * kTcStatSlots + i] / grid, mx[i] = std::max(mx[i], h[(size_t)c * kTcStatSlots + i]);
+    long long g_first = h[12], g_last = h[13];
+    for (int c = 0; c < grid; ++c) g_first = std::min(g_first, h[(size_t)c * kTcStatSlots + 12]), g_last = std::max(g_last, h[(size_t)c * kTcStatSlots + 13]);
+    fprintf(stderr, "[tc-stats] grid span %.1f us (globaltimer, first CTA start -> last CTA end) = %.2f GHz over the mean CTA\n",
+            (g_last - g_first) / 1e3, mean[11] / std::max(1.0, (double)(g_last - g_first)));
+    fprintf(stderr,
+            "[tc-stats] pair %dx C%d k%d d%d Tq %d grid %d items %d | kcycles mean (max): total %.0f (%.0f) | producer: a_empty %.0f w_empty %.0f of %.0f | "
+            "mma: acc_empty %.0f a_ready %.0f w_full %.0f c2_full %.0f of %.0f | transform: raw_full %.0f of %.0f | epilogue: acc_full %.0f c2_empty %.0f of %.0f | smem %zu\n",
+            n, a.Cout, ch[n - 1].KS1, ch[n - 1].dil1, a.Tq, grid, wl.n_items, mean[11] / 1e3, mx[11] / 1e3, mean[0] / 1e3, mean[1] / 1e3, mean[2] / 1e3,
+            mean[3] / 1e3, mean[4] / 1e3, mean[5] / 1e3, mean[14] / 1e3, mean[6] / 1e3, mean[7] / 1e3, mean[8] / 1e3, mean[9] / 1e3, mean[15] / 1e3,
+            mean[10] / 1e3, smem);
+    return SVB_OK;
+}
+
 }
 
 extern "C" int64_t svb_tc_schedule_probe(int32_t n_layers, const int32_t *KS, const int32_t *has_res, const int32_t *accumulate, int32_t Cin,
@@ -1031,3 +1697,29 @@
     for (int c = 0; c <= grid; ++c) off_out[c] = off[c];
     return (int64_t)items.size();
 }
+
+extern "C" int64_t svb_tc_pair_schedule_probe(int32_t n_chains, const int32_t *KS1, const int32_t *KS2, int32_t C, int32_t B, int32_t Tq,
+                                              const int32_t *rows_per_clip, int32_t chain_ordered, int32_t grid, int32_t *items_out,
+                                              int64_t items_capacity, int32_t *off_out, double *balance_out) {
+    SVB_CHECK(n_chains >= 1 && n_chains <= svb::kTcMaxLayers && KS1 && KS2 && B > 0 && Tq > 0 && grid >= 1 && items_out && off_out && balance_out,
+              SVB_ERR_INVALID, "tc_pair_schedule_probe: bad argument");
+    std::vector<int> rows;
+    if (rows_per_clip) {
+        for (int b = 0; b < B; ++b)
+            SVB_CHECK(rows_per_clip[b] >= 1 && rows_per_clip[b] <= Tq, SVB_ERR_INVALID, "tc_pair_schedule_probe: clip %d has %d rows", b, rows_per_clip[b]);
+        rows.assign(rows_per_clip, rows_per_clip + B);
+    }
+    int k1[svb::kTcMaxLayers], k2[svb::kTcMaxLayers];
+    for (int l = 0; l < n_chains; ++l) k1[l] = KS1[l], k2[l] = KS2[l];
+    std::vector<int4> items;
+    std::vector<int> off;
+    SVB_TRY(svb::tc_pair_schedule(n_chains, k1, k2, C, B, Tq, chain_ordered != 0, grid, &items, &off, balance_out, rows.empty() ? nullptr : rows.data()));
+    SVB_CHECK((int64_t)items.size() <= items_capacity, SVB_ERR_INVALID, "tc_pair_schedule_probe: %zu items, capacity %lld", items.size(),
+              (long long)items_capacity);
+    for (size_t i = 0; i < items.size(); ++i) {
+        int32_t *o = items_out + 5 * i;
+        o[0] = items[i].x & 0xff, o[1] = items[i].y, o[2] = items[i].z, o[3] = items[i].x >> 8, o[4] = items[i].w;
+    }
+    for (int c = 0; c <= grid; ++c) off_out[c] = off[c];
+    return (int64_t)items.size();
+}
diff --git a/neuralsvb_b200/csrc/conv_tc.cuh b/neuralsvb_b200/csrc/conv_tc.cuh
--- a/neuralsvb_b200/csrc/conv_tc.cuh
+++ b/neuralsvb_b200/csrc/conv_tc.cuh
@@ -31,6 +31,19 @@
 void tc_worklist_free(TcWorkList *wl);
 bool tc_merge_fits(int n, int B, int Tq, int Cout, int n_tile, const int *rows = nullptr);
 int launch_conv_tc_multi(int n, const TcWeights *const *w, const ConvArgs *a, int precision, cudaStream_t st, const TcWorkList &wl);
+struct TcPairChain {
+    const TcWeights *w1, *w2;
+    const float *b1, *b2;
+    const float *x;
+    float *out;
+    int KS1, dil1, KS2;
+    float out_scale;
+    int accumulate;
+};
+bool tc_pair_supported(int C, int precision, const TcWeights &w1, const TcWeights &w2, int KS1, int dil1, int KS2, int dil2);
+int tc_pair_worklist_build(int n, const TcPairChain *ch, const ConvArgs &a, int precision, bool chain_ordered, TcWorkList *out,
+                           const int *rows = nullptr, cudaStream_t st = 0);
+int launch_conv_pair_tc(int n, const TcPairChain *ch, const ConvArgs &a, int precision, cudaStream_t st, const TcWorkList &wl);
 int launch_conv_tc(const TcWeights &w, const ConvArgs &a, int precision, cudaStream_t st, int max_ctas = 0);
 
 }
diff --git a/neuralsvb_b200/csrc/generator.cu b/neuralsvb_b200/csrc/generator.cu
--- a/neuralsvb_b200/csrc/generator.cu
+++ b/neuralsvb_b200/csrc/generator.cu
@@ -189,6 +189,31 @@
     return SVB_ERR_STATE;
 }
 
+int run_pair(svb_gen *g, int stage, int nk, const TcPairChain *ch, const ConvLayer *const *L1, const ConvLayer *const *L2, bool chain_ordered,
+             int B, int Tq, int Tp, cudaStream_t st) {
+    double bytes = 0, flops = 0;
+    const double rows = valid_rows_total(g, Tq);
+    for (int j = 0; j < nk; ++j) {
+        bytes += 4.0 * (rows * L1[j]->Cin + rows * L1[j]->Cout);
+        bytes += 4.0 * (rows * L2[j]->Cin + rows * L2[j]->Cout * (2 + (ch[j].accumulate ? 1 : 0)));
+        flops += 2.0 * (L1[j]->macs_per_row + L2[j]->macs_per_row) * rows;
+    }
+    g->last_launches += 1;
+    g->last_flops += flops;
+    ProfScope ps(g, st, "conv1d_c4_tc (resblock)", bytes, flops);
+    ConvArgs a;
+    a.in = ch[0].x, a.out = ch[0].out, a.res = nullptr, a.w = nullptr, a.bias = ch[0].b1;
+    a.B = B, a.Cin = L1[0]->Cin, a.Cout = L1[0]->Cout, a.CoutP = L1[0]->CoutP, a.in_Tp = Tp, a.out_Tp = Tp, a.Tq = Tq;
+    a.KS = ch[0].KS1, a.dil = ch[0].dil1, a.ups_u = 0, a.in_slope = 0.1f, a.out_scale = 1.f, a.accumulate = 0;
+    a.rows = g->cur_len_dev, a.rows_mul = Tq / g->cur_T;
+    TcWorkList &wl = g->worklists[1000 + stage * 2 + (chain_ordered ? 1 : 0)];
+    if (!wl.valid) {
+        const std::vector<int> rh = clip_rows(g, Tq);
+        SVB_TRY(tc_pair_worklist_build(nk, ch, a, g->cfg.precision, chain_ordered, &wl, rh.empty() ? nullptr : rh.data(), st));
+    }
+    return launch_conv_pair_tc(nk, ch, a, g->cfg.precision, st, wl);
+}
+
 int forward_impl(svb_gen *g, const float *mel, bool mel_frame_major, const float *f0, const float *rand_ini,
                  const float *noise, uint64_t seed, int B, int T, float *wav, cudaStream_t st, const int32_t *lens = nullptr,
                  bool packed = false) {
@@ -329,7 +354,12 @@
         g->taps["ups" + std::to_string(i)] = Tap{X, s.C, Ti, Tip, false};
         const bool par = g->chains > 1 && nk > 1 && nk <= 3 && g->cfg.precision != SVB_PREC_FP32 && !g->profile;
         const int sms = 148;
-        bool merged = g->merge && !par && nk > 1 && nk <= kTcMaxLayers && g->cfg.precision != SVB_PREC_FP32 &&
+        bool pair = g->merge && g->pair && !par && !g->training && g->cfg.resblock == 1 && nk <= kTcMaxLayers && s.C == 32;
+        for (int j = 0; pair && j < nk; ++j)
+            for (int m = 0; m < nd; ++m)
+                pair = pair && tc_pair_supported(s.C, g->cfg.precision, s.c1[j][m].tc, s.c2[j][m].tc, s.c1[j][m].KS, s.c1[j][m].dil,
+                                                 s.c2[j][m].KS, s.c2[j][m].dil);
+        bool merged = !pair && g->merge && !par && nk > 1 && nk <= kTcMaxLayers && g->cfg.precision != SVB_PREC_FP32 &&
                       s.c1[0][0].tc.ok;
         if (merged) {
             const std::vector<int> rh = clip_rows(g, Ti);
@@ -343,7 +373,21 @@
                 merged = merged && tc_supported(s.c1[j][m].tc, probe) && s.c1[j][m].tc.n_tile == s.c1[0][0].tc.n_tile;
                 if (g->cfg.resblock == 1) merged = merged && s.c2[j][m].tc.ok && s.c2[j][m].tc.n_tile == s.c1[0][0].tc.n_tile;
             }
-        if (merged) {
+        if (pair) {
+            for (int m = 0; m < nd; ++m) {
+                const bool last = m == nd - 1;
+                TcPairChain ch[kTcMaxLayers];
+                const ConvLayer *L1[kTcMaxLayers], *L2[kTcMaxLayers];
+                for (int j = 0; j < nk; ++j) {
+                    const ConvLayer &c1 = s.c1[j][m], &c2 = s.c2[j][m];
+                    float *out = last ? S : (m % 2 ? F(bf.A[i][j][m]) : F(bf.R[i][j][m]));
+                    const float *x = m == 0 ? X : (m % 2 ? F(bf.R[i][j][m - 1]) : F(bf.A[i][j][m - 1]));
+                    ch[j] = TcPairChain{&c1.tc, &c2.tc, c1.b, c2.b, x, out, c1.KS, c1.dil, c2.KS, last ? 1.f / nk : 1.f, (last && j > 0) ? 1 : 0};
+                    L1[j] = &c1, L2[j] = &c2;
+                }
+                SVB_TRY(run_pair(g, (int)i, nk, ch, L1, L2, last, B, Ti, Tip, st));
+            }
+        } else if (merged) {
             for (int m = 0; m < nd; ++m) {
                 const bool last = m == nd - 1;
                 const ConvLayer *L1[kTcMaxLayers], *L2[kTcMaxLayers];
@@ -373,7 +417,7 @@
             }
         }
         if (par) SVB_CUDA(cudaEventRecord(g->ev_fork, st));
-        for (int j = 0; j < nk && !merged; ++j) {
+        for (int j = 0; j < nk && !merged && !pair; ++j) {
             cudaStream_t cs = par ? g->side[j] : st;
             int cap = 0;
             if (par) {
@@ -467,6 +511,7 @@
     }
     if (const char *e = getenv("SVB_CHAINS")) g->chains = atoi(e);
     if (const char *e = getenv("SVB_MERGE")) g->merge = atoi(e) != 0;
+    if (const char *e = getenv("SVB_PAIR")) g->pair = atoi(e) != 0;
     if (const char *e = getenv("SVB_CHAIN_BIAS")) g->chain_bias = atof(e);
     *out = g;
     return SVB_OK;
diff --git a/neuralsvb_b200/csrc/generator.cuh b/neuralsvb_b200/csrc/generator.cuh
--- a/neuralsvb_b200/csrc/generator.cuh
+++ b/neuralsvb_b200/csrc/generator.cuh
@@ -128,6 +128,7 @@
     double chain_bias = 4.0;
 
     bool merge = true;
+    bool pair = true;
     std::map<int, svb::TcWorkList> worklists;
     std::vector<int> wl_len;
 
```

Result: faster. 5366, median of 6 (+2.8%).
